# cyu0330/ptbxl-multimodal

Hardware: AMD Instinct MI355X
Metric: ECG windows/s (train step) at 12x1000, batch 256 (higher is better)
Workload: dtype f32; 1 GPU; ECGCNN(5) train step fwd+BCE+bwd+AdamW, 12x1000, fp32, batch 256/GPU, global batch 256; global_batch=256, parallelism=dp1, loop=train_one_epoch, optimizer=FlatAdamW, priming_steps=30

## Files before the change

include/ecg_hip.h:

```cpp
#ifndef ECG_HIP_H
#define ECG_HIP_H

#include <stddef.h>
#include <stdint.h>

#ifdef __cplusplus
extern "C" {
#endif

typedef void *ecg_stream_t;

enum {
    ECG_OK = 0,
    ECG_EINVAL = 1,
    ECG_ELAUNCH = 2,
    ECG_ENODEV = 3
};

int ecg_version(void);
const char *ecg_last_error(void);
int ecg_check_device(void);


int ecg_conv1d_pack_weights(const float *w, float *w_fwd, float *w_bwd,
                            int C_out, int C_in, int K, ecg_stream_t stream);

int ecg_pack_weights_grouped(const float *const *w, float *const *w_fwd, float *const *w_bwd,
                             const int *C_out, const int *C_in, const int *K, int count,
                             ecg_stream_t stream);

int ecg_pack_weights_grouped_mixed(const float *const *w, float *const *w_fwd, float *const *w_bwd,
                                   void *const *wb_fwd, void *const *wb_bwd, const int *C_out,
                                   const int *C_in, const int *K, int count, ecg_stream_t stream);

int ecg_conv1d_fwd_stat_partials(int N, int C_in, int C_out, int L, int K, int pad);

int ecg_conv1d_fwd(const float *x, const float *w_fwd, const float *bias, float *y,
                   float *stat_partials, int N, int C_in, int C_out, int L, int K, int pad,
                   ecg_stream_t stream);

int ecg_conv1d_bwd_data(const float *dy, const float *w_bwd, float *dx,
                        int N, int C_in, int C_out, int L, int K, int pad, ecg_stream_t stream);

int ecg_conv1d_dy_row_stride(int N, int C_in, int C_out, int L, int K, int pad, int need_dx);

int ecg_conv1d_multiplies_per_output_pair(int op, int C_in, int C_out, int K, int pad);
int ecg_conv1d_bwd_data_ld(const float *dy, int ldy, const float *w_bwd, float *dx,
                           int N, int C_in, int C_out, int L, int K, int pad, ecg_stream_t stream);
int ecg_conv1d_bwd_weight_bias_ld(const float *dy, int ldy, const float *x, float *dw, float *db,
                                  float *ws, int N, int C_in, int C_out, int L, int K, int pad,
                                  ecg_stream_t stream);

size_t ecg_conv1d_bwd_weight_ws_floats(int N, int C_in, int C_out, int L, int K, int pad);
int ecg_conv1d_bwd_weight_bias(const float *dy, const float *x, float *dw, float *db, float *ws,
                               int N, int C_in, int C_out, int L, int K, int pad,
                               ecg_stream_t stream);

int ecg_conv1d_bf16_supported(int C_in, int C_out, int K, int pad);
size_t ecg_conv1d_bf16_packed_elems(int C_reduce, int C_result, int K);
int ecg_conv1d_pack_weights_bf16(const float *w, void *wb_fwd, void *wb_bwd, int C_out, int C_in,
                                 int K, ecg_stream_t stream);
int ecg_conv1d_fwd_bf16_yh(const void *x, int x_bf16, int ldx, const void *wb_fwd, const float *bias, void *y_bf16,
                           int ldy, float *stat_partials, int N, int C_in, int C_out, int L, int K, int pad,
                           ecg_stream_t stream);
int ecg_conv1d_fwd_bf16_yh_stat_partials(int N, int C_in, int C_out, int L, int K, int pad, int x_bf16, int ldx, int ldy);
int ecg_conv1d_bf16_ring_tile(int N, int C_red, int C_res, int L_out, int K, int pad, int ld_in, int ld_out);
int ecg_bn_stats_relu_pool_fwd_h(const float *stat_partials, int P, long long count, float *running_mean,
                                 float *running_var, long long *num_batches_tracked, float momentum, float eps,
                                 const void *y_bf16, int ldy, const float *gamma, const float *beta, float *mean,
                                 float *invstd, void *p_bf16, int ldp, int N, int C, int L, ecg_stream_t stream);
int ecg_bn_stats_relu_pool_gap_fwd_yh(const float *stat_partials, int P, long long count, float *running_mean,
                                      float *running_var, long long *num_batches_tracked, float momentum, float eps,
                                      const void *y_bf16, int ldy, const float *gamma, const float *beta, float *mean,
                                      float *invstd, float *out, int N, int C, int L, ecg_stream_t stream);
int ecg_bn_relu_pool_bwd_h(const void *y_bf16, int ldyy, const void *dp, int dp_kind, int ldp, const float *gamma,
                           const float *beta, const float *mean, const float *invstd, void *dy_bf16, int ldy,
                           float *dgamma, float *dbeta, float *ws, int N, int C, int L, int train,
                           ecg_stream_t stream);
int ecg_conv1d_bwd_data_bf16hh(const void *dy_bf16, int ldy, const void *wb_bwd, void *dx_bf16, int ldx, int N,
                               int C_in, int C_out, int L, int K, int pad, ecg_stream_t stream);
int ecg_conv1d_bf16_tk_supported(int C_in, int C_out, int K, int pad);
int ecg_conv1d_bf16_tk_dy_stride(int Lo);
size_t ecg_conv1d_bwd_weight_bf16_ncl_ws_floats(int N, int C_in, int C_out, int L, int K, int pad);
int ecg_conv1d_bwd_weight_bias_bf16_ncl(const void *dy_bf16, int ldy, const void *x, int x_is_bf16, int ldx,
                                        float *dw, float *db, float *ws, int N, int C_in, int C_out, int L,
                                        int K, int pad, ecg_stream_t stream);


int ecg_bn_stat_partials_count(int N, int C, int L);
int ecg_bn_stat_partials(const float *y, float *stat_partials, int N, int C, int L,
                         ecg_stream_t stream);

int ecg_bn_finalize(const float *stat_partials, int P, long long count,
                    float *mean, float *invstd, float *running_mean, float *running_var,
                    long long *num_batches_tracked, int C, float momentum, float eps,
                    ecg_stream_t stream);

int ecg_bn_invstd(const float *var, float *invstd, int C, float eps, ecg_stream_t stream);

int ecg_bn_relu_pool_fwd(const float *y, const float *gamma, const float *beta,
                         const float *mean, const float *invstd, float *p,
                         int N, int C, int L, ecg_stream_t stream);
int ecg_bn_stats_relu_pool_fwd(const float *stat_partials, int P, long long count, float *running_mean,
                               float *running_var, long long *num_batches_tracked, float momentum, float eps,
                               const float *y, const float *gamma, const float *beta, float *mean,
                               float *invstd, float *out, int N, int C, int L, int mode, ecg_stream_t stream);

int ecg_bn_relu_pool_bwd_one_launch_splits(int N, int C, int L, int ldy);
size_t ecg_bn_relu_pool_bwd_one_launch_counter_uints(int N, int C, int L, int ldy);
int ecg_bn_relu_pool_bwd_one_launch(const float *y, const float *dp, const float *gamma, const float *beta,
                                    const float *mean, const float *invstd, float *dy, int ldy,
                                    float *dgamma, float *dbeta, uint32_t *counters, int N, int C, int L,
                                    int train, int gap, int spin_polls, ecg_stream_t stream);

size_t ecg_bn_relu_pool_bwd_ws_floats(int N, int C, int L);
int ecg_bn_relu_pool_bwd(const float *y, const float *dp, const float *gamma, const float *beta,
                         const float *mean, const float *invstd,
                         float *dy, float *dgamma, float *dbeta, float *ws,
                         int N, int C, int L, int train, ecg_stream_t stream);
int ecg_bn_relu_pool_bwd_ld(const float *y, const float *dp, const float *gamma, const float *beta,
                            const float *mean, const float *invstd,
                            float *dy, int ldy, float *dgamma, float *dbeta, float *ws,
                            int N, int C, int L, int train, ecg_stream_t stream);

int ecg_conv1d_bn_relu_pool_eval_supported(int C_in, int C_out, int K, int pad);
int ecg_conv1d_bn_relu_pool_eval_fwd(const float *x, const float *w_fwd, const float *bias,
                                     const float *gamma, const float *beta,
                                     const float *running_mean, const float *running_var,
                                     float eps, float *p, int N, int C_in, int C_out, int L,
                                     int K, int pad, ecg_stream_t stream);
int ecg_conv1d_bn_relu_pool_gap_eval_supported(int C_in, int C_out, int L, int K, int pad);
int ecg_conv1d_bn_relu_pool_gap_eval_fwd(const float *x, const float *w_fwd, const float *bias,
                                         const float *gamma, const float *beta,
                                         const float *running_mean, const float *running_var,
                                         float eps, float *g, int N, int C_in, int C_out, int L,
                                         int K, int pad, ecg_stream_t stream);

int ecg_conv1d_bn_relu_pool_eval_bf16_supported(int C_in, int C_out, int L, int K, int pad, int gap);
int ecg_conv1d_bn_relu_pool_eval_fwd_bf16(const void *x, int x_bf16, int ldx, const void *wb_fwd, const float *bias,
                                          const float *gamma, const float *beta, const float *running_mean,
                                          const float *running_var, float eps, void *p, int p_bf16, int ldp, int N,
                                          int C_in, int C_out, int L, int K, int pad, ecg_stream_t stream);
int ecg_conv1d_bn_relu_pool_gap_eval_fwd_bf16(const void *x, int x_bf16, int ldx, const void *wb_fwd, const float *bias,
                                              const float *gamma, const float *beta, const float *running_mean,
                                              const float *running_var, float eps, float *g, int N, int C_in, int C_out,
                                              int L, int K, int pad, ecg_stream_t stream);

int ecg_bn_relu_pool_gap_fwd(const float *y, const float *gamma, const float *beta,
                             const float *mean, const float *invstd, float *g,
                             int N, int C, int L, ecg_stream_t stream);
int ecg_bn_relu_pool_gap_bwd(const float *y, const float *dg, const float *gamma, const float *beta,
                             const float *mean, const float *invstd,
                             float *dy, float *dgamma, float *dbeta, float *ws,
                             int N, int C, int L, int train, ecg_stream_t stream);
int ecg_bn_relu_pool_gap_bwd_ld(const float *y, const float *dg, const float *gamma,
                                const float *beta, const float *mean, const float *invstd,
                                float *dy, int ldy, float *dgamma, float *dbeta, float *ws,
                                int N, int C, int L, int train, ecg_stream_t stream);

int ecg_gradcam_supported(int C, int Lo, int K, int S);
size_t ecg_gradcam_ws_floats(int N, int C, int Lo, int K, int S);
int ecg_gradcam_fwd(const float *a, int lda, const float *scale, const float *shift, const float *u,
                    long long u_stride_n, float *cam, float *raw, float *alpha, float *g, float *ws,
                    int N, int C, int Lo, int K, int S, int norm, ecg_stream_t stream);

int ecg_bn_apply_fwd(const float *y, const float *gamma, const float *beta, const float *mean,
                     const float *invstd, float *out, int N, int C, int L, ecg_stream_t stream);
size_t ecg_bn_bwd_ws_floats(int N, int C, int L);
int ecg_bn_bwd(const float *y, const float *dout, const float *gamma, const float *mean,
               const float *invstd, float *dy, float *dgamma, float *dbeta, float *ws,
               int N, int C, int L, int train, ecg_stream_t stream);
int ecg_relu_fwd(const float *x, float *out, size_t n, ecg_stream_t stream);
int ecg_relu_bwd(const float *out, const float *dout, float *dx, size_t n, ecg_stream_t stream);
int ecg_maxpool2_fwd(const float *x, float *p, int rows, int L, ecg_stream_t stream);
int ecg_maxpool2_bwd(const float *x, const float *dp, float *dx, int rows, int L, ecg_stream_t stream);


int ecg_gap_fwd(const float *p, float *g, int rows, int L, ecg_stream_t stream);
int ecg_gap_bwd(const float *dg, float *dp, int rows, int L, ecg_stream_t stream);

int ecg_linear_fwd(const float *x, const float *w, const float *b, float *y,
                   int M, int In, int Out, int relu, ecg_stream_t stream);
size_t ecg_linear_bwd_ws_floats(int M, int In, int Out);
int ecg_linear_bwd(const float *x, const float *w, const float *y, const float *dy,
                   float *dx, float *dw, float *db, float *ws,
                   int M, int In, int Out, int relu, ecg_stream_t stream);

int ecg_film_fwd(const float *z, const float *film, float *zc, int M, int F, ecg_stream_t stream);
int ecg_film_bwd(const float *z, const float *film, const float *dzc, float *dz, float *dfilm,
                 int M, int F, ecg_stream_t stream);

int ecg_bce_logits_fwd(const float *x, const float *target, float *loss, float *dx,
                       int numel, double *running_sum, double weight, ecg_stream_t stream);
int ecg_sigmoid_fwd(const float *x, float *prob, size_t n, ecg_stream_t stream);


int ecg_transpose(const float *w, float *wT, int rows, int cols, ecg_stream_t stream);

int ecg_tail_fwd(const float *g, const float *xd, const float *WpT, const float *bp,
                 const float *W0, const float *b0, const float *W2, const float *b2,
                 const float *WfT, const float *bf, const float *Wh, const float *bh,
                 float *z, float *h1, float *h2, float *film, float *zc, float *logits,
                 int M, int F0, int F, int D, int H1, int H, int C, ecg_stream_t stream);

int ecg_tail_bwd_chain(const float *dlogits, const float *dz_extra, const float *z,
                       const float *h1, const float *h2, const float *film,
                       const float *Wp, const float *W0, const float *W2, const float *Wf,
                       const float *Wh, float *dzc, float *dz, float *dfilm, float *dh2m,
                       float *dh1m, float *dg, float *dxd, int M, int F0, int F, int D,
                       int H1, int H, int C, int demo, ecg_stream_t stream);

int ecg_linear_wgrad_grouped(const float *const *G, const float *const *X, float *const *dW,
                             float *const *db, const int *Out, const int *In, int count,
                             int M, ecg_stream_t stream);

int ecg_adamw_step(float *p, const float *g, float *m, float *v, size_t n, int step,
                   float lr, float beta1, float beta2, float eps, float weight_decay,
                   float grad_scale, ecg_stream_t stream);

int ecg_adamw_step_graph(float *p, const float *g, float *m, float *v, size_t n, int *step_dev,
                         float lr, float beta1, float beta2, float eps, float weight_decay,
                         float grad_scale, ecg_stream_t stream);

int ecg_wfdb16_physical(const int16_t *d, const double *gain, const int *baseline, float *out,
                        int B, int T, int leads, ecg_stream_t stream);
int ecg_wfdb16_zscore(const int16_t *d, const double *gain, const int *baseline, float *out,
                      float *stats, int B, int T, int leads, ecg_stream_t stream);
int ecg_zscore_rows(const float *x, float *out, float *stats, int rows, int T, ecg_stream_t stream);
int ecg_host_gather_rows(const void *src, size_t row_bytes, const long long *rows, int n, void *dst);

#ifdef __cplusplus
}
#endif
#endif
```

ptbxl-multimodal_amd/csrc/conv1d_api.hip:

```cpp
#include "common.h"

namespace ecg {
int direct_fwd_stat_partials(int N, int Lo);
int direct_fwd(const float *x, const float *wp, const float *bias, float *y, float *partials,
               int N, int Cin, int Cout, int L, int K, int pad, hipStream_t st);
size_t direct_wgrad_ws_floats(int N, int Cin, int Cout, int K);
int direct_wgrad(const float *dy, const float *x, float *dw, float *db, float *ws, int N, int Cin,
                 int Cout, int L, int K, int pad, hipStream_t st);
int pack_weights(const float *w, float *w_fwd, float *w_bwd, int Co, int Ci, int K,
                 hipStream_t st);
int pack_weights_grouped(const float *const *w, float *const *w_fwd, float *const *w_bwd, void *const *wb_fwd,
                         void *const *wb_bwd, const int *Co, const int *Ci, const int *K, int count, hipStream_t st);
bool mfma_fwd_supported(int Cin, int Cout, int K, int pad);
int mfma_fwd_stat_partials(int N, int Cin, int Cout, int Lo);
int mfma_fwd(const float *x, int ldx, const float *wp, const float *bias, float *y, float *partials,
             int N, int Cin, int Cout, int L, int K, int pad, hipStream_t st);
int mfma_fwd_eval_pool(const float *x, const float *wp, const float *bias, const float *gamma,
                       const float *beta, const float *mean, const float *var, float eps, float *p,
                       int N, int Cin, int Cout, int L, int K, int pad, hipStream_t st, int gap);
bool mfma_fwd_eval_gap_supported(int Cin, int Cout, int L, int K, int pad);
bool mfma_wgrad_supported(int Cin, int Cout, int K, int pad);
size_t mfma_wgrad_ws_floats(int N, int Cin, int Cout, int L, int K, int pad);
bool mfma_wgrad_dma_supported(int Cin, int Cout, int K);
int mfma_multiplies_per_pair(int op, int Cin, int Cout, int K, int pad);
int mfma_wgrad(const float *dy, int ldy, const float *x, float *dw, float *db, float *ws, int N,
               int Cin, int Cout, int L, int K, int pad, hipStream_t st);

static int check_conv_shape(int N, int Cin, int Cout, int L, int K, int pad) {
    ECG_REQUIRE(N > 0 && Cin > 0 && Cout > 0 && L > 0, "conv1d: N=%d C_in=%d C_out=%d L=%d must be > 0",
                N, Cin, Cout, L);
    ECG_REQUIRE(K >= 1 && K <= 31, "conv1d: kernel size %d outside [1,31]", K);
    ECG_REQUIRE(pad >= 0 && pad < K, "conv1d: padding %d outside [0,K)", pad);
    ECG_REQUIRE(L + 2 * pad - K + 1 > 0, "conv1d: empty output (L=%d K=%d pad=%d)", L, K, pad);
    ECG_REQUIRE(N <= 65535, "conv1d: N=%d exceeds grid.z limit 65535", N);
    return ECG_OK;
}
}

using namespace ecg;

ECG_API int ecg_conv1d_pack_weights(const float *w, float *w_fwd, float *w_bwd, int C_out,
                                    int C_in, int K, ecg_stream_t stream) {
    ECG_REQUIRE(w && (w_fwd || w_bwd), "pack_weights: null pointer");
    ECG_REQUIRE(C_out > 0 && C_in > 0 && K >= 1 && K <= 31, "pack_weights: bad shape");
    return pack_weights(w, w_fwd, w_bwd, C_out, C_in, K, as_stream(stream));
}

ECG_API int ecg_pack_weights_grouped(const float *const *w, float *const *w_fwd,
                                     float *const *w_bwd, const int *C_out, const int *C_in,
                                     const int *K, int count, ecg_stream_t stream) {
    ECG_REQUIRE(w && w_fwd && w_bwd && C_out && C_in && K, "pack_weights_grouped: null table");
    ECG_REQUIRE(count >= 1 && count <= 16, "pack_weights_grouped: count=%d outside [1,16]", count);
    for (int q = 0; q < count; ++q) {
        ECG_REQUIRE(w[q] && (w_fwd[q] || w_bwd[q]), "pack_weights_grouped: problem %d has null pointers", q);
        ECG_REQUIRE(C_out[q] > 0 && C_in[q] > 0 && K[q] >= 1 && K[q] <= 31,
                    "pack_weights_grouped: problem %d has a bad shape", q);
    }
    return pack_weights_grouped(w, w_fwd, w_bwd, nullptr, nullptr, C_out, C_in, K, count, as_stream(stream));
}

ECG_API int ecg_pack_weights_grouped_mixed(const float *const *w, float *const *w_fwd, float *const *w_bwd,
                                           void *const *wb_fwd, void *const *wb_bwd, const int *C_out,
                                           const int *C_in, const int *K, int count, ecg_stream_t stream) {
    ECG_REQUIRE(w && w_fwd && w_bwd && wb_fwd && wb_bwd && C_out && C_in && K, "pack_weights_grouped_mixed: null table");
    ECG_REQUIRE(count >= 1 && count <= 16, "pack_weights_grouped_mixed: count=%d outside [1,16]", count);
    for (int q = 0; q < count; ++q) {
        ECG_REQUIRE(w[q] && (w_fwd[q] || w_bwd[q] || wb_fwd[q] || wb_bwd[q]),
                    "pack_weights_grouped_mixed: problem %d has null pointers", q);
        ECG_REQUIRE(C_out[q] > 0 && C_in[q] > 0 && K[q] >= 1 && K[q] <= 31,
                    "pack_weights_grouped_mixed: problem %d has a bad shape", q);
        ECG_REQUIRE(K[q] <= 15 || !(wb_fwd[q] || wb_bwd[q]),
                    "pack_weights_grouped_mixed: problem %d asks for bf16 operands with K=%d > 15", q, K[q]);
    }
    return pack_weights_grouped(w, w_fwd, w_bwd, wb_fwd, wb_bwd, C_out, C_in, K, count, as_stream(stream));
}

ECG_API int ecg_conv1d_fwd_stat_partials(int N, int C_in, int C_out, int L, int K, int pad) {
    int Lo = L + 2 * pad - K + 1;
    if (mfma_fwd_supported(C_in, C_out, K, pad)) return mfma_fwd_stat_partials(N, C_in, C_out, Lo);
    return direct_fwd_stat_partials(N, Lo);
}

ECG_API int ecg_conv1d_fwd(const float *x, const float *w_fwd, const float *bias, float *y,
                           float *stat_partials, int N, int C_in, int C_out, int L, int K, int pad,
                           ecg_stream_t stream) {
    int rc = check_conv_shape(N, C_in, C_out, L, K, pad);
    if (rc) return rc;
    ECG_REQUIRE(x && w_fwd && y, "conv1d_fwd: null pointer");
    if (mfma_fwd_supported(C_in, C_out, K, pad))
        return mfma_fwd(x, L, w_fwd, bias, y, stat_partials, N, C_in, C_out, L, K, pad, as_stream(stream));
    return direct_fwd(x, w_fwd, bias, y, stat_partials, N, C_in, C_out, L, K, pad, as_stream(stream));
}

ECG_API int ecg_conv1d_dy_row_stride(int N, int C_in, int C_out, int L, int K, int pad, int need_dx) {
    (void)N;
    const int Lo = L + 2 * pad - K + 1;
    if (Lo <= 0) return Lo;
    if (mfma_wgrad_dma_supported(C_in, C_out, K) && (!need_dx || mfma_fwd_supported(C_out, C_in, K, K - 1 - pad)))
        return cdiv(Lo, 64) * 64;
    return Lo;
}

ECG_API int ecg_conv1d_multiplies_per_output_pair(int op, int C_in, int C_out, int K, int pad) {
    if (op < 0 || op > 3 || K < 1) return 0;
    return mfma_multiplies_per_pair(op, C_in, C_out, K, pad);
}

ECG_API int ecg_conv1d_bwd_data_ld(const float *dy, int ldy, const float *w_bwd, float *dx, int N,
                                   int C_in, int C_out, int L, int K, int pad, ecg_stream_t stream) {
    int rc = check_conv_shape(N, C_in, C_out, L, K, pad);
    if (rc) return rc;
    ECG_REQUIRE(dy && w_bwd && dx, "conv1d_bwd_data: null pointer");
    const int Lo = L + 2 * pad - K + 1, padb = K - 1 - pad;
    ECG_REQUIRE(ldy >= Lo, "conv1d_bwd_data: dY row stride %d < row length %d", ldy, Lo);
    if (mfma_fwd_supported(C_out, C_in, K, padb))
        return mfma_fwd(dy, ldy, w_bwd, nullptr, dx, nullptr, N, C_out, C_in, Lo, K, padb, as_stream(stream));
    ECG_REQUIRE(ldy == Lo, "conv1d_bwd_data: this shape needs dense dY rows (stride %d != %d); "
                "use the stride ecg_conv1d_dy_row_stride returns", ldy, Lo);
    return direct_fwd(dy, w_bwd, nullptr, dx, nullptr, N, C_out, C_in, Lo, K, padb, as_stream(stream));
}

ECG_API int ecg_conv1d_bwd_data(const float *dy, const float *w_bwd, float *dx, int N, int C_in,
                                int C_out, int L, int K, int pad, ecg_stream_t stream) {
    return ecg_conv1d_bwd_data_ld(dy, L + 2 * pad - K + 1, w_bwd, dx, N, C_in, C_out, L, K, pad, stream);
}

ECG_API size_t ecg_conv1d_bwd_weight_ws_floats(int N, int C_in, int C_out, int L, int K, int pad) {
    if (mfma_wgrad_supported(C_in, C_out, K, pad)) return mfma_wgrad_ws_floats(N, C_in, C_out, L, K, pad);
    return direct_wgrad_ws_floats(N, C_in, C_out, K);
}

ECG_API int ecg_conv1d_bwd_weight_bias_ld(const float *dy, int ldy, const float *x, float *dw,
                                          float *db, float *ws, int N, int C_in, int C_out, int L,
                                          int K, int pad, ecg_stream_t stream) {
    int rc = check_conv_shape(N, C_in, C_out, L, K, pad);
    if (rc) return rc;
    ECG_REQUIRE(dy && x && dw && ws, "conv1d_bwd_weight_bias: null pointer");
    const int Lo = L + 2 * pad - K + 1;
    ECG_REQUIRE(ldy >= Lo, "conv1d_bwd_weight_bias: dY row stride %d < row length %d", ldy, Lo);
    if (mfma_wgrad_supported(C_in, C_out, K, pad))
        return mfma_wgrad(dy, ldy, x, dw, db, ws, N, C_in, C_out, L, K, pad, as_stream(stream));
    ECG_REQUIRE(ldy == Lo, "conv1d_bwd_weight_bias: this shape needs dense dY rows (stride %d != %d); "
                "use the stride ecg_conv1d_dy_row_stride returns", ldy, Lo);
    return direct_wgrad(dy, x, dw, db, ws, N, C_in, C_out, L, K, pad, as_stream(stream));
}

ECG_API int ecg_conv1d_bwd_weight_bias(const float *dy, const float *x, float *dw, float *db,
                                       float *ws, int N, int C_in, int C_out, int L, int K, int pad,
                                       ecg_stream_t stream) {
    return ecg_conv1d_bwd_weight_bias_ld(dy, L + 2 * pad - K + 1, x, dw, db, ws, N, C_in, C_out, L, K,
                                         pad, stream);
}

ECG_API int ecg_conv1d_bn_relu_pool_eval_supported(int C_in, int C_out, int K, int pad) {
    return mfma_fwd_supported(C_in, C_out, K, pad) ? 1 : 0;
}

ECG_API int ecg_conv1d_bn_relu_pool_eval_fwd(const float *x, const float *w_fwd, const float *bias,
                                             const float *gamma, const float *beta,
                                             const float *running_mean, const float *running_var,
                                             float eps, float *p, int N, int C_in, int C_out, int L,
                                             int K, int pad, ecg_stream_t stream) {
    int rc = check_conv_shape(N, C_in, C_out, L, K, pad);
    if (rc) return rc;
    ECG_REQUIRE(x && w_fwd && gamma && beta && running_mean && running_var,
                "conv1d_bn_relu_pool_eval_fwd: null pointer");
    ECG_REQUIRE(mfma_fwd_supported(C_in, C_out, K, pad),
                "conv1d_bn_relu_pool_eval_fwd: shape not covered by the fused kernel "
                "(query ecg_conv1d_bn_relu_pool_eval_supported and use the unfused sequence)");
    const int Lo = L + 2 * pad - K + 1;
    if (Lo / 2 == 0) return ECG_OK;
    ECG_REQUIRE(p, "conv1d_bn_relu_pool_eval_fwd: null output");
    return mfma_fwd_eval_pool(x, w_fwd, bias, gamma, beta, running_mean, running_var, eps, p, N,
                              C_in, C_out, L, K, pad, as_stream(stream), 0);
}

ECG_API int ecg_conv1d_bn_relu_pool_gap_eval_supported(int C_in, int C_out, int L, int K, int pad) {
    return mfma_fwd_eval_gap_supported(C_in, C_out, L, K, pad) ? 1 : 0;
}

ECG_API int ecg_conv1d_bn_relu_pool_gap_eval_fwd(const float *x, const float *w_fwd, const float *bias,
                                                 const float *gamma, const float *beta,
                                                 const float *running_mean, const float *running_var,
                                                 float eps, float *g, int N, int C_in, int C_out, int L,
                                                 int K, int pad, ecg_stream_t stream) {
    int rc = check_conv_shape(N, C_in, C_out, L, K, pad);
    if (rc) return rc;
    ECG_REQUIRE(x && w_fwd && gamma && beta && running_mean && running_var && g,
                "conv1d_bn_relu_pool_gap_eval_fwd: null pointer");
    ECG_REQUIRE(mfma_fwd_eval_gap_supported(C_in, C_out, L, K, pad),
                "conv1d_bn_relu_pool_gap_eval_fwd: shape not covered (the conv output row must fit one time tile; "
                "query ecg_conv1d_bn_relu_pool_gap_eval_supported)");
    return mfma_fwd_eval_pool(x, w_fwd, bias, gamma, beta, running_mean, running_var, eps, g, N,
                              C_in, C_out, L, K, pad, as_stream(stream), 1);
}
```

ptbxl-multimodal_amd/csrc/conv1d_direct.hip:

```cpp
#include "common.h"
#include <cstdlib>

namespace ecg {

constexpr int kTT = 256;
constexpr int kKMax = 31;
constexpr int kCiChunk = 8;

__global__ void pack_weights_kernel(const float *__restrict__ w, float *__restrict__ w_fwd,
                                    float *__restrict__ w_bwd, int Co, int Ci, int K) {
    int idx = blockIdx.x * blockDim.x + threadIdx.x;
    int total = Co * Ci * K;
    if (idx >= total) return;
    int k = idx % K;
    int ci = (idx / K) % Ci;
    int co = idx / (K * Ci);
    float v = w[idx];
    if (w_fwd) w_fwd[((size_t)k * Ci + ci) * Co + co] = v;
    if (w_bwd) w_bwd[((size_t)(K - 1 - k) * Co + co) * Ci + ci] = v;
}

template <int CO_T, bool STATS>
__global__ __launch_bounds__(kTT) void conv1d_direct_kernel(
    const float *__restrict__ x, const float *__restrict__ wp, const float *__restrict__ bias,
    float *__restrict__ y, float *__restrict__ partials, int Cin, int Cout, int L, int Lo, int K,
    int pad, int P) {
    __shared__ float xs[kCiChunk][kTT + kKMax - 1];
    __shared__ float red[4][CO_T * 2];

    const int tl = threadIdx.x;
    const int t0 = blockIdx.x * kTT;
    const int co0 = blockIdx.y * CO_T;
    const int n = blockIdx.z;
    const int span = kTT + K - 1;

    float acc[CO_T];
#pragma unroll
    for (int j = 0; j < CO_T; ++j) acc[j] = 0.f;

    const float *xn = x + (size_t)n * Cin * L;
    for (int ci0 = 0; ci0 < Cin; ci0 += kCiChunk) {
        const int nci = min(kCiChunk, Cin - ci0);
        for (int c = 0; c < nci; ++c) {
            const float *xr = xn + (size_t)(ci0 + c) * L;
            for (int i = tl; i < span; i += kTT) {
                int s = t0 - pad + i;
                xs[c][i] = (s >= 0 && s < L) ? xr[s] : 0.f;
            }
        }
        __syncthreads();
        for (int c = 0; c < nci; ++c) {
            for (int k = 0; k < K; ++k) {
                const float xv = xs[c][tl + k];
                const float *wr = wp + ((size_t)k * Cin + (ci0 + c)) * Cout + co0;
#pragma unroll
                for (int j = 0; j < CO_T; ++j) acc[j] = __fmaf_rn(wr[j], xv, acc[j]);
            }
        }
        __syncthreads();
    }

    const int t = t0 + tl;
    const bool valid = t < Lo;
#pragma unroll
    for (int j = 0; j < CO_T; ++j) {
        if (bias) acc[j] += bias[co0 + j];
        if (valid) y[((size_t)n * Cout + co0 + j) * Lo + t] = acc[j];
    }

    if (STATS) {
        const int wave = tl >> 6, lane = tl & 63;
#pragma unroll
        for (int j = 0; j < CO_T; ++j) {
            float v = valid ? acc[j] : 0.f;
            float s = wave_sum(v), q = wave_sum(v * v);
            if (lane == 0) { red[wave][2 * j] = s; red[wave][2 * j + 1] = q; }
        }
        __syncthreads();
        if (tl < CO_T * 2) {
            float s = red[0][tl] + red[1][tl] + red[2][tl] + red[3][tl];
            int j = tl >> 1;
            int pidx = n * gridDim.x + blockIdx.x;
            partials[((size_t)(co0 + j) * P + pidx) * 2 + (tl & 1)] = s;
        }
    }
}

static int pick_co_tile(int Cout) {
    for (int c : {16, 8, 4, 2}) if (Cout % c == 0) return c;
    return 1;
}

template <bool STATS>
static void launch_direct(const float *x, const float *wp, const float *bias, float *y,
                          float *partials, int N, int Cin, int Cout, int L, int Lo, int K, int pad,
                          int P, hipStream_t st) {
    int cot = pick_co_tile(Cout);
    dim3 grid(cdiv(Lo, kTT), Cout / cot, N), block(kTT);
#define ECG_LAUNCH(CT) \
    hipLaunchKernelGGL((conv1d_direct_kernel<CT, STATS>), grid, block, 0, st, x, wp, bias, y, \
                       partials, Cin, Cout, L, Lo, K, pad, P)
    switch (cot) {
        case 16: ECG_LAUNCH(16); break;
        case 8: ECG_LAUNCH(8); break;
        case 4: ECG_LAUNCH(4); break;
        case 2: ECG_LAUNCH(2); break;
        default: ECG_LAUNCH(1); break;
    }
#undef ECG_LAUNCH
}

int direct_fwd_stat_partials(int N, int Lo) { return N * cdiv(Lo, kTT); }

int direct_fwd(const float *x, const float *wp, const float *bias, float *y, float *partials,
               int N, int Cin, int Cout, int L, int K, int pad, hipStream_t st) {
    const int Lo = L + 2 * pad - K + 1;
    const int P = direct_fwd_stat_partials(N, Lo);
    if (partials)
        launch_direct<true>(x, wp, bias, y, partials, N, Cin, Cout, L, Lo, K, pad, P, st);
    else
        launch_direct<false>(x, wp, bias, y, nullptr, N, Cin, Cout, L, Lo, K, pad, P, st);
    return check_launch("conv1d_direct_kernel");
}

template <int KK, int CO_R>
__global__ __launch_bounds__(kTT) void conv1d_wgrad_direct_kernel(
    const float *__restrict__ dy, const float *__restrict__ x, float *__restrict__ slab,
    int N, int Cin, int Cout, int L, int Lo, int pad, int S) {
    __shared__ float xs[kTT + KK - 1];
    __shared__ float red[4][CO_R * KK + CO_R];

    const int tl = threadIdx.x;
    const int ci = blockIdx.x;
    const int co0 = blockIdx.y * CO_R;
    const int s = blockIdx.z;
    const int n_begin = (int)((long long)N * s / S), n_end = (int)((long long)N * (s + 1) / S);

    float acc[CO_R][KK];
    float bacc[CO_R];
#pragma unroll
    for (int j = 0; j < CO_R; ++j) {
        bacc[j] = 0.f;
#pragma unroll
        for (int k = 0; k < KK; ++k) acc[j][k] = 0.f;
    }

    for (int n = n_begin; n < n_end; ++n) {
        const float *xr = x + ((size_t)n * Cin + ci) * L;
        const float *dyn = dy + ((size_t)n * Cout + co0) * Lo;
        for (int t0 = 0; t0 < Lo; t0 += kTT) {
            __syncthreads();
            for (int i = tl; i < kTT + KK - 1; i += kTT) {
                int sidx = t0 - pad + i;
                xs[i] = (sidx >= 0 && sidx < L) ? xr[sidx] : 0.f;
            }
            __syncthreads();
            const int t = t0 + tl;
            float xv[KK];
#pragma unroll
            for (int k = 0; k < KK; ++k) xv[k] = xs[tl + k];
#pragma unroll
            for (int j = 0; j < CO_R; ++j) {
                float d = (t < Lo) ? dyn[(size_t)j * Lo + t] : 0.f;
                bacc[j] += d;
#pragma unroll
                for (int k = 0; k < KK; ++k) acc[j][k] = __fmaf_rn(d, xv[k], acc[j][k]);
            }
        }
    }

    const int wave = tl >> 6, lane = tl & 63;
#pragma unroll
    for (int j = 0; j < CO_R; ++j) {
#pragma unroll
        for (int k = 0; k < KK; ++k) {
            float v = wave_sum(acc[j][k]);
            if (lane == 0) red[wave][j * KK + k] = v;
        }
        float b = wave_sum(bacc[j]);
        if (lane == 0) red[wave][CO_R * KK + j] = b;
    }
    __syncthreads();
    const size_t wslab = (size_t)Cout * Cin * KK;
    if (tl < CO_R * KK) {
        int j = tl / KK, k = tl % KK;
        float v = red[0][tl] + red[1][tl] + red[2][tl] + red[3][tl];
        slab[(size_t)s * wslab + ((size_t)(co0 + j) * Cin + ci) * KK + k] = v;
    } else if (tl < CO_R * KK + CO_R && ci == 0) {
        int j = tl - CO_R * KK;
        float v = red[0][tl] + red[1][tl] + red[2][tl] + red[3][tl];
        slab[(size_t)S * wslab + (size_t)s * Cout + co0 + j] = v;
    }
}

__global__ __launch_bounds__(kTT) void conv1d_wgrad_generic_kernel(
    const float *__restrict__ dy, const float *__restrict__ x, float *__restrict__ slab,
    int N, int Cin, int Cout, int L, int Lo, int K, int pad) {
    __shared__ double red[4];
    const int ci = blockIdx.x, co = blockIdx.y, tl = threadIdx.x;
    const int wave = tl >> 6, lane = tl & 63;
    const size_t wslab = (size_t)Cout * Cin * K;
    for (int k = 0; k <= K; ++k) {
        if (k == K && ci != 0) break;
        double a = 0.0;
        for (int n = 0; n < N; ++n) {
            const float *dyr = dy + ((size_t)n * Cout + co) * Lo;
            const float *xr = x + ((size_t)n * Cin + ci) * L;
            for (int t = tl; t < Lo; t += kTT) {
                if (k == K) { a += dyr[t]; continue; }
                int sidx = t + k - pad;
                if (sidx >= 0 && sidx < L) a += (double)dyr[t] * (double)xr[sidx];
            }
        }
        a = wave_sum(a);
        __syncthreads();
        if (lane == 0) red[wave] = a;
        __syncthreads();
        if (tl == 0) {
            float v = (float)(red[0] + red[1] + red[2] + red[3]);
            if (k == K) slab[wslab + co] = v;
            else slab[((size_t)co * Cin + ci) * K + k] = v;
        }
    }
}

template <int G>
__global__ __launch_bounds__(64 * G) void wgrad_reduce_kernel(const float *__restrict__ slab,
                                                              float *__restrict__ dw,
                                                              float *__restrict__ db, size_t wslab,
                                                              int Cout, int S) {
    __shared__ double part[G][64];
    const int lane = threadIdx.x & 63, w = threadIdx.x >> 6;
    const size_t i = (size_t)blockIdx.x * 64 + lane;
    const size_t total = wslab + Cout;
    const bool live = i < total && (i < wslab || db);
    double a = 0.0;
    if (live) {
        const float *src = i < wslab ? slab + i : slab + (size_t)S * wslab + (i - wslab);
        const size_t stride = i < wslab ? wslab : (size_t)Cout;
        int s = w;
        for (; s + 3 * G < S; s += 4 * G) {
            const float v0 = src[(size_t)s * stride], v1 = src[(size_t)(s + G) * stride];
            const float v2 = src[(size_t)(s + 2 * G) * stride], v3 = src[(size_t)(s + 3 * G) * stride];
            a += (double)v0; a += (double)v1; a += (double)v2; a += (double)v3;
        }
        for (; s < S; s += G) a += (double)src[(size_t)s * stride];
    }
    if (G > 1) {
        part[w][lane] = a;
        __syncthreads();
        if (w != 0) return;
#pragma unroll
        for (int g = 1; g < G; ++g) a += part[g][lane];
    }
    if (live) {
        if (i < wslab) dw[i] = (float)a; else db[i - wslab] = (float)a;
    }
}

template <int G>
__global__ __launch_bounds__(64 * G) void wgrad_reduce4_kernel(const float *__restrict__ slab, float *__restrict__ dw,
                                                               float *__restrict__ db, size_t wslab, int Cout, int S) {
    __shared__ double part[G][64][4];
    const int lane = threadIdx.x & 63, w = threadIdx.x >> 6;
    const size_t i = ((size_t)blockIdx.x * 64 + lane) * 4;
    const size_t total = wslab + Cout;
    const bool live = i < total && (i < wslab || db);
    double a[4] = {0.0, 0.0, 0.0, 0.0};
    if (live) {
        const float *src = i < wslab ? slab + i : slab + (size_t)S * wslab + (i - wslab);
        const size_t stride = i < wslab ? wslab : (size_t)Cout;
        int s = w;
        for (; s + 7 * G < S; s += 8 * G) {
            float4 v[8];
#pragma unroll
            for (int u = 0; u < 8; ++u) v[u] = *reinterpret_cast<const float4 *>(src + (size_t)(s + u * G) * stride);
#pragma unroll
            for (int u = 0; u < 8; ++u) {
                a[0] += (double)v[u].x; a[1] += (double)v[u].y; a[2] += (double)v[u].z; a[3] += (double)v[u].w;
            }
        }
        for (; s + 3 * G < S; s += 4 * G) {
            const float4 v0 = *reinterpret_cast<const float4 *>(src + (size_t)s * stride);
            const float4 v1 = *reinterpret_cast<const float4 *>(src + (size_t)(s + G) * stride);
            const float4 v2 = *reinterpret_cast<const float4 *>(src + (size_t)(s + 2 * G) * stride);
            const float4 v3 = *reinterpret_cast<const float4 *>(src + (size_t)(s + 3 * G) * stride);
            a[0] += (double)v0.x; a[0] += (double)v1.x; a[0] += (double)v2.x; a[0] += (double)v3.x;
            a[1] += (double)v0.y; a[1] += (double)v1.y; a[1] += (double)v2.y; a[1] += (double)v3.y;
            a[2] += (double)v0.z; a[2] += (double)v1.z; a[2] += (double)v2.z; a[2] += (double)v3.z;
            a[3] += (double)v0.w; a[3] += (double)v1.w; a[3] += (double)v2.w; a[3] += (double)v3.w;
        }
        for (; s < S; s += G) {
            const float4 v = *reinterpret_cast<const float4 *>(src + (size_t)s * stride);
            a[0] += (double)v.x; a[1] += (double)v.y; a[2] += (double)v.z; a[3] += (double)v.w;
        }
    }
    if (G > 1) {
#pragma unroll
        for (int e = 0; e < 4; ++e) part[w][lane][e] = a[e];
        __syncthreads();
        if (w != 0) return;
#pragma unroll
        for (int g = 1; g < G; ++g)
#pragma unroll
            for (int e = 0; e < 4; ++e) a[e] += part[g][lane][e];
    }
    if (live) {
        const float4 o = make_float4((float)a[0], (float)a[1], (float)a[2], (float)a[3]);
        if (i < wslab) *reinterpret_cast<float4 *>(dw + i) = o; else *reinterpret_cast<float4 *>(db + (i - wslab)) = o;
    }
}

int wgrad_reduce(const float *ws, float *dw, float *db, size_t wslab, int Cout, int S,
                 hipStream_t st) {
    const size_t total = wslab + Cout;
    if (wslab % 4 == 0 && Cout % 4 == 0 && (size_t)cdiv(total, 64) >= 1024 &&
        ((reinterpret_cast<uintptr_t>(ws) | reinterpret_cast<uintptr_t>(dw) | reinterpret_cast<uintptr_t>(db)) & 15) == 0) {
        hipLaunchKernelGGL((wgrad_reduce4_kernel<1>), dim3(cdiv(total / 4, 64)), dim3(64), 0, st, ws, dw, db, wslab, Cout, S);
        return check_launch("wgrad_reduce4_kernel");
    }
    const dim3 grid(cdiv(total, 64));
    int G = 1;
    while (G < 16 && (size_t)grid.x * G < 1024 && S / (2 * G) >= 8) G *= 2;
#define ECG_RED(GG) hipLaunchKernelGGL((wgrad_reduce_kernel<GG>), grid, dim3(64 * GG), 0, st, ws, dw, db, wslab, Cout, S)
    switch (G) {
        case 1: ECG_RED(1); break;
        case 2: ECG_RED(2); break;
        case 4: ECG_RED(4); break;
        case 8: ECG_RED(8); break;
        default: ECG_RED(16); break;
    }
#undef ECG_RED
    return check_launch("wgrad_reduce_kernel");
}

static bool wgrad_fast_ok(int Cout, int K) { return K == 15 && Cout % 8 == 0; }

int direct_wgrad_splits(int N, int Cin, int Cout, int K) {
    if (!wgrad_fast_ok(Cout, K)) return 1;
    long long base = (long long)Cin * (Cout / 8);
    long long s = (2048 + base - 1) / base;
    if (s < 1) s = 1;
    if (s > N) s = N;
    return (int)s;
}

size_t direct_wgrad_ws_floats(int N, int Cin, int Cout, int K) {
    int S = direct_wgrad_splits(N, Cin, Cout, K);
    return (size_t)S * ((size_t)Cout * Cin * K + Cout);
}

int direct_wgrad(const float *dy, const float *x, float *dw, float *db, float *ws, int N, int Cin,
                 int Cout, int L, int K, int pad, hipStream_t st) {
    const int Lo = L + 2 * pad - K + 1;
    const int S = direct_wgrad_splits(N, Cin, Cout, K);
    const size_t wslab = (size_t)Cout * Cin * K;
    if (wgrad_fast_ok(Cout, K)) {
        dim3 grid(Cin, Cout / 8, S), block(kTT);
        hipLaunchKernelGGL((conv1d_wgrad_direct_kernel<15, 8>), grid, block, 0, st, dy, x, ws, N,
                           Cin, Cout, L, Lo, pad, S);
    } else {
        dim3 grid(Cin, Cout), block(kTT);
        hipLaunchKernelGGL(conv1d_wgrad_generic_kernel, grid, block, 0, st, dy, x, ws, N, Cin,
                           Cout, L, Lo, K, pad);
    }
    int rc = check_launch("conv1d_wgrad kernel");
    if (rc) return rc;
    return wgrad_reduce(ws, dw, db, wslab, Cout, S, st);
}

int pack_weights(const float *w, float *w_fwd, float *w_bwd, int Co, int Ci, int K, hipStream_t st);

constexpr int kMaxPack = 16;
constexpr int kPackCo = 16, kPackCi = 16, kPackKMax = 15;
struct PackProb { const float *w; float *w_fwd, *w_bwd; unsigned short *wb_fwd, *wb_bwd; int Co, Ci, K, block0, ci_tiles; };
struct PackArgs { PackProb p[kMaxPack]; int count; };

__device__ __forceinline__ unsigned pack_bf16_pair(float lo, float hi) {
    return (unsigned)__builtin_bit_cast(unsigned short, (__bf16)lo) | ((unsigned)__builtin_bit_cast(unsigned short, (__bf16)hi) << 16);
}

__device__ __forceinline__ void pack_tile_bf16(const PackProb &pr, const float *tile, int ld, int co0, int ci0, int nco,
                                               int nci, int tid) {
    const int K = pr.K;
    if (pr.wb_fwd) {
        unsigned *dst = reinterpret_cast<unsigned *>(pr.wb_fwd + ((size_t)(ci0 / kPackCi) * K * pr.Co + co0) * kPackCi);
        for (int e = tid; e < K * nco * 8; e += 256) {
            const int jp = e & 7, r = e >> 3, co = r % nco, k = r / nco;
            const float lo = 2 * jp < nci ? tile[co * ld + (2 * jp) * K + k] : 0.f;
            const float hi = 2 * jp + 1 < nci ? tile[co * ld + (2 * jp + 1) * K + k] : 0.f;
            dst[((size_t)k * pr.Co + co) * 8 + jp] = pack_bf16_pair(lo, hi);
        }
    }
    if (pr.wb_bwd) {
        unsigned *dst = reinterpret_cast<unsigned *>(pr.wb_bwd + ((size_t)(co0 / kPackCo) * K * pr.Ci + ci0) * kPackCo);
        for (int e = tid; e < K * nci * 8; e += 256) {
            const int jp = e & 7, r = e >> 3, ci = r % nci, k = r / nci;
            const float lo = 2 * jp < nco ? tile[(2 * jp) * ld + ci * K + (K - 1 - k)] : 0.f;
            const float hi = 2 * jp + 1 < nco ? tile[(2 * jp + 1) * ld + ci * K + (K - 1 - k)] : 0.f;
            dst[((size_t)k * pr.Ci + ci) * 8 + jp] = pack_bf16_pair(lo, hi);
        }
    }
}

__global__ __launch_bounds__(256) void pack_weights_grouped_kernel(PackArgs a) {
    __shared__ float tile[kPackCo * (kPackCi * kPackKMax + 1)];
    int pi = 0;
#pragma unroll
    for (int q = 1; q < kMaxPack; ++q)
        if (q < a.count && (int)blockIdx.x >= a.p[q].block0) pi = q;
    const PackProb pr = a.p[pi];
    const int t = (int)blockIdx.x - pr.block0;
    const int co0 = (t / pr.ci_tiles) * kPackCo, ci0 = (t % pr.ci_tiles) * kPackCi;
    const int nco = min(kPackCo, pr.Co - co0), nci = min(kPackCi, pr.Ci - ci0);
    const int K = pr.K, run = nci * K, ld = kPackCi * kPackKMax + 1;
    const int tid = threadIdx.x;
    if (K == 15 && nco == kPackCo && nci == kPackCi) {
        constexpr int KC = 15, RUN = kPackCi * KC;
        const float *src = pr.w + ((size_t)co0 * pr.Ci + ci0) * KC;
        static_assert((kPackCo * RUN) % 256 == 0, "whole passes");
#pragma unroll
        for (int it = 0; it < kPackCo * RUN / 256; ++it) {
            const int e = tid + 256 * it;
            const int co = e / RUN, r = e - co * RUN;
            tile[co * ld + r] = src[(size_t)co * pr.Ci * KC + r];
        }
        __syncthreads();
        if (pr.w_fwd) {
#pragma unroll
            for (int it = 0; it < kPackCo * RUN / 256; ++it) {
                const int e = tid + 256 * it;
                const int co = e % kPackCo, r = e / kPackCo, k = r / kPackCi, ci = r - k * kPackCi;
                pr.w_fwd[((size_t)k * pr.Ci + ci0 + ci) * pr.Co + co0 + co] = tile[co * ld + ci * KC + k];
            }
        }
        if (pr.w_bwd) {
#pragma unroll
            for (int it = 0; it < kPackCo * RUN / 256; ++it) {
                const int e = tid + 256 * it;
                const int ci = e % kPackCi, r = e / kPackCi, co = r % kPackCo, k = r / kPackCo;
                pr.w_bwd[((size_t)(KC - 1 - k) * pr.Co + co0 + co) * pr.Ci + ci0 + ci] = tile[co * ld + ci * KC + k];
            }
        }
        pack_tile_bf16(pr, tile, ld, co0, ci0, nco, nci, tid);
        return;
    }
    for (int e = tid; e < nco * run; e += 256) {
        const int co = e / run, r = e - co * run;
        tile[co * ld + r] = pr.w[((size_t)(co0 + co) * pr.Ci + ci0) * K + r];
    }
    __syncthreads();
    if (pr.w_fwd)
        for (int e = tid; e < run * kPackCo; e += 256) {
            const int co = e % kPackCo, r = e / kPackCo;
            const int k = r / nci, ci = r - k * nci;
            if (co < nco) pr.w_fwd[((size_t)k * pr.Ci + ci0 + ci) * pr.Co + co0 + co] = tile[co * ld + ci * K + k];
        }
    if (pr.w_bwd)
        for (int e = tid; e < K * nco * nci; e += 256) {
            const int ci = e % nci, r = e / nci;
            const int co = r % nco, k = r / nco;
            pr.w_bwd[((size_t)(K - 1 - k) * pr.Co + co0 + co) * pr.Ci + ci0 + ci] = tile[co * ld + ci * K + k];
        }
    pack_tile_bf16(pr, tile, ld, co0, ci0, nco, nci, tid);
}

int pack_weights_grouped(const float *const *w, float *const *w_fwd, float *const *w_bwd, void *const *wb_fwd,
                         void *const *wb_bwd, const int *Co, const int *Ci, const int *K, int count, hipStream_t st) {
    PackArgs a;
    a.count = count;
    int blocks = 0;
    for (int q = 0; q < count; ++q) {
        if (K[q] > kPackKMax) {
            int rc = pack_weights(w[q], w_fwd[q], w_bwd[q], Co[q], Ci[q], K[q], st);
            if (rc) return rc;
            a.p[q] = PackProb{nullptr, nullptr, nullptr, nullptr, nullptr, 0, 0, 1, blocks, 1};
            continue;
        }
        const int ci_tiles = cdiv(Ci[q], kPackCi);
        a.p[q] = PackProb{w[q], w_fwd[q], w_bwd[q], static_cast<unsigned short *>(wb_fwd ? wb_fwd[q] : nullptr),
                          static_cast<unsigned short *>(wb_bwd ? wb_bwd[q] : nullptr), Co[q], Ci[q], K[q], blocks, ci_tiles};
        blocks += cdiv(Co[q], kPackCo) * ci_tiles;
    }
    for (int q = count; q < kMaxPack; ++q) a.p[q] = PackProb{nullptr, nullptr, nullptr, nullptr, nullptr, 0, 0, 1, 1 << 30, 1};
    if (blocks == 0) return ECG_OK;
    hipLaunchKernelGGL(pack_weights_grouped_kernel, dim3(blocks), dim3(256), 0, st, a);
    return check_launch("pack_weights_grouped_kernel");
}

int pack_weights(const float *w, float *w_fwd, float *w_bwd, int Co, int Ci, int K,
                 hipStream_t st) {
    int total = Co * Ci * K;
    hipLaunchKernelGGL(pack_weights_kernel, dim3(cdiv(total, 256)), dim3(256), 0, st, w, w_fwd,
                       w_bwd, Co, Ci, K);
    return check_launch("pack_weights_kernel");
}

}
```

ptbxl-multimodal_amd/csrc/conv1d_mfma.hip:

```cpp
#include "mfma_util.h"
#include <cstdlib>
#include <type_traits>

namespace ecg {

constexpr int kKM = 15;

#ifdef ECG_STAMP
__device__ unsigned long long *g_stamps = nullptr;
#endif

__device__ __forceinline__ f32x16 mfma32(float a, float b, f32x16 c) {
    return __builtin_amdgcn_mfma_f32_32x32x2f32(a, b, c, 0, 0, 0);
}

__device__ __forceinline__ void wait_lgkm_f(int n) {
    switch (n) {
        case 1: __builtin_amdgcn_s_waitcnt(0xC17F); break;
        case 2: __builtin_amdgcn_s_waitcnt(0xC27F); break;
        case 3: __builtin_amdgcn_s_waitcnt(0xC37F); break;
        case 4: __builtin_amdgcn_s_waitcnt(0xC47F); break;
        default: break;
    }
}

enum { EPI_PLAIN = 0, EPI_STATS = 1, EPI_EVAL = 2, EPI_EVAL_GAP = 3 };
struct EvalEpi { const float *gamma, *beta, *mean, *var; float eps; int gap; };

#ifndef ECG_FFA_MINB
#define ECG_FFA_MINB 2
#endif
#ifndef ECG_FFA_FLP2
#define ECG_FFA_FLP2 64
#endif
template <int CO_T, int M_T, int WCO, int WT, int EPI, int CI_C = 4, int FLP = 1>
__global__ __launch_bounds__(256, ECG_FFA_MINB) void conv1d_mfma_ffa_kernel(
    const float *__restrict__ x, const float *__restrict__ wp, const float *__restrict__ bias,
    float *__restrict__ y, float *__restrict__ partials, int Cin, int Cout, int L, int ldx, int Lo,
    int pad, int P, int tiles_t, EvalEpi ev) {
    constexpr bool STATS = (EPI == EPI_STATS), GAP = (EPI == EPI_EVAL_GAP);
    constexpr bool EVALM = (EPI == EPI_EVAL || EPI == EPI_EVAL_GAP);
    static_assert(WCO * WT == 4, "4 waves per workgroup");
    static_assert(kKM == 15, "tap split 8 + 7");
    static_assert(CO_T / WCO == 32 && M_T / WT == 32, "one 32 x 32 accumulator per product and wave");
    constexpr int KK = kKM, NJ = (KK + 1) / 2, NST = NJ * (CI_C / 2);
    constexpr int T_T = 2 * M_T, TS = T_T - 2;
    constexpr int XS = T_T + 16;
    constexpr int WSZ = KK * CI_C * CO_T;
    constexpr int NDMA = (WSZ + 255) / 256;
    constexpr int WPAD = NDMA * 256;
    constexpr int DPW = (NDMA + 3) / 4;
    constexpr int XEL = CI_C * XS;
    constexpr int XLOADS = (XEL + 255) / 256;
    constexpr int IMG = WPAD + XEL;
    constexpr int BXS = M_T + 1;
    constexpr int REDF = (STATS || GAP) ? 4 * 32 * 2 : 0;
    static_assert(CO_T * BXS + REDF <= 2 * IMG, "B exchange + stat scratch alias the dead images");
    static_assert(NST >= 2 * XLOADS + DPW, "not enough steps to spread the staging over");

    __shared__ __attribute__((aligned(1024))) float lds[2 * IMG];

    const int tid = threadIdx.x, lane = tid & 63, wave = tid >> 6;
    const int half = lane >> 5, l31 = lane & 31;
    ECG_STAMP_AT(g_stamps, 0);
    const int CT = Cout / CO_T;
    const int tile = xcd_chunked(blockIdx.x, gridDim.x);
    const int tile_co = tile % CT, tile_nt = tile / CT;
    const int tile_t = tile_nt % tiles_t, n = tile_nt / tiles_t;
    const int t0 = tile_t * TS, co0 = tile_co * CO_T;
    const int wco = (wave / WT) * 32, wm = (wave % WT) * 32;
    const float *xn = x + (size_t)n * Cin * ldx;

    f32x16 acc[3], acc2[3];
    f32x16 zero16;
#pragma unroll
    for (int r = 0; r < 16; ++r) zero16[r] = 0.f;
#pragma unroll
    for (int a = 0; a < 3; ++a) { acc[a] = zero16; acc2[a] = zero16; }

    const int pch = co0 + wco + acc_row(l31 & 15, half);
    const float p_b = bias ? bias[pch] : 0.f;
    float p_mu = 0.f, p_sc = 0.f, p_be = 0.f;
    if (EVALM) {
        const float is = (float)(1.0 / sqrt((double)ev.var[pch] + (double)ev.eps));
        p_sc = is * ev.gamma[pch]; p_mu = ev.mean[pch]; p_be = ev.beta[pch];
    }

    int woff[DPW];
#pragma unroll
    for (int j = 0; j < DPW; ++j) {
        const int e = min(((j * 4 + wave) * 64 + lane) * 4, WSZ - 4);
        const int row = e / CO_T, col = e - row * CO_T;
        const int k = row / CI_C, ci = row - k * CI_C;
        woff[j] = (k * Cin + ci) * Cout + col;
    }
    int xoff[XLOADS];
    unsigned xmask = 0;
#pragma unroll
    for (int j = 0; j < XLOADS; ++j) {
        const int e = min(tid + 256 * j, XEL - 1);
        const int ci = e / XS, pos = e - ci * XS;
        const int s = t0 - pad + pos;
        xoff[j] = ci * ldx + min(max(s, 0), L - 1);
        xmask |= ((s >= 0) && (s < L)) ? (1u << j) : 0u;
    }
    float xreg[XLOADS];

    const unsigned lds_base = (unsigned)(size_t)(__attribute__((address_space(3))) float *)lds;
    const int wave_u = __builtin_amdgcn_readfirstlane(wave);
    auto dma_w = [&](int j, int ci0, float *img) {
        if ((j * 4 + wave_u) < NDMA)
            glds16(wp + (size_t)ci0 * Cout + co0, (unsigned)woff[j] * 4u,
                   (unsigned)__builtin_amdgcn_readfirstlane((int)(lds_base + (unsigned)((img - lds) + (j * 4 + wave_u) * 256) * 4u)));
    };
    auto load_x = [&](int j, int ci0) { xreg[j] = xn[(size_t)ci0 * ldx + xoff[j]]; };
    auto commit_x = [&](int j, float *img) {
        const int e = tid + 256 * j;
        const unsigned keep = 0u - ((xmask >> j) & 1u);
        if (256 * (j + 1) <= XEL || e < XEL)
            img[WPAD + e] = __uint_as_float(__float_as_uint(xreg[j]) & keep);
    };

    const int nchunks = Cin / CI_C;
#pragma unroll
    for (int j = 0; j < DPW; ++j) dma_w(j, 0, lds);
#pragma unroll
    for (int j = 0; j < XLOADS; ++j) load_x(j, 0);
#pragma unroll
    for (int j = 0; j < XLOADS; ++j) commit_x(j, lds);
    if (nchunks > 1) {
#pragma unroll
        for (int j = 0; j < XLOADS; ++j) load_x(j, CI_C);
    }
    asm volatile("s_waitcnt vmcnt(0)" ::: "memory");
    __syncthreads();
    ECG_STAMP_AT(g_stamps, 1);

    typedef float f32x2t __attribute__((ext_vector_type(2)));
    auto chunk = [&](int c, auto open_c, auto close_c) {
        constexpr bool OPEN = decltype(open_c)::value, CLOSE = decltype(close_c)::value;
        const float *ws = lds + (c & 1) * IMG, *xs = ws + WPAD;
        float *nxt = lds + ((c + 1) & 1) * IMG;
        const bool do_next = c + 1 < nchunks, do_next2 = c + 2 < nchunks;
        const int ci_next = (c + 1) * CI_C, ci_next2 = (c + 2) * CI_C;

        auto ld = [&](int st, float &wa, float &wb, f32x2t &xq) {
            const int j = st / (CI_C / 2), cp = st % (CI_C / 2);
            const float *wrow = ws + ((2 * j * CI_C + 2 * cp + half) * CO_T + wco + l31);
            wa = wrow[0];
            wb = (2 * j + 1 < KK) ? wrow[CI_C * CO_T] : 0.f;
            xq = *reinterpret_cast<const f32x2t *>(xs + (2 * cp + half) * XS + 2 * (wm + l31) + 2 * j);
        };
        float wa_c, wb_c, wa_n, wb_n, wprev[CI_C / 2];
        f32x2t xq_c, xq_n;
#pragma unroll
        for (int i = 0; i < CI_C / 2; ++i) wprev[i] = 0.f;
        ld(0, wa_c, wb_c, xq_c);
#pragma unroll
        for (int st = 0; st < NST; ++st) {
            const int j = st / (CI_C / 2), cp = st % (CI_C / 2);
            ld(st + 1 < NST ? st + 1 : 0, wa_n, wb_n, xq_n);
            wait_lgkm_f(3);
            if (st < XLOADS) {
                if (do_next) commit_x(st, nxt);
            } else if (st < XLOADS + DPW) {
                if (do_next) dma_w(st - XLOADS, ci_next, nxt);
            } else if (st < 2 * XLOADS + DPW) {
                if (do_next2) load_x(st - XLOADS - DPW, ci_next2);
            }
            const float wc = wa_c - wprev[cp];
            const float xc = xq_c[0] - xq_c[1];
            __builtin_amdgcn_sched_barrier(0);
            acc[0] = mfma32(wa_c, xq_c[0], (OPEN && j == 0 && cp == 0) ? zero16 : acc[0]);
            if (2 * j + 1 < KK) acc[1] = mfma32(wb_c, xq_c[1], (OPEN && j == 0 && cp == 0) ? zero16 : acc[1]);
            acc[2] = mfma32(wc, xc, (OPEN && j == 0 && cp == 0) ? zero16 : acc[2]);
            __builtin_amdgcn_sched_barrier(0);
            wprev[cp] = wb_c;
            wa_c = wa_n; wb_c = wb_n; xq_c = xq_n;
        }
        if (CLOSE) {
#pragma unroll
            for (int a = 0; a < 3; ++a) acc2[a] += acc[a];
        }
        asm volatile("s_waitcnt vmcnt(0)" ::: "memory");
        __syncthreads();
        if (c == 0) ECG_STAMP_AT(g_stamps, 2);
    };
    {
        const std::true_type yes{};
        const std::false_type no{};
        int c = 0;
        if (FLP == 2) {
            for (; c + 1 < nchunks; c += 2) { chunk(c, yes, no); chunk(c + 1, no, yes); }
        }
        for (; c < nchunks; ++c) chunk(c, yes, yes);
    }
#pragma unroll
    for (int a = 0; a < 3; ++a) acc[a] = acc2[a];
    ECG_STAMP_AT(g_stamps, 3);

    __builtin_amdgcn_s_waitcnt(0x0F70);
    float *bx = lds, *red = lds + CO_T * BXS;
#pragma unroll
    for (int r = 0; r < 16; ++r) bx[(wco + acc_row(r, half)) * BXS + wm + l31] = acc[1][r];
    __syncthreads();
    f32x16 bn;
#pragma unroll
    for (int r = 0; r < 16; ++r) bn[r] = bx[(wco + acc_row(r, half)) * BXS + min(wm + l31 + 1, M_T - 1)];
    auto pick = [&](float v, int r) {
        const int vi = __float_as_int(v);
        const float lo = __int_as_float(__builtin_amdgcn_readlane(vi, r));
        const float hi = __int_as_float(__builtin_amdgcn_readlane(vi, r + 32));
        return half ? hi : lo;
    };
    float st_s = 0.f, st_q = 0.f;
    const int m = wm + l31, t = t0 + 2 * m;
    const bool ok0 = m < M_T - 1 && t < Lo, ok1 = m < M_T - 1 && t + 1 < Lo;
    const int Lp = Lo >> 1, pm = (t0 >> 1) + m;
    const bool okp = m < M_T - 1 && pm < Lp;
    float *yw = EVALM ? y + ((size_t)n * Cout + co0 + wco + 4 * half) * Lp + pm
                      : y + ((size_t)n * Cout + co0 + wco + 4 * half) * Lo + t;
#pragma unroll
    for (int r = 0; r < 16; ++r) {
        const int rowk = (r & 3) + 8 * (r >> 2);
        const float bv = pick(p_b, r);
        const float v0 = (acc[0][r] + acc[1][r]) + bv;
        const float v1 = ((acc[0][r] + bn[r]) - acc[2][r]) + bv;
        float s = 0.f, q = 0.f;
        if (EVALM) {
            const float mu = pick(p_mu, r), sc = pick(p_sc, r), be = pick(p_be, r);
            const float mx = fmaxf(fmaxf(bn_apply1(v0, mu, sc, be), bn_apply1(v1, mu, sc, be)), 0.f);
            if (GAP) {
                s = row16_sum(okp ? mx : 0.f);
                st_s += ((l31 & 15) == r) ? s : 0.f;
            } else if (okp) yw[rowk * Lp] = mx;
            continue;
        }
        typedef float f32x2u __attribute__((ext_vector_type(2), aligned(4)));
        if (ok1) { f32x2u v; v[0] = v0; v[1] = v1; *reinterpret_cast<f32x2u *>(yw + rowk * Lo) = v; }
        else if (ok0) yw[rowk * Lo] = v0;
        if (STATS) {
            if (ok0) { s += v0; q = __fmaf_rn(v0, v0, q); }
            if (ok1) { s += v1; q = __fmaf_rn(v1, v1, q); }
        }
        if (STATS) {
            const bool mine = (l31 & 15) == r;
            s = row16_sum(s);
            st_s += mine ? s : 0.f;
            q = row16_sum(q);
            st_q += mine ? q : 0.f;
        }
    }
    if (STATS || GAP) {
        const float s = st_s + __shfl_xor(st_s, 16, 64);
        const float q = st_q + __shfl_xor(st_q, 16, 64);
        if (l31 < 16) {
            const int lc = acc_row(l31, half);
            red[(wave * 32 + lc) * 2] = s;
            red[(wave * 32 + lc) * 2 + 1] = q;
        }
        __syncthreads();
    }
    if (GAP) {
        for (int col = tid; col < CO_T; col += 256) {
            const int wrow = col / 32, lc = col - wrow * 32;
            float g = 0.f;
#pragma unroll
            for (int j = 0; j < WT; ++j) g += red[((wrow * WT + j) * 32 + lc) * 2];
            y[(size_t)n * Cout + co0 + col] = g / (float)Lp;
        }
    }
    if (STATS) {
        for (int e = tid; e < CO_T * 2; e += 256) {
            const int col = e >> 1, w = e & 1;
            const int wrow = col / 32, lc = col - wrow * 32;
            float s2 = 0.f;
#pragma unroll
            for (int j = 0; j < WT; ++j) s2 += red[((wrow * WT + j) * 32 + lc) * 2 + w];
            const int pidx = n * tiles_t + tile_t;
            partials[((size_t)(co0 + col) * P + pidx) * 2 + w] = s2;
        }
    }
#ifdef ECG_STAMP
    asm volatile("s_waitcnt vmcnt(0)" ::: "memory");
#endif
    ECG_STAMP_AT(g_stamps, 4);
}

struct FwdCfg { int co_t, t_t, stride; };

static FwdCfg fwd_cfg(int Cout) {
    if (Cout % 64 == 0) return {64, 128, 126};
    return {32, 256, 254};
}

bool mfma_fwd_supported(int Cin, int Cout, int K, int pad) {
    (void)pad;
    return K == kKM && Cin % 4 == 0 && Cout % 32 == 0;
}

int mfma_fwd_stat_partials(int N, int Cin, int Cout, int Lo) {
    (void)Cin;
    return N * cdiv(Lo, fwd_cfg(Cout).stride);
}

template <int CO_T, int T_T, int WCO, int WT>
static void launch_fwd(const float *x, const float *wp, const float *bias, float *y,
                       float *partials, const EvalEpi *ev, int N, int Cin, int Cout, int L, int ldx,
                       int Lo, int pad, hipStream_t st) {
    const int tiles_t = cdiv(Lo, T_T - 2);
    dim3 grid((unsigned)((size_t)tiles_t * (Cout / CO_T) * N)), block(256);
    const int P = N * tiles_t;
    const EvalEpi none{nullptr, nullptr, nullptr, nullptr, 0.f, 0};
#define ECG_FFA(MODE, EV) do { \
    if (ECG_FFA_FLP2 && Cin % 8 == 0 && Cin >= ECG_FFA_FLP2) \
        hipLaunchKernelGGL((conv1d_mfma_ffa_kernel<CO_T, T_T / 2, WCO, WT, MODE, 4, 2>), grid, block, 0, st, x, wp, \
                           bias, y, partials, Cin, Cout, L, ldx, Lo, pad, P, tiles_t, EV); \
    else \
        hipLaunchKernelGGL((conv1d_mfma_ffa_kernel<CO_T, T_T / 2, WCO, WT, MODE>), grid, block, 0, st, x, wp, bias, y, \
                           partials, Cin, Cout, L, ldx, Lo, pad, P, tiles_t, EV); } while (0)
    if (ev && ev->gap) ECG_FFA(EPI_EVAL_GAP, *ev);
    else if (ev) ECG_FFA(EPI_EVAL, *ev);
    else if (partials) ECG_FFA(EPI_STATS, none);
    else ECG_FFA(EPI_PLAIN, none);
#undef ECG_FFA
}

static int mfma_fwd_any(const float *x, const float *wp, const float *bias, float *y,
                        float *partials, const EvalEpi *ev, int N, int Cin, int Cout, int L, int ldx,
                        int K, int pad, hipStream_t st) {
    const int Lo = L + 2 * pad - K + 1;
    if (fwd_cfg(Cout).co_t == 64)
        launch_fwd<64, 128, 2, 2>(x, wp, bias, y, partials, ev, N, Cin, Cout, L, ldx, Lo, pad, st);
    else
        launch_fwd<32, 256, 1, 4>(x, wp, bias, y, partials, ev, N, Cin, Cout, L, ldx, Lo, pad, st);
    return check_launch("conv1d_mfma_ffa_kernel");
}

int mfma_fwd(const float *x, int ldx, const float *wp, const float *bias, float *y, float *partials,
             int N, int Cin, int Cout, int L, int K, int pad, hipStream_t st) {
    return mfma_fwd_any(x, wp, bias, y, partials, nullptr, N, Cin, Cout, L, ldx, K, pad, st);
}

int mfma_fwd_eval_pool(const float *x, const float *wp, const float *bias, const float *gamma,
                       const float *beta, const float *mean, const float *var, float eps, float *p,
                       int N, int Cin, int Cout, int L, int K, int pad, hipStream_t st, int gap) {
    const EvalEpi ev{gamma, beta, mean, var, eps, gap};
    return mfma_fwd_any(x, wp, bias, p, nullptr, &ev, N, Cin, Cout, L, L, K, pad, st);
}

bool mfma_fwd_eval_gap_supported(int Cin, int Cout, int L, int K, int pad) {
    const int Lo = L + 2 * pad - K + 1;
    return mfma_fwd_supported(Cin, Cout, K, pad) && Lo >= 2 && Lo <= fwd_cfg(Cout).stride;
}

template <int M_T, int R_T, int WM, int WR, int WK, int T_T, int KK>
__global__ __launch_bounds__(256, 2) void conv1d_mfma_wgrad_kernel(
    const float *__restrict__ dy, const float *__restrict__ x, float *__restrict__ slab, int N,
    int Cin, int Cout, int L, int Lo, int ldy, int pad, int S) {
    static_assert(WM * WR * WK == 4, "4 waves per workgroup");
    constexpr int MC = M_T / WM / 32, MR = R_T / WR / 32;
    constexpr int TW = T_T / WK;
    constexpr int NST = TW / 2;
    constexpr int DS = T_T + 1;
    constexpr int XSPAN = T_T + KK - 1;
    constexpr int XS = ((XSPAN - KK + 31) / 32) * 32 + KK;
    constexpr int NCI = (R_T + KK - 2) / KK + 1;
    constexpr int DEL = M_T * T_T, DLOADS = DEL / 256;
    constexpr int XEL = NCI * XS, XLOADS = (XEL + 255) / 256;
    constexpr int NOPS = DLOADS + XLOADS;
    constexpr int IMG = M_T * DS + XEL;
    constexpr int ACCF = MC * MR * 16 * 64;
    constexpr int LDSF = (WK > 1 && WM * WR * ACCF > 2 * IMG) ? WM * WR * ACCF : 2 * IMG;
    static_assert(XS >= XSPAN, "x row stride too small");
    static_assert(DEL % 256 == 0, "dY tile must be a whole number of 256-thread passes");
    static_assert(256 % T_T == 0 || T_T % 256 == 0, "dY tile rows per pass");
    static_assert(XLOADS <= 32 && DLOADS <= 64, "mask bits");

    __shared__ float lds[LDSF + (WK > 1 ? 4 * 32 : 0)];

    const int tid = threadIdx.x, lane = tid & 63, wave = tid >> 6;
    const int half = lane >> 5, l31 = lane & 31;
    const int R = Cin * KK;
    const int RT = (R + R_T - 1) / R_T, CT = Cout / M_T;
    const int tile = xcd_chunked(blockIdx.x, gridDim.x);
    const int tile_r = tile % RT, tile_cs = tile / RT;
    const int r0 = tile_r * R_T, co0 = (tile_cs % CT) * M_T, s = tile_cs / CT;
    const int wk = wave % WK, wr = (wave / WK) % WR, wm = wave / (WK * WR);
    const int wm0 = wm * (M_T / WM), wr0 = wr * (R_T / WR), wt0 = wk * TW;
    const int ci_base = r0 / KK;
    const int n_begin = (int)((long long)N * s / S), n_end = (int)((long long)N * (s + 1) / S);

    int xcol[MR];
#pragma unroll
    for (int j = 0; j < MR; ++j) {
        int r = r0 + wr0 + 32 * j + l31;
        if (r >= R) r = R - 1;
        const int ci = r / KK;
        xcol[j] = (ci - ci_base) * XS + (r - ci * KK);
    }

    f32x16 acc[MC][MR], acc2[MC][MR];
    f32x16 zero16;
#pragma unroll
    for (int r = 0; r < 16; ++r) zero16[r] = 0.f;
#pragma unroll
    for (int a = 0; a < MC; ++a)
#pragma unroll
        for (int b = 0; b < MR; ++b) { acc[a][b] = zero16; acc2[a][b] = zero16; }
    float bsum[MC], bsum2[MC];
#pragma unroll
    for (int a = 0; a < MC; ++a) bsum[a] = bsum2[a] = 0.f;
    const bool want_bias = (tile_r == 0) && (wr == 0);

    constexpr int RPP = (T_T >= 256) ? 1 : 256 / T_T;
    constexpr int PPR = (T_T >= 256) ? T_T / 256 : 1;
    const int drow0 = (T_T >= 256) ? 0 : tid / T_T, dtt = (T_T >= 256) ? tid : tid % T_T;
    int xci[XLOADS], xpos[XLOADS];
#pragma unroll
    for (int j = 0; j < XLOADS; ++j) {
        const int e = min(tid + 256 * j, XEL - 1);
        xci[j] = min(ci_base + e / XS, Cin - 1) * L;
        xpos[j] = e % XS - pad;
    }
    float dreg[DLOADS], xreg[XLOADS];
    unsigned xmask = 0, dmask = 0;
    const int ntt = (Lo + T_T - 1) / T_T;
    const int total = (n_end - n_begin) * ntt;

    const float *dyn = dy, *xn = x;
    int dvoff = 0, t0 = 0;
    auto stage_setup = [&](int it) {
        const int n = n_begin + it / ntt;
        t0 = (it % ntt) * T_T;
        dyn = dy + ((size_t)n * Cout + co0) * ldy + t0;
        xn = x + (size_t)n * Cin * L;
        dvoff = drow0 * ldy + min(dtt, Lo - 1 - t0);
        dmask = 0;
#pragma unroll
        for (int q = 0; q < PPR; ++q) dmask |= (t0 + dtt + 256 * q < Lo) ? (1u << q) : 0u;
    };
    auto load_op = [&](int o) {
        if (o < DLOADS) {
            const int extra = (o % PPR) * 256;
            const float *pj = dyn + (size_t)(o / PPR) * RPP * ldy;
            dreg[o] = pj[PPR == 1 ? dvoff : drow0 * ldy + min(dtt + extra, Lo - 1 - t0)];
        } else {
            const int j = o - DLOADS;
            const int sidx = t0 + xpos[j];
            xreg[j] = xn[xci[j] + min(max(sidx, 0), L - 1)];
            const unsigned bit = ((sidx >= 0) && (sidx < L)) ? (1u << j) : 0u;
            xmask = (j == 0) ? bit : (xmask | bit);
        }
    };
    unsigned cxmask = 0, cdmask = 0;
    auto commit_op = [&](int o, float *img) {
        if (o < DLOADS) {
            const int row = drow0 + (o / PPR) * RPP, tt = dtt + (o % PPR) * 256;
            const unsigned keep = 0u - ((cdmask >> (o % PPR)) & 1u);
            img[row * DS + tt] = __uint_as_float(__float_as_uint(dreg[o]) & keep);
        } else {
            const int j = o - DLOADS;
            const int e = tid + 256 * j;
            const unsigned keep = 0u - ((cxmask >> j) & 1u);
            if (256 * (j + 1) <= XEL || e < XEL)
                img[M_T * DS + e] = __uint_as_float(__float_as_uint(xreg[j]) & keep);
        }
    };

    if (total > 0) {
        stage_setup(0);
#pragma unroll
        for (int o = 0; o < NOPS; ++o) load_op(o);
        cxmask = xmask; cdmask = dmask;
#pragma unroll
        for (int o = 0; o < NOPS; ++o) commit_op(o, lds);
        if (total > 1) {
            stage_setup(1);
#pragma unroll
            for (int o = 0; o < NOPS; ++o) load_op(o);
        }
    }
    __syncthreads();

    for (int it = 0; it < total; ++it) {
        const float *dys = lds + (it & 1) * IMG, *xs = dys + M_T * DS;
        float *nxt = lds + ((it + 1) & 1) * IMG;
        const bool do_commit = it + 1 < total, do_load = it + 2 < total;
        cxmask = xmask; cdmask = dmask;
        if (do_load) stage_setup(it + 2);

        const float *arow = dys + (wm0 + l31) * DS + wt0 + half;
        const float *brow = xs + wt0 + half;
        auto ld = [&](int tp, float *a, float *b) {
#pragma unroll
            for (int i = 0; i < MC; ++i) a[i] = arow[32 * i * DS + tp];
#pragma unroll
            for (int j = 0; j < MR; ++j) b[j] = brow[xcol[j] + tp];
        };
        float a_c[MC], b_c[MR], a_n[MC], b_n[MR];
        ld(0, a_c, b_c);
        constexpr int H1 = NST / 2;
#pragma unroll
        for (int st = 0; st < NST; ++st) {
            ld(st + 1 < NST ? 2 * (st + 1) : 0, a_n, b_n);
            if (st < H1) {
                if (do_commit) {
#pragma unroll
                    for (int o = st * NOPS / H1; o < (st + 1) * NOPS / H1; ++o) commit_op(o, nxt);
                }
            } else {
                if (do_load) {
#pragma unroll
                    for (int o = (st - H1) * NOPS / (NST - H1); o < (st - H1 + 1) * NOPS / (NST - H1); ++o)
                        load_op(o);
                }
            }
            __builtin_amdgcn_sched_barrier(0);
#pragma unroll
            for (int i = 0; i < MC; ++i) bsum[i] = (st == 0) ? a_c[i] : bsum[i] + a_c[i];
#pragma unroll
            for (int i = 0; i < MC; ++i)
#pragma unroll
                for (int j = 0; j < MR; ++j)
                    acc[i][j] = mfma32(a_c[i], b_c[j], (st == 0) ? zero16 : acc[i][j]);
            __builtin_amdgcn_sched_barrier(0);
#pragma unroll
            for (int i = 0; i < MC; ++i) a_c[i] = a_n[i];
#pragma unroll
            for (int j = 0; j < MR; ++j) b_c[j] = b_n[j];
        }
#pragma unroll
        for (int i = 0; i < MC; ++i)
#pragma unroll
            for (int j = 0; j < MR; ++j) acc2[i][j] += acc[i][j];
#pragma unroll
        for (int i = 0; i < MC; ++i) bsum2[i] += bsum[i];
        __syncthreads();
    }

#pragma unroll
    for (int i = 0; i < MC; ++i) {
        bsum[i] = bsum2[i];
#pragma unroll
        for (int j = 0; j < MR; ++j) acc[i][j] = acc2[i][j];
    }
    if (WK > 1) {
        float *bred = lds + LDSF;
        float *ex = lds + (wr + WR * wm) * ACCF;
        for (int w = 1; w < WK; ++w) {
            __syncthreads();
            if (wk == w) {
#pragma unroll
                for (int i = 0; i < MC; ++i)
#pragma unroll
                    for (int j = 0; j < MR; ++j)
#pragma unroll
                        for (int r = 0; r < 16; ++r)
                            ex[((i * MR + j) * 16 + r) * 64 + lane] = acc[i][j][r];
            }
            __syncthreads();
            if (wk == 0) {
#pragma unroll
                for (int i = 0; i < MC; ++i)
#pragma unroll
                    for (int j = 0; j < MR; ++j)
#pragma unroll
                        for (int r = 0; r < 16; ++r)
                            acc[i][j][r] += ex[((i * MR + j) * 16 + r) * 64 + lane];
            }
        }
        static_assert(WK == 1 || (WM == 1 && MC == 1), "the bias exchange below assumes one 32-channel row, wk fastest in the wave index");
        {
            const float b = bsum[0] + __shfl_xor(bsum[0], 32, 64);
            __syncthreads();
            if (want_bias && half == 0) bred[wave * 32 + l31] = b;
            __syncthreads();
            if (want_bias && wave == 0 && half == 0) {
                float t = bred[l31];
                for (int w = 1; w < WK; ++w) t += bred[w * 32 + l31];
                bsum[0] = t;
            }
        }
    } else if (want_bias) {
#pragma unroll
        for (int i = 0; i < MC; ++i) bsum[i] += __shfl_xor(bsum[i], 32, 64);
    }

    const size_t wslab = (size_t)Cout * R;
    if (wk == 0) {
        float *out = slab + (size_t)s * wslab;
#pragma unroll
        for (int i = 0; i < MC; ++i)
#pragma unroll
            for (int j = 0; j < MR; ++j) {
                const int r = r0 + wr0 + 32 * j + l31;
                if (r < R) {
#pragma unroll
                    for (int q = 0; q < 16; ++q) {
                        const int co = co0 + wm0 + 32 * i + acc_row(q, half);
                        out[(size_t)co * R + r] = acc[i][j][q];
                    }
                }
            }
        if (want_bias && half == 0) {
#pragma unroll
            for (int i = 0; i < MC; ++i)
                slab[(size_t)S * wslab + (size_t)s * Cout + co0 + wm0 + 32 * i + l31] = bsum[i];
        }
    }
}

template <int M_T, int R_T, int WM, int WR, int WK, int KK, int T_T = 64>
__global__ __launch_bounds__(256, 2) void conv1d_mfma_wgrad_dma_kernel(
    const float *__restrict__ dy, const float *__restrict__ x, float *__restrict__ slab, int N,
    int Cin, int Cout, int L, int Lo, int ldy, int pad, int S) {
    static_assert(WM * WR * WK == 4, "4 waves per workgroup");
    static_assert(T_T == 64 || T_T == 128, "64 or 128 time steps per stage");
    constexpr int LPR = T_T / 4, RPP = 64 / LPR;
    constexpr int MC = M_T / WM / 32, MR = R_T / WR / 32;
    constexpr int TW = T_T / WK;
    constexpr int NST = TW / 2, NGRP = NST / 4;
    static_assert(NST % 4 == 0, "whole groups of four steps");
    constexpr int XSPAN = T_T + KK - 1;
    constexpr int XS = ((XSPAN - KK + 31) / 32) * 32 + KK;
    constexpr int NCI = (R_T + KK - 2) / KK + 1;
    constexpr int XEL = NCI * XS, XLOADS = (XEL + 255) / 256;
    constexpr int AEL = M_T * T_T;
    constexpr int NDMA = AEL / 256;
    constexpr int DPW = NDMA / 4;
    constexpr int IMG = ((AEL + XEL + 63) / 64) * 64;
    constexpr int ACCF = MC * MR * 16 * 64;
    static_assert(WK == 1 || WM * WR * ACCF + 4 * 32 <= 2 * IMG, "accumulator exchange must fit the dead images");
    static_assert(XS >= XSPAN, "x row stride too small");
    static_assert(NDMA % 4 == 0, "dY image must split evenly over the four waves");
    static_assert(XLOADS <= 32, "mask bits");
    static_assert(NST >= 2 * XLOADS + DPW, "not enough steps to spread the staging over");

    __shared__ __attribute__((aligned(1024))) float lds[2 * IMG];
    ECG_STAMP_AT(g_stamps, 0);

    const int tid = threadIdx.x, lane = tid & 63, wave = tid >> 6;
    const int half = lane >> 5, l31 = lane & 31;
    const int R = Cin * KK;
    const int RT = (R + R_T - 1) / R_T, CT = Cout / M_T;
    const int tile = xcd_chunked(blockIdx.x, gridDim.x);
    const int tile_r = tile % RT, tile_cs = tile / RT;
    const int r0 = tile_r * R_T, co0 = (tile_cs % CT) * M_T, s = tile_cs / CT;
    const int wk = wave % WK, wr = (wave / WK) % WR, wm = wave / (WK * WR);
    const int wm0 = wm * (M_T / WM), wr0 = wr * (R_T / WR), wt0 = wk * TW;
    const int ci_base = r0 / KK;
    const int ntt = (Lo + T_T - 1) / T_T;
    const int it_begin = (int)((long long)N * ntt * s / S), it_end = (int)((long long)N * ntt * (s + 1) / S);

    int xcol[MR];
#pragma unroll
    for (int j = 0; j < MR; ++j) {
        int r = r0 + wr0 + 32 * j + l31;
        if (r >= R) r = R - 1;
        const int ci = r / KK;
        xcol[j] = (ci - ci_base) * XS + (r - ci * KK);
    }

    f32x16 acc[MC][MR], acc2[MC][MR];
    f32x16 zero16;
#pragma unroll
    for (int r = 0; r < 16; ++r) zero16[r] = 0.f;
#pragma unroll
    for (int a = 0; a < MC; ++a)
#pragma unroll
        for (int b = 0; b < MR; ++b) { acc[a][b] = zero16; acc2[a][b] = zero16; }
    float bsum[MC], bsum2[MC];
#pragma unroll
    for (int a = 0; a < MC; ++a) bsum[a] = bsum2[a] = 0.f;
    const bool want_bias = (tile_r == 0) && (wr == 0);

    int doff[DPW];
#pragma unroll
    for (int j = 0; j < DPW; ++j) {
        const int row = (j * 4 + wave) * RPP + lane / LPR;
        doff[j] = row * ldy + (((lane % LPR) ^ (row & 15)) << 2);
    }
    int xci[XLOADS], xpos[XLOADS];
#pragma unroll
    for (int j = 0; j < XLOADS; ++j) {
        const int e = min(tid + 256 * j, XEL - 1);
        xci[j] = min(ci_base + e / XS, Cin - 1) * L;
        xpos[j] = e % XS - pad;
    }
    float xreg[XLOADS];
    unsigned xmask = 0, cxmask = 0;
    const int total = it_end - it_begin;

    int sn = it_begin / ntt, stt = it_begin - sn * ntt;
    int dn = sn, dtt = stt;
    auto advance = [&]() { if (++stt == ntt) { stt = 0; ++sn; } };
    const unsigned lds_base = (unsigned)(size_t)(__attribute__((address_space(3))) float *)lds;
    const int wave_u = __builtin_amdgcn_readfirstlane(wave);
    auto dma_a = [&](int j, float *img) {
        const float *base = dy + ((size_t)min(dn, N - 1) * Cout + co0) * ldy + dtt * T_T;
        glds16(base, (unsigned)doff[j] * 4u,
               (unsigned)__builtin_amdgcn_readfirstlane((int)(lds_base + (unsigned)((img - lds) + (j * 4 + wave_u) * 256) * 4u)));
    };
    auto load_x = [&](int j) {
        const float *xn = x + (size_t)min(sn, N - 1) * Cin * L;
        const int sidx = stt * T_T + xpos[j];
        xreg[j] = xn[xci[j] + min(max(sidx, 0), L - 1)];
        const unsigned bit = ((sidx >= 0) && (sidx < L)) ? (1u << j) : 0u;
        xmask = (j == 0) ? bit : (xmask | bit);
    };
    auto commit_x = [&](int j, float *img) {
        const int e = tid + 256 * j;
        const unsigned keep = 0u - ((cxmask >> j) & 1u);
        if (256 * (j + 1) <= XEL || e < XEL)
            img[AEL + e] = __uint_as_float(__float_as_uint(xreg[j]) & keep);
    };

    if (total > 0) {
#pragma unroll
        for (int j = 0; j < DPW; ++j) dma_a(j, lds);
#pragma unroll
        for (int j = 0; j < XLOADS; ++j) load_x(j);
        cxmask = xmask;
#pragma unroll
        for (int j = 0; j < XLOADS; ++j) commit_x(j, lds);
        advance();
        dn = sn; dtt = stt;
#pragma unroll
        for (int j = 0; j < XLOADS; ++j) load_x(j);
        advance();
    }
    asm volatile("s_waitcnt vmcnt(0)" ::: "memory");
    __syncthreads();
    ECG_STAMP_AT(g_stamps, 1);

    const int aoff = (wm0 + l31) * T_T, swz = (l31 & 15) << 2;
    for (int it = 0; it < total; ++it) {
        const float *dys = lds + (it & 1) * IMG, *xs = dys + AEL;
        float *nxt = lds + ((it + 1) & 1) * IMG;
        cxmask = xmask;

        const float *arow = dys + aoff;
        const float *brow = xs + 4 * half + wt0;
        auto lda = [&](int g, f32x4 *a) {
#pragma unroll
            for (int i = 0; i < MC; ++i)
                a[i] = *reinterpret_cast<const f32x4 *>(arow + 32 * i * T_T + ((((2 * g) << 2) + (half << 2) + wt0) ^ swz));
        };
        auto ldb = [&](int st, float *b) {
            const int tp = 8 * (st >> 2) + (st & 3);
#pragma unroll
            for (int j = 0; j < MR; ++j) b[j] = brow[xcol[j] + tp];
        };
        f32x4 aq_c[MC], aq_n[MC];
        float b_c[MR], b_n[MR];
        lda(0, aq_c);
        ldb(0, b_c);
#pragma unroll
        for (int st = 0; st < NST; ++st) {
            const int j4 = st & 3;
            ldb(st + 1 < NST ? st + 1 : 0, b_n);
            if (j4 == 2 && (st >> 2) + 1 < NGRP) lda((st >> 2) + 1, aq_n);
            if (st < XLOADS) commit_x(st, nxt);
            else if (st < 2 * XLOADS) load_x(st - XLOADS);
            else if (st < 2 * XLOADS + DPW) dma_a(st - 2 * XLOADS, nxt);
            __builtin_amdgcn_sched_barrier(0);
#pragma unroll
            for (int i = 0; i < MC; ++i) bsum[i] = (st == 0) ? aq_c[i][j4] : bsum[i] + aq_c[i][j4];
#pragma unroll
            for (int i = 0; i < MC; ++i)
#pragma unroll
                for (int j = 0; j < MR; ++j)
                    acc[i][j] = mfma32(aq_c[i][j4], b_c[j], (st == 0) ? zero16 : acc[i][j]);
            __builtin_amdgcn_sched_barrier(0);
#pragma unroll
            for (int j = 0; j < MR; ++j) b_c[j] = b_n[j];
            if (j4 == 3) {
#pragma unroll
                for (int i = 0; i < MC; ++i) aq_c[i] = aq_n[i];
            }
        }
#pragma unroll
        for (int i = 0; i < MC; ++i)
#pragma unroll
            for (int j = 0; j < MR; ++j) acc2[i][j] += acc[i][j];
#pragma unroll
        for (int i = 0; i < MC; ++i) bsum2[i] += bsum[i];
        dn = sn; dtt = stt;
        advance();
        asm volatile("s_waitcnt vmcnt(0)" ::: "memory");
        __syncthreads();
        if (it == 0) ECG_STAMP_AT(g_stamps, 2);
    }
    ECG_STAMP_AT(g_stamps, 3);
#ifdef ECG_STAMP
    if (g_stamps && threadIdx.x == 0)
        g_stamps[(size_t)blockIdx.x * 8 + 5] = (unsigned long long)(total & 0xFFFF) |
            ((unsigned long long)__builtin_amdgcn_s_getreg((31 << 11) | 4) << 16) |
            ((unsigned long long)(__builtin_amdgcn_s_getreg((31 << 11) | 20) & 0xF) << 48);
#endif

#pragma unroll
    for (int i = 0; i < MC; ++i) {
        bsum[i] = bsum2[i];
#pragma unroll
        for (int j = 0; j < MR; ++j) acc[i][j] = acc2[i][j];
    }
    if (want_bias) {
#pragma unroll
        for (int i = 0; i < MC; ++i) bsum[i] += __shfl_xor(bsum[i], 32, 64);
    }
    if (WK > 1) {
        float *ex = lds + (wr + WR * wm) * ACCF, *bex = lds + WM * WR * ACCF;
        for (int w = 1; w < WK; ++w) {
            __syncthreads();
            if (wk == w) {
#pragma unroll
                for (int i = 0; i < MC; ++i)
#pragma unroll
                    for (int j = 0; j < MR; ++j)
#pragma unroll
                        for (int r = 0; r < 16; ++r) ex[((i * MR + j) * 16 + r) * 64 + lane] = acc[i][j][r];
                if (want_bias && half == 0 && MC == 1) bex[(wr + WR * wm) * 32 + l31] = bsum[0];
            }
            __syncthreads();
            if (wk == 0) {
#pragma unroll
                for (int i = 0; i < MC; ++i)
#pragma unroll
                    for (int j = 0; j < MR; ++j)
#pragma unroll
                        for (int r = 0; r < 16; ++r) acc[i][j][r] += ex[((i * MR + j) * 16 + r) * 64 + lane];
                if (want_bias && half == 0 && MC == 1) bsum[0] += bex[(wr + WR * wm) * 32 + l31];
            }
        }
        static_assert(WK == 1 || MC == 1, "the bias exchange above assumes one 32-channel row per wave");
        if (wk != 0) return;
    }
    const size_t wslab = (size_t)Cout * R;
    float *out = slab + (size_t)s * wslab;
#pragma unroll
    for (int i = 0; i < MC; ++i)
#pragma unroll
        for (int j = 0; j < MR; ++j) {
            const int r = r0 + wr0 + 32 * j + l31;
            if (r < R) {
#pragma unroll
                for (int q = 0; q < 16; ++q) {
                    const int co = co0 + wm0 + 32 * i + acc_row(q, half);
                    out[(size_t)co * R + r] = acc[i][j][q];
                }
            }
        }
    if (want_bias && half == 0) {
#pragma unroll
        for (int i = 0; i < MC; ++i)
            slab[(size_t)S * wslab + (size_t)s * Cout + co0 + wm0 + 32 * i + l31] = bsum[i];
    }
#ifdef ECG_STAMP
    asm volatile("s_waitcnt vmcnt(0)" ::: "memory");
#endif
    ECG_STAMP_AT(g_stamps, 4);
}

template <int M_T, int R_T, int WM, int WR, int T_T>
__global__ __launch_bounds__(256, 2) void conv1d_mfma_wgrad_ffa_kernel(
    const float *__restrict__ dy, const float *__restrict__ x, float *__restrict__ slab, int N,
    int Cin, int Cout, int L, int Lo, int ldy, int pad, int S) {
    static_assert(WM * WR == 4, "4 waves per workgroup");
    static_assert(kKM == 15, "tap split 8 + 7");
    static_assert(T_T == 64 || T_T == 128, "64 or 128 time steps per stage");
    constexpr int LPR = T_T / 4, RPP = 64 / LPR;
    constexpr int MC = M_T / WM / 32, MR = R_T / WR / 32;
    constexpr int NST = T_T / 4, NGRP = NST / 4;
    constexpr int XS = T_T + 16;
    static_assert(XS % 64 == 16, "x rows 16 banks apart");
    constexpr int NCI = (R_T + 6) / 7 + 1;
    constexpr int XEL = NCI * XS, XLOADS = (XEL + 255) / 256;
    constexpr int AEL = M_T * T_T;
    constexpr int NDMA = AEL / 256;
    constexpr int DPW = NDMA / 4;
    constexpr int IMG = ((AEL + XEL + 63) / 64) * 64;
    constexpr int OPS = 2 * XLOADS + DPW;
    static_assert(NDMA % 4 == 0, "dY image must split evenly over the four waves");
    static_assert(XLOADS <= 32, "mask bits");
    static_assert(2 * IMG * 4 <= 80 * 1024, "two workgroups per CU");

    __shared__ __attribute__((aligned(1024))) float lds[2 * IMG];
    ECG_STAMP_AT(g_stamps, 0);

    const int tid = threadIdx.x, lane = tid & 63, wave = tid >> 6;
    const int half = lane >> 5, l31 = lane & 31;
    const int RU = Cin * 8, RV = Cin * 7;
    const int TU = (RU + R_T - 1) / R_T, TV = (RV + R_T - 1) / R_T;
    const int RT = 2 * TU + TV, CT = Cout / M_T;
    const int tile = xcd_chunked(blockIdx.x, gridDim.x);
    const int tile_r = tile % RT, tile_cs = tile / RT;
    const int fam = tile_r < TU ? 0 : (tile_r < TU + TV ? 1 : 2);
    const int tile_rf = tile_r - (fam == 0 ? 0 : (fam == 1 ? TU : TU + TV));
    const int NJ = fam == 1 ? 7 : 8, RF = Cin * NJ, offf = fam == 0 ? 0 : (fam == 1 ? RU : RU + RV);
    const int r0 = tile_rf * R_T, co0 = (tile_cs % CT) * M_T, s = tile_cs / CT;
    const int wr = wave % WR, wm = wave / WR;
    const int wm0 = wm * (M_T / WM), wr0 = wr * (R_T / WR);
    const int ci_base = r0 / NJ;
    const int ntt = (Lo + T_T - 1) / T_T;
    const int it_begin = (int)((long long)N * ntt * s / S), it_end = (int)((long long)N * ntt * (s + 1) / S);

    int xcol[MR];
#pragma unroll
    for (int j = 0; j < MR; ++j) {
        int r = r0 + wr0 + 32 * j + l31;
        if (r >= RF) r = RF - 1;
        const int ci = r / NJ;
        xcol[j] = (ci - ci_base) * XS + 2 * (r - ci * NJ) + 8 * half;
    }

    f32x16 acc[MC][MR], acc2[MC][MR];
    f32x16 zero16;
#pragma unroll
    for (int r = 0; r < 16; ++r) zero16[r] = 0.f;
#pragma unroll
    for (int a = 0; a < MC; ++a)
#pragma unroll
        for (int b = 0; b < MR; ++b) { acc[a][b] = zero16; acc2[a][b] = zero16; }
    float bsum[MC], bsum2[MC];
#pragma unroll
    for (int a = 0; a < MC; ++a) bsum[a] = bsum2[a] = 0.f;
    const bool want_bias = (tile_r == 0) && (wr == 0);

    int doff[DPW];
#pragma unroll
    for (int j = 0; j < DPW; ++j) {
        const int row = (j * 4 + wave) * RPP + lane / LPR;
        doff[j] = row * ldy + (((lane % LPR) ^ (row & 15)) << 2);
    }
    float xreg[XLOADS];
    unsigned xmask = 0, cxmask = 0;
    const int total = it_end - it_begin;

    int sn = it_begin / ntt, stt = it_begin - sn * ntt;
    int dn = sn, dtt = stt;
    auto advance = [&]() { if (++stt == ntt) { stt = 0; ++sn; } };
    const unsigned lds_base = (unsigned)(size_t)(__attribute__((address_space(3))) float *)lds;
    const int wave_u = __builtin_amdgcn_readfirstlane(wave);
    auto dma_a = [&](int j, float *img) {
        const float *base = dy + ((size_t)min(dn, N - 1) * Cout + co0) * ldy + dtt * T_T;
        glds16(base, (unsigned)doff[j] * 4u,
               (unsigned)__builtin_amdgcn_readfirstlane((int)(lds_base + (unsigned)((img - lds) + (j * 4 + wave_u) * 256) * 4u)));
    };
    auto load_x = [&](int j) {
        const float *xn = x + (size_t)min(sn, N - 1) * Cin * L;
        const int e = min(tid + 256 * j, XEL - 1), row = e / XS;
        const int sidx = stt * T_T + (e - row * XS) - pad;
        xreg[j] = xn[min(ci_base + row, Cin - 1) * L + min(max(sidx, 0), L - 1)];
        const unsigned bit = ((sidx >= 0) && (sidx < L)) ? (1u << j) : 0u;
        xmask = (j == 0) ? bit : (xmask | bit);
    };
    auto commit_x = [&](int j, float *img) {
        const int e = tid + 256 * j;
        const unsigned keep = 0u - ((cxmask >> j) & 1u);
        if (256 * (j + 1) <= XEL || e < XEL)
            img[AEL + e] = __uint_as_float(__float_as_uint(xreg[j]) & keep);
    };

    if (total > 0) {
#pragma unroll
        for (int j = 0; j < DPW; ++j) dma_a(j, lds);
#pragma unroll
        for (int j = 0; j < XLOADS; ++j) load_x(j);
        cxmask = xmask;
#pragma unroll
        for (int j = 0; j < XLOADS; ++j) commit_x(j, lds);
        advance();
        dn = sn; dtt = stt;
#pragma unroll
        for (int j = 0; j < XLOADS; ++j) load_x(j);
        advance();
    }
    asm volatile("s_waitcnt vmcnt(0)" ::: "memory");
    __syncthreads();
    ECG_STAMP_AT(g_stamps, 1);

    typedef float f32x2t __attribute__((ext_vector_type(2)));
    const int aoff = (wm0 + l31) * T_T, swz = (l31 & 15) << 2;
    auto stage = [&](auto fam_c, int it) {
        constexpr int FAM = decltype(fam_c)::value;
        const float *dys = lds + (it & 1) * IMG, *xs = dys + AEL;
        float *nxt = lds + ((it + 1) & 1) * IMG;
        cxmask = xmask;
        const float *arow = dys + aoff;
        auto lda_lo = [&](int g, f32x4 *lo, float *prev) {
#pragma unroll
            for (int i = 0; i < MC; ++i) {
                const float *rb = arow + 32 * i * T_T;
                const int c0 = 4 * g + 2 * half;
                lo[i] = *reinterpret_cast<const f32x4 *>(rb + ((c0 << 2) ^ swz));
                if (FAM == 1) {
                    const float pv = rb[((max(c0 - 1, 0) << 2) ^ swz) + 3];
                    prev[i] = (g == 0 && half == 0) ? 0.f : pv;
                }
            }
        };
        auto lda_hi = [&](int g, f32x4 *hi) {
#pragma unroll
            for (int i = 0; i < MC; ++i)
                hi[i] = *reinterpret_cast<const f32x4 *>(arow + 32 * i * T_T + (((4 * g + 2 * half + 1) << 2) ^ swz));
        };
        auto ldb = [&](int st, f32x2t *b) {
            const int tp = 16 * (st >> 2) + 2 * (st & 3);
#pragma unroll
            for (int j = 0; j < MR; ++j) b[j] = *reinterpret_cast<const f32x2t *>(xs + xcol[j] + tp);
        };
        f32x4 lo_c[MC], hi_c[MC], lo_n[MC];
        float pv_c[MC], pv_n[MC];
        f32x2t b_c[MR], b_n[MR];
        lda_lo(0, lo_c, pv_c);
        lda_hi(0, hi_c);
        ldb(0, b_c);
#pragma unroll
        for (int st = 0; st < NST; ++st) {
            const int j4 = st & 3;
            ldb(st + 1 < NST ? st + 1 : 0, b_n);
            if (j4 == 2 && (st >> 2) + 1 < NGRP) lda_lo((st >> 2) + 1, lo_n, pv_n);
            if (j4 == 0 && st > 0) lda_hi(st >> 2, hi_c);
#pragma unroll
            for (int o = st * OPS / NST; o < (st + 1) * OPS / NST; ++o) {
                if (o < DPW) dma_a(o, nxt);
                else if (o < DPW + XLOADS) commit_x(o - DPW, nxt);
                else load_x(o - DPW - XLOADS);
            }
            float av[MC], bv[MR];
#pragma unroll
            for (int i = 0; i < MC; ++i) {
                const f32x4 d = j4 < 2 ? lo_c[i] : hi_c[i];
                const float d0 = d[2 * (j4 & 1)], d1 = d[2 * (j4 & 1) + 1];
                const float dp = j4 == 0 ? pv_c[i] : (j4 == 1 ? lo_c[i][1] : (j4 == 2 ? lo_c[i][3] : hi_c[i][1]));
                av[i] = FAM == 0 ? d0 + d1 : (FAM == 1 ? d0 + dp : d1);
            }
#pragma unroll
            for (int j = 0; j < MR; ++j) bv[j] = FAM == 0 ? b_c[j][0] : (FAM == 1 ? b_c[j][1] : b_c[j][0] - b_c[j][1]);
            __builtin_amdgcn_sched_barrier(0);
            if (FAM == 0) {
#pragma unroll
                for (int i = 0; i < MC; ++i) bsum[i] = (st == 0) ? av[i] : bsum[i] + av[i];
            }
#pragma unroll
            for (int i = 0; i < MC; ++i)
#pragma unroll
                for (int j = 0; j < MR; ++j)
                    acc[i][j] = mfma32(av[i], bv[j], (st == 0) ? zero16 : acc[i][j]);
            __builtin_amdgcn_sched_barrier(0);
#pragma unroll
            for (int j = 0; j < MR; ++j) b_c[j] = b_n[j];
            if (j4 == 3) {
#pragma unroll
                for (int i = 0; i < MC; ++i) { lo_c[i] = lo_n[i]; pv_c[i] = pv_n[i]; }
            }
        }
        if (FAM == 1) {
#pragma unroll
            for (int i = 0; i < MC; ++i) {
                const float dl = arow[32 * i * T_T + (((LPR - 1) << 2) ^ swz) + 3];
                const float a = half ? 0.f : dl;
#pragma unroll
                for (int j = 0; j < MR; ++j)
                    acc[i][j] = mfma32(a, xs[xcol[j] - 8 * half + T_T + 1], acc[i][j]);
            }
        }
#pragma unroll
        for (int i = 0; i < MC; ++i)
#pragma unroll
            for (int j = 0; j < MR; ++j) acc2[i][j] += acc[i][j];
        if (FAM == 0) {
#pragma unroll
            for (int i = 0; i < MC; ++i) bsum2[i] += bsum[i];
        }
        dn = sn; dtt = stt;
        advance();
        asm volatile("s_waitcnt vmcnt(%0)" :: "n"(XLOADS) : "memory");
        __syncthreads();
    };
    if (fam == 0) { for (int it = 0; it < total; ++it) { stage(std::integral_constant<int, 0>{}, it); if (it == 0) ECG_STAMP_AT(g_stamps, 2); } }
    else if (fam == 1) { for (int it = 0; it < total; ++it) { stage(std::integral_constant<int, 1>{}, it); if (it == 0) ECG_STAMP_AT(g_stamps, 2); } }
    else { for (int it = 0; it < total; ++it) { stage(std::integral_constant<int, 2>{}, it); if (it == 0) ECG_STAMP_AT(g_stamps, 2); } }
    ECG_STAMP_AT(g_stamps, 3);
#ifdef ECG_STAMP
    if (g_stamps && threadIdx.x == 0)
        g_stamps[(size_t)blockIdx.x * 8 + 5] = (unsigned long long)(total & 0xFFFF) |
            ((unsigned long long)__builtin_amdgcn_s_getreg((31 << 11) | 4) << 16) |
            ((unsigned long long)(__builtin_amdgcn_s_getreg((31 << 11) | 20) & 0xF) << 48);
#endif

#pragma unroll
    for (int i = 0; i < MC; ++i) {
        bsum[i] = bsum2[i];
#pragma unroll
        for (int j = 0; j < MR; ++j) acc[i][j] = acc2[i][j];
    }
    if (want_bias) {
#pragma unroll
        for (int i = 0; i < MC; ++i) bsum[i] += __shfl_xor(bsum[i], 32, 64);
    }
    const size_t RVT = (size_t)Cin * 23, wslab = (size_t)Cout * RVT;
    float *out = slab + (size_t)s * wslab + offf;
#pragma unroll
    for (int i = 0; i < MC; ++i)
#pragma unroll
        for (int j = 0; j < MR; ++j) {
            const int r = r0 + wr0 + 32 * j + l31;
            if (r < RF) {
#pragma unroll
                for (int q = 0; q < 16; ++q) {
                    const int co = co0 + wm0 + 32 * i + acc_row(q, half);
                    out[(size_t)co * RVT + r] = acc[i][j][q];
                }
            }
        }
    if (want_bias && half == 0) {
#pragma unroll
        for (int i = 0; i < MC; ++i)
            slab[(size_t)S * wslab + (size_t)s * Cout + co0 + wm0 + 32 * i + l31] = bsum[i];
    }
#ifdef ECG_STAMP
    asm volatile("s_waitcnt vmcnt(0)" ::: "memory");
#endif
    ECG_STAMP_AT(g_stamps, 4);
}

__global__ __launch_bounds__(64) void wgrad_ffa_reduce_kernel(const float *__restrict__ slab, float *__restrict__ dw,
                                                              float *__restrict__ db, int Cin, int Cout, int S) {
    const int lane = threadIdx.x;
    const size_t i = (size_t)blockIdx.x * 64 + lane;
    const size_t npair = (size_t)Cout * Cin * 8, RVT = (size_t)Cin * 23, wslab = (size_t)Cout * RVT;
    const bool live = i < npair + Cout && (i < npair || db);
    double a[4] = {0.0, 0.0, 0.0, 0.0};
    int j = 0;
    size_t o = 0;
    if (live) {
        if (i < npair) {
            const int co = (int)(i / ((size_t)Cin * 8)), rem = (int)(i - (size_t)co * Cin * 8);
            const int ci = rem >> 3;
            j = rem & 7;
            o = ((size_t)co * Cin + ci) * 15 + 2 * j;
            const int jv = j < 7 ? j : 6;
            const float *pu = slab + (size_t)co * RVT + ci * 8 + j;
            const float *pg = slab + (size_t)co * RVT + Cin * 15 + ci * 8 + j;
            const float *pv = slab + (size_t)co * RVT + Cin * 8 + ci * 7 + jv;
            const int g1 = j < 7 ? 1 : 0;
            int s = 0;
            for (; s + 3 < S; s += 4) {
                float v[4][4];
#pragma unroll
                for (int u = 0; u < 4; ++u) {
                    const size_t off = (size_t)(s + u) * wslab;
                    v[u][0] = pu[off]; v[u][1] = pg[off]; v[u][2] = pv[off]; v[u][3] = pg[off + g1];
                }
#pragma unroll
                for (int u = 0; u < 4; ++u)
#pragma unroll
                    for (int e = 0; e < 4; ++e) a[e] += (double)v[u][e];
            }
            for (; s < S; ++s) {
                const size_t off = (size_t)s * wslab;
                a[0] += (double)pu[off]; a[1] += (double)pg[off]; a[2] += (double)pv[off]; a[3] += (double)pg[off + g1];
            }
        } else {
            const float *src = slab + (size_t)S * wslab + (i - npair);
            for (int s = 0; s < S; ++s) a[0] += (double)src[(size_t)s * Cout];
        }
    }
    if (live) {
        if (i < npair) {
            dw[o] = (float)(a[0] - a[1]);
            if (j < 7) dw[o + 1] = (float)(a[2] + a[3]);
        } else db[i - npair] = (float)a[0];
    }
}

int wgrad_reduce(const float *ws, float *dw, float *db, size_t wslab, int Cout, int S,
                 hipStream_t st);

struct WgCfg { int m_t, r_t, splits; };

#ifndef ECG_WG_SLOTS
#define ECG_WG_SLOTS 512
#endif
#ifndef ECG_WG_TT128
#define ECG_WG_TT128 1
#endif

static WgCfg wgrad_cfg(int N, int Cin, int Cout, int Lo, bool dma, int tt = 64) {
    const int R = Cin * kKM;
    constexpr int slots = ECG_WG_SLOTS;
    WgCfg c;
    if (Cout % 128 == 0) c = {128, 128, 0};
    else if (Cout % 64 == 0) c = {64, 128, 0};
    else c = {32, 192, 0};
    const int tiles = cdiv(R, c.r_t) * (Cout / c.m_t);
    int s = slots / tiles;
    const long long cap = dma ? (long long)N * cdiv(Lo, tt) : N;
    if (s > cap) s = (int)cap;
    if (s < 1) s = 1;
    c.splits = s;
    return c;
}

static bool wgrad_ffa_ok(int Cin, int Cout, bool dma) { return dma && Cout % 128 == 0 && Cin >= 128; }
static int wgrad_ffa_tiles(int Cin, int Cout) { return (2 * cdiv(Cin * 8, 128) + cdiv(Cin * 7, 128)) * (Cout / 128); }
static int wgrad_ffa_splits(int N, int Cin, int Cout, int Lo) {
    long long s = ECG_WG_SLOTS / wgrad_ffa_tiles(Cin, Cout);
    const long long cap = (long long)N * cdiv(Lo, 64);
    if (s > cap) s = cap;
    if (s < 1) s = 1;
    return (int)s;
}

bool mfma_wgrad_dma_supported(int Cin, int Cout, int K);
int mfma_multiplies_per_pair(int op, int Cin, int Cout, int K, int pad) {
    if (op == 2) return (K == kKM && wgrad_ffa_ok(Cin, Cout, mfma_wgrad_dma_supported(Cin, Cout, K))) ? 23 : 2 * K;
    const bool mfma = op == 1 ? mfma_fwd_supported(Cout, Cin, K, K - 1 - pad) : mfma_fwd_supported(Cin, Cout, K, pad);
    return mfma ? 23 : 2 * K;
}

bool mfma_wgrad_supported(int Cin, int Cout, int K, int pad) {
    (void)pad; (void)Cin;
    return K == kKM && Cout % 32 == 0;
}

size_t mfma_wgrad_ws_floats(int N, int Cin, int Cout, int L, int K, int pad) {
    const int Lo = L + 2 * pad - K + 1;
    const WgCfg a = wgrad_cfg(N, Cin, Cout, Lo, false), b = wgrad_cfg(N, Cin, Cout, Lo, true);
    size_t need = (size_t)(a.splits > b.splits ? a.splits : b.splits) * ((size_t)Cout * Cin * K + Cout);
    if (wgrad_ffa_ok(Cin, Cout, true)) {
        const size_t ffa = (size_t)wgrad_ffa_splits(N, Cin, Cout, Lo) * ((size_t)Cout * Cin * 23 + Cout);
        if (ffa > need) need = ffa;
    }
    return need;
}

bool mfma_wgrad_dma_supported(int Cin, int Cout, int K) {
    (void)Cin;
    return K == kKM && Cout % 32 == 0;
}

int mfma_wgrad(const float *dy, int ldy, const float *x, float *dw, float *db, float *ws, int N,
               int Cin, int Cout, int L, int K, int pad, hipStream_t st) {
    const int Lo = L + 2 * pad - K + 1;
    const int R = Cin * K;
    const bool dma = mfma_wgrad_dma_supported(Cin, Cout, K) && ldy % 64 == 0 && ldy >= cdiv(Lo, 64) * 64 &&
                     (reinterpret_cast<uintptr_t>(dy) & 15) == 0;
    const bool tt128 = ECG_WG_TT128 && dma && Cout % 128 != 0 && ldy % 128 == 0 && ldy >= cdiv(Lo, 128) * 128;
    if (wgrad_ffa_ok(Cin, Cout, dma)) {
        const int S = wgrad_ffa_splits(N, Cin, Cout, Lo);
        dim3 fgrid((unsigned)(wgrad_ffa_tiles(Cin, Cout) * S)), fblock(256);
        hipLaunchKernelGGL((conv1d_mfma_wgrad_ffa_kernel<128, 128, 2, 2, 64>), fgrid, fblock, 0, st, dy, x, ws, N, Cin, Cout, L, Lo,
                           ldy, pad, S);
        int frc = check_launch("conv1d_mfma_wgrad_ffa_kernel");
        if (frc) return frc;
        const size_t nout = (size_t)Cout * Cin * 8 + Cout;
        const dim3 rgrid((unsigned)cdiv(nout, (size_t)64));
        hipLaunchKernelGGL(wgrad_ffa_reduce_kernel, rgrid, dim3(64), 0, st, ws, dw, db, Cin, Cout, S);
        return check_launch("wgrad_ffa_reduce_kernel");
    }
    const WgCfg c = wgrad_cfg(N, Cin, Cout, Lo, dma, tt128 ? 128 : 64);
    dim3 grid((unsigned)(cdiv(R, c.r_t) * (Cout / c.m_t) * c.splits)), block(256);
#define ECG_WG(KERNEL) \
    hipLaunchKernelGGL(KERNEL, grid, block, 0, st, dy, x, ws, N, Cin, Cout, L, Lo, ldy, pad, c.splits)
    if (dma && c.m_t == 128) ECG_WG((conv1d_mfma_wgrad_dma_kernel<128, 128, 2, 2, 1, kKM>));
    else if (tt128 && c.m_t == 64) ECG_WG((conv1d_mfma_wgrad_dma_kernel<64, 128, 2, 2, 1, kKM, 128>));
    else if (tt128) ECG_WG((conv1d_mfma_wgrad_dma_kernel<32, 192, 1, 2, 2, kKM, 128>));
    else if (dma && c.m_t == 64) ECG_WG((conv1d_mfma_wgrad_dma_kernel<64, 128, 2, 2, 1, kKM>));
    else if (dma) ECG_WG((conv1d_mfma_wgrad_dma_kernel<32, 192, 1, 2, 2, kKM>));
    else if (c.m_t == 128) ECG_WG((conv1d_mfma_wgrad_kernel<128, 128, 2, 2, 1, 64, kKM>));
    else if (c.m_t == 64) ECG_WG((conv1d_mfma_wgrad_kernel<64, 128, 2, 2, 1, 64, kKM>));
    else ECG_WG((conv1d_mfma_wgrad_kernel<32, 192, 1, 2, 2, 128, kKM>));
#undef ECG_WG
    int rc = check_launch("conv1d_mfma_wgrad_kernel");
    if (rc) return rc;
    return wgrad_reduce(ws, dw, db, (size_t)Cout * R, Cout, c.splits, st);
}

}

#ifdef ECG_STAMP
extern "C" __attribute__((visibility("default"))) int ecg_debug_set_stamp_buffer(unsigned long long *buf) {
    return (int)hipMemcpyToSymbol(HIP_SYMBOL(ecg::g_stamps), &buf, sizeof(buf));
}
#endif
```

ptbxl-multimodal_amd/ecg_hip/_lib.py:

```python
import ctypes
import functools
import os
import threading

import torch

_HERE = os.path.dirname(os.path.abspath(__file__))
LIB_PATH = os.environ.get("ECG_HIP_LIB") or os.path.join(os.path.dirname(_HERE), "lib", "libecg_hip.so")

_vp, _i, _f, _sz, _ll = ctypes.c_void_p, ctypes.c_int, ctypes.c_float, ctypes.c_size_t, ctypes.c_longlong

SIGNATURES = {
    "ecg_version": (_i, []),
    "ecg_last_error": (ctypes.c_char_p, []),
    "ecg_check_device": (_i, []),
    "ecg_conv1d_pack_weights": (_i, [_vp, _vp, _vp, _i, _i, _i, _vp]),
    "ecg_pack_weights_grouped": (_i, [_vp, _vp, _vp, _vp, _vp, _vp, _i, _vp]),
    "ecg_bn_relu_pool_bwd_one_launch_splits": (_i, [_i, _i, _i, _i]),
    "ecg_bn_relu_pool_bwd_one_launch_counter_uints": (_sz, [_i, _i, _i, _i]),
    "ecg_bn_relu_pool_bwd_one_launch": (_i, [_vp] * 7 + [_i] + [_vp] * 3 + [_i] * 6 + [_vp]),
    "ecg_pack_weights_grouped_mixed": (_i, [_vp, _vp, _vp, _vp, _vp, _vp, _vp, _vp, _i, _vp]),
    "ecg_conv1d_fwd_stat_partials": (_i, [_i, _i, _i, _i, _i, _i]),
    "ecg_conv1d_fwd": (_i, [_vp, _vp, _vp, _vp, _vp, _i, _i, _i, _i, _i, _i, _vp]),
    "ecg_conv1d_bwd_data": (_i, [_vp, _vp, _vp, _i, _i, _i, _i, _i, _i, _vp]),
    "ecg_conv1d_bwd_weight_ws_floats": (_sz, [_i, _i, _i, _i, _i, _i]),
    "ecg_conv1d_bwd_weight_bias": (_i, [_vp, _vp, _vp, _vp, _vp, _i, _i, _i, _i, _i, _i, _vp]),
    "ecg_conv1d_dy_row_stride": (_i, [_i] * 7),
    "ecg_conv1d_multiplies_per_output_pair": (_i, [_i] * 5),
    "ecg_conv1d_bwd_data_ld": (_i, [_vp, _i, _vp, _vp, _i, _i, _i, _i, _i, _i, _vp]),
    "ecg_conv1d_bwd_weight_bias_ld": (_i, [_vp, _i, _vp, _vp, _vp, _vp, _i, _i, _i, _i, _i, _i, _vp]),
    "ecg_conv1d_bf16_supported": (_i, [_i, _i, _i, _i]),
    "ecg_conv1d_bf16_packed_elems": (_sz, [_i, _i, _i]),
    "ecg_conv1d_pack_weights_bf16": (_i, [_vp, _vp, _vp, _i, _i, _i, _vp]),
    "ecg_conv1d_fwd_bf16_yh": (_i, [_vp, _i, _i, _vp, _vp, _vp, _i, _vp] + [_i] * 6 + [_vp]),
    "ecg_conv1d_fwd_bf16_yh_stat_partials": (_i, [_i] * 9),
    "ecg_conv1d_bf16_ring_tile": (_i, [_i] * 8),
    "ecg_bn_stats_relu_pool_fwd_h": (_i, [_vp, _i, _ll, _vp, _vp, _vp, _f, _f, _vp, _i, _vp, _vp, _vp, _vp, _vp, _i, _i, _i, _i, _vp]),
    "ecg_bn_relu_pool_bwd_h": (_i, [_vp, _i, _vp, _i, _i] + [_vp] * 5 + [_i] + [_vp] * 3 + [_i] * 4 + [_vp]),
    "ecg_conv1d_bwd_data_bf16hh": (_i, [_vp, _i, _vp, _vp, _i] + [_i] * 6 + [_vp]),
    "ecg_conv1d_bf16_tk_supported": (_i, [_i] * 4),
    "ecg_conv1d_bf16_tk_dy_stride": (_i, [_i]),
    "ecg_conv1d_bwd_weight_bf16_ncl_ws_floats": (_sz, [_i] * 6),
    "ecg_conv1d_bwd_weight_bias_bf16_ncl": (_i, [_vp, _i, _vp, _i, _i, _vp, _vp, _vp] + [_i] * 6 + [_vp]),
    "ecg_bn_stat_partials_count": (_i, [_i, _i, _i]),
    "ecg_bn_stat_partials": (_i, [_vp, _vp, _i, _i, _i, _vp]),
    "ecg_bn_finalize": (_i, [_vp, _i, _ll, _vp, _vp, _vp, _vp, _vp, _i, _f, _f, _vp]),
    "ecg_bn_invstd": (_i, [_vp, _vp, _i, _f, _vp]),
    "ecg_bn_relu_pool_fwd": (_i, [_vp, _vp, _vp, _vp, _vp, _vp, _i, _i, _i, _vp]),
    "ecg_bn_stats_relu_pool_fwd": (_i, [_vp, _i, _ll, _vp, _vp, _vp, _f, _f] + [_vp] * 6 + [_i] * 4 + [_vp]),
    "ecg_bn_stats_relu_pool_gap_fwd_yh": (_i, [_vp, _i, _ll, _vp, _vp, _vp, _f, _f, _vp, _i] + [_vp] * 5 + [_i] * 3 + [_vp]),
    "ecg_bn_relu_pool_bwd_ws_floats": (_sz, [_i, _i, _i]),
    "ecg_bn_relu_pool_bwd": (_i, [_vp] * 10 + [_i, _i, _i, _i, _vp]),
    "ecg_bn_relu_pool_bwd_ld": (_i, [_vp] * 7 + [_i] + [_vp] * 3 + [_i, _i, _i, _i, _vp]),
    "ecg_conv1d_bn_relu_pool_eval_supported": (_i, [_i, _i, _i, _i]),
    "ecg_conv1d_bn_relu_pool_eval_fwd": (_i, [_vp] * 7 + [_f, _vp, _i, _i, _i, _i, _i, _i, _vp]),
    "ecg_conv1d_bn_relu_pool_gap_eval_supported": (_i, [_i] * 5),
    "ecg_conv1d_bn_relu_pool_gap_eval_fwd": (_i, [_vp] * 7 + [_f, _vp, _i, _i, _i, _i, _i, _i, _vp]),
    "ecg_conv1d_bn_relu_pool_eval_bf16_supported": (_i, [_i] * 6),
    "ecg_conv1d_bn_relu_pool_eval_fwd_bf16": (_i, [_vp, _i, _i] + [_vp] * 6 + [_f, _vp, _i, _i] + [_i] * 6 + [_vp]),
    "ecg_conv1d_bn_relu_pool_gap_eval_fwd_bf16": (_i, [_vp, _i, _i] + [_vp] * 6 + [_f, _vp] + [_i] * 6 + [_vp]),
    "ecg_bn_relu_pool_gap_fwd": (_i, [_vp, _vp, _vp, _vp, _vp, _vp, _i, _i, _i, _vp]),
    "ecg_bn_relu_pool_gap_bwd": (_i, [_vp] * 10 + [_i, _i, _i, _i, _vp]),
    "ecg_bn_relu_pool_gap_bwd_ld": (_i, [_vp] * 7 + [_i] + [_vp] * 3 + [_i, _i, _i, _i, _vp]),
    "ecg_gradcam_supported": (_i, [_i] * 4),
    "ecg_gradcam_ws_floats": (_sz, [_i] * 5),
    "ecg_gradcam_fwd": (_i, [_vp, _i, _vp, _vp, _vp, _ll] + [_vp] * 5 + [_i] * 6 + [_vp]),
    "ecg_bn_apply_fwd": (_i, [_vp] * 6 + [_i, _i, _i, _vp]),
    "ecg_bn_bwd_ws_floats": (_sz, [_i, _i, _i]),
    "ecg_bn_bwd": (_i, [_vp] * 9 + [_i, _i, _i, _i, _vp]),
    "ecg_relu_fwd": (_i, [_vp, _vp, _sz, _vp]),
    "ecg_relu_bwd": (_i, [_vp, _vp, _vp, _sz, _vp]),
    "ecg_maxpool2_fwd": (_i, [_vp, _vp, _i, _i, _vp]),
    "ecg_maxpool2_bwd": (_i, [_vp, _vp, _vp, _i, _i, _vp]),
    "ecg_gap_fwd": (_i, [_vp, _vp, _i, _i, _vp]),
    "ecg_gap_bwd": (_i, [_vp, _vp, _i, _i, _vp]),
    "ecg_linear_fwd": (_i, [_vp, _vp, _vp, _vp, _i, _i, _i, _i, _vp]),
    "ecg_linear_bwd_ws_floats": (_sz, [_i, _i, _i]),
    "ecg_linear_bwd": (_i, [_vp] * 8 + [_i, _i, _i, _i, _vp]),
    "ecg_film_fwd": (_i, [_vp, _vp, _vp, _i, _i, _vp]),
    "ecg_film_bwd": (_i, [_vp] * 5 + [_i, _i, _vp]),
    "ecg_bce_logits_fwd": (_i, [_vp, _vp, _vp, _vp, _i, _vp, ctypes.c_double, _vp]),
    "ecg_sigmoid_fwd": (_i, [_vp, _vp, _sz, _vp]),
    "ecg_transpose": (_i, [_vp, _vp, _i, _i, _vp]),
    "ecg_tail_fwd": (_i, [_vp] * 18 + [_i] * 7 + [_vp]),
    "ecg_tail_bwd_chain": (_i, [_vp] * 18 + [_i] * 8 + [_vp]),
    "ecg_linear_wgrad_grouped": (_i, [_vp, _vp, _vp, _vp, _vp, _vp, _i, _i, _vp]),
    "ecg_adamw_step": (_i, [_vp, _vp, _vp, _vp, _sz, _i, _f, _f, _f, _f, _f, _f, _vp]),
    "ecg_adamw_step_graph": (_i, [_vp, _vp, _vp, _vp, _sz, _vp, _f, _f, _f, _f, _f, _f, _vp]),
    "ecg_wfdb16_physical": (_i, [_vp, _vp, _vp, _vp, _i, _i, _i, _vp]),
    "ecg_wfdb16_zscore": (_i, [_vp, _vp, _vp, _vp, _vp, _i, _i, _i, _vp]),
    "ecg_zscore_rows": (_i, [_vp, _vp, _vp, _i, _i, _vp]),
    "ecg_host_gather_rows": (_i, [_vp, _sz, _vp, _i, _vp]),
}

_lock = threading.Lock()
_lib = None


class EcgHipError(RuntimeError):
    pass


def load():
    global _lib
    if _lib is not None:
        return _lib
    with _lock:
        if _lib is None:
            if not os.path.exists(LIB_PATH):
                raise EcgHipError(
                    f"{LIB_PATH} is missing: build it with `python -c 'import __graft_entry__ as g; g.build()'` "
                    "(or `make -C ptbxl-multimodal_amd/csrc`). CUDA tensors have no fallback path.")
            lib = ctypes.CDLL(LIB_PATH)
            for name, (res, args) in SIGNATURES.items():
                fn = getattr(lib, name)
                fn.restype, fn.argtypes = res, args
            _lib = lib
    return _lib


def last_error():
    return load().ecg_last_error().decode("utf-8", "replace")


_raw_stream = getattr(torch._C, "_cuda_getCurrentRawStream", None)
_raw_device = getattr(torch._C, "_cuda_getDevice", None)


def stream():
    if _raw_stream is not None and _raw_device is not None:
        return _raw_stream(_raw_device())
    return torch.cuda.current_stream().cuda_stream


def ptr(t):
    if t is None:
        return None
    if t.is_cuda and t.is_contiguous():
        return t.data_ptr()
    if not t.is_cuda:
        raise EcgHipError("a CPU tensor reached a HIP kernel wrapper: ecg_hip.functional's Functions take CUDA(HIP) "
                          "tensors only (the nn modules route CPU inputs to stock torch before getting here)")
    raise EcgHipError("ecg_hip kernels need contiguous tensors")


_F32 = torch.float32


def f32(t):
    if t is None:
        return None
    if t.dtype is _F32 and t.is_cuda and t.is_contiguous():
        return t.data_ptr()
    if t.dtype != torch.float32:
        raise EcgHipError(f"ecg_hip kernels compute in float32; got {t.dtype}")
    return ptr(t)


_events = None


def call(name, *args):
    lib = load()
    if _events is None:
        rc = getattr(lib, name)(*args)
    else:
        e0, e1 = torch.cuda.Event(enable_timing=True), torch.cuda.Event(enable_timing=True)
        e0.record()
        rc = getattr(lib, name)(*args)
        e1.record()
        _events.append((name, tuple(a for a in args[:-1] if isinstance(a, int) and abs(a) < (1 << 31)), e0, e1))
    if rc != 0:
        raise EcgHipError(f"{name} failed (code {rc}): {last_error()}")


class kernel_timing:

    def __enter__(self):
        global _events
        _events = []
        self.result = {}
        return self

    def __exit__(self, *exc):
        global _events
        ev, _events = _events, None
        torch.cuda.synchronize()
        for name, sig, e0, e1 in ev:
            self.result.setdefault((name, sig), []).append(e0.elapsed_time(e1))
        return False


def ptr_table(tensors, any_dtype=False):
    arr = (ctypes.c_void_p * len(tensors))(*[(ptr if any_dtype else f32)(t) for t in tensors])
    return arr


def int_table(values):
    return (ctypes.c_int * len(values))(*[int(v) for v in values])


@functools.lru_cache(maxsize=4096)
def query(name, *args):
    return getattr(load(), name)(*args)
```

ptbxl-multimodal_amd/ecg_hip/functional.py:

```python
import torch

from . import _lib as L
from . import eval_bf16 as _EB

_call, _query, _f32, _st = L.call, L.query, L.f32, L.stream


def _empty(ref, *shape):
    return torch.empty(shape, dtype=torch.float32, device=ref.device)


import weakref as _weakref

_grad_sinks = {}


def register_grad_sinks(params, views):
    for p, v in zip(params, views):
        _grad_sinks[p.data_ptr()] = (_weakref.ref(p), v)


def unregister_grad_sinks(keys):
    for k in keys:
        _grad_sinks.pop(k, None)


_sinks_handed = set()


def _forget_handed_sinks():
    _sinks_handed.clear()


def _grad_out(key, ref, *shape):
    ent = _grad_sinks.get(key) if key is not None else None
    if ent is not None and key not in _sinks_handed:
        p, v = ent[0](), ent[1]
        if p is not None and p.grad is None and v.device == ref.device and v.numel() == _numel(shape):
            try:
                if not _sinks_handed:
                    torch.autograd.Variable._execution_engine.queue_callback(_forget_handed_sinks)
                _sinks_handed.add(key)
            except RuntimeError:
                return torch.empty(shape, dtype=torch.float32, device=ref.device)
            return v.view(shape)
    return torch.empty(shape, dtype=torch.float32, device=ref.device)


import os as _os

_bn_one_launch = (_os.environ.get("ECG_BN_BWD_RESIDENT", "1") != "0"
                  and _os.environ.get("ECG_HIP_REHEARSE_ON_ONE_GPU") != "1")
_bn_spin_polls = int(_os.environ.get("ECG_BN_BWD_RESIDENT_SPIN", "-1"))
_backward_collectives = {}
_collectives_by_ptr = None
_bn_counters = {}


def set_bn_backward_one_launch(on, spin_polls=None):
    global _bn_one_launch, _bn_spin_polls
    prev, _bn_one_launch = _bn_one_launch, bool(on)
    if spin_polls is not None:
        _bn_spin_polls = int(spin_polls)
    return prev


def declare_backward_collectives(params, busy, owner=None):
    global _collectives_by_ptr
    for p in params:
        k = p if isinstance(p, int) else id(p)
        if busy is None:
            ent = _backward_collectives.get(k)
            if ent is not None and (owner is None or ent[2] == owner):
                del _backward_collectives[k]
        elif not isinstance(p, int):
            _backward_collectives[k] = (_weakref.ref(p), bool(busy), owner)
    _collectives_by_ptr = None


def parameters_rehomed():
    global _collectives_by_ptr
    _collectives_by_ptr = None


def _multi_rank():
    d = torch.distributed
    return d.is_available() and d.is_initialized() and d.get_world_size() > 1


def bn_backward_one_launch_allowed(key):
    global _collectives_by_ptr
    if not _bn_one_launch:
        return False
    if _collectives_by_ptr is None:
        tab = {}
        for k, (ref, busy, _owner) in list(_backward_collectives.items()):
            p = ref()
            if p is None:
                del _backward_collectives[k]
            else:
                tab[p.data_ptr()] = busy
        _collectives_by_ptr = tab
    busy = _collectives_by_ptr.get(key)
    return (not _multi_rank()) if busy is None else (not busy)


def _bn_bwd_counters(ref, n_uints):
    if torch.cuda.is_current_stream_capturing():
        return torch.zeros(n_uints, dtype=torch.int32, device=ref.device)
    key = (ref.device.index, _st())
    t = _bn_counters.get(key)
    if t is None or t.numel() < n_uints:
        t = torch.zeros(max(n_uints, 4352), dtype=torch.int32, device=ref.device)
        _bn_counters[key] = t
    return t


def _numel(shape):
    n = 1
    for d in shape:
        n *= int(d)
    return n


def _key(t):
    return None if t is None else t.data_ptr()


def _contig(t):
    return t if t.is_contiguous() else t.contiguous()


def conv1d_pack(w, need_bwd=True):
    Co, Ci, K = w.shape
    w_fwd = torch.empty_like(w).view(K, Ci, Co)
    w_bwd = torch.empty_like(w).view(K, Co, Ci) if need_bwd else None
    _call("ecg_conv1d_pack_weights", _f32(w), _f32(w_fwd), _f32(w_bwd), Co, Ci, K, _st())
    return w_fwd, w_bwd


_conv_precision = _os.environ.get("ECG_HIP_CONV_PRECISION", "fp32")


def set_conv_precision(mode):
    global _conv_precision
    if mode not in ("fp32", "bf16"):
        raise ValueError("conv precision must be 'fp32' or 'bf16'")
    _conv_precision = mode


def get_conv_precision():
    return _conv_precision


class conv_precision:

    def __init__(self, mode):
        self.mode = mode

    def __enter__(self):
        self.prev = get_conv_precision()
        set_conv_precision(self.mode)

    def __exit__(self, *exc):
        set_conv_precision(self.prev)
        return False


_inference_precision = _os.environ.get("ECG_HIP_INFERENCE_PRECISION", "fp32")


def set_inference_precision(mode):
    global _inference_precision
    if mode not in ("fp32", "bf16"):
        raise ValueError("inference precision must be 'fp32' or 'bf16'")
    _inference_precision = mode


def get_inference_precision():
    return _inference_precision


class inference_precision(conv_precision):

    def __enter__(self):
        self.prev = get_inference_precision()
        set_inference_precision(self.mode)

    def __exit__(self, *exc):
        set_inference_precision(self.prev)
        return False


def conv1d_pack_bf16(w, need_bwd=True):
    Co, Ci, K = w.shape
    nf = _query("ecg_conv1d_bf16_packed_elems", Ci, Co, K)
    wb_fwd = torch.empty(nf, dtype=torch.bfloat16, device=w.device)
    wb_bwd = None
    if need_bwd:
        wb_bwd = torch.empty(_query("ecg_conv1d_bf16_packed_elems", Co, Ci, K), dtype=torch.bfloat16, device=w.device)
    _call("ecg_conv1d_pack_weights_bf16", _f32(w), L.ptr(wb_fwd), L.ptr(wb_bwd), Co, Ci, K, _st())
    return wb_fwd, wb_bwd


class WeightPacker:

    def __init__(self):
        self._key = None

    def __deepcopy__(self, memo):
        return WeightPacker()

    def __getstate__(self):
        return {}

    def __setstate__(self, state):
        self._key = None

    def pack(self, convs, linears, need_bwd):
        srcs = [c.weight for c in convs] + [l.weight for l in linears]
        mixed = _conv_precision == "bf16" and bool(need_bwd)
        infer = _inference_precision == "bf16" and not need_bwd
        key = (need_bwd, mixed, infer) + tuple((w.data_ptr(), tuple(w.shape)) for w in srcs)
        if key != self._key:
            self._key = key
            self.conv_packs, self.linear_T, fw, bw, hf, hb, co, ci, kk = [], [], [], [], [], [], [], [], []
            for i, c in enumerate(convs):
                w = _contig(c.weight)
                Co, Ci, K = w.shape
                want_bwd = need_bwd and i > 0
                if (mixed and _bf16_block_ok(Ci, Co, K, c.padding[0], 16, want_bwd)) or (infer and _EB.packable(Ci, Co, K,
                                                                                                    c.padding[0])):
                    wf = wb = None
                    hwf = torch.empty(_query("ecg_conv1d_bf16_packed_elems", Ci, Co, K), dtype=torch.bfloat16, device=w.device)
                    hwb = (torch.empty(_query("ecg_conv1d_bf16_packed_elems", Co, Ci, K), dtype=torch.bfloat16,
                                       device=w.device) if want_bwd else None)
                    self.conv_packs.append((None, None, hwf, hwb))
                else:
                    hwf = hwb = None
                    wf = torch.empty_like(w).view(K, Ci, Co)
                    wb = torch.empty_like(w).view(K, Co, Ci) if want_bwd else None
                    self.conv_packs.append((wf, wb))
                fw.append(wf); bw.append(wb); hf.append(hwf); hb.append(hwb); co.append(Co); ci.append(Ci); kk.append(K)
            for l in linears:
                w = _contig(l.weight)
                wt = torch.empty(w.shape[1], w.shape[0], dtype=w.dtype, device=w.device)
                self.linear_T.append(wt)
                fw.append(wt); bw.append(None); hf.append(None); hb.append(None)
                co.append(w.shape[0]); ci.append(w.shape[1]); kk.append(1)
            self._mixed = any(t is not None for t in hf)
            tabs = [L.ptr_table([_contig(w) for w in srcs]), L.ptr_table(fw), L.ptr_table(bw)]
            if self._mixed:
                tabs += [L.ptr_table(hf, any_dtype=True), L.ptr_table(hb, any_dtype=True)]
            self._tables = tuple(tabs) + (L.int_table(co), L.int_table(ci), L.int_table(kk), len(srcs))
        _call("ecg_pack_weights_grouped_mixed" if self._mixed else "ecg_pack_weights_grouped", *self._tables, _st())
        return self.conv_packs, self.linear_T


def conv1d_forward_raw(x, w_fwd, bias, Co, K, pad, want_stats):
    N, Ci, Lin = x.shape
    Lo = Lin + 2 * pad - K + 1
    if Lo <= 0:
        raise L.EcgHipError(f"conv1d: empty output for L={Lin}, K={K}, pad={pad}")
    y = _empty(x, N, Co, Lo)
    partials, P = None, 0
    if want_stats:
        P = _query("ecg_conv1d_fwd_stat_partials", N, Ci, Co, Lin, K, pad)
        partials = _empty(x, Co * P * 2)
    _call("ecg_conv1d_fwd", _f32(x), _f32(w_fwd), _f32(bias), _f32(y), _f32(partials),
          N, Ci, Co, Lin, K, pad, _st())
    return y, partials, P


def conv1d_backward_raw(x, dy, w_shape, w_bwd, pad, need_dx, need_db=True, ldy=None, sink_keys=(None, None)):
    N, Ci, Lin = x.shape
    Co, _, K = w_shape
    if ldy is None:
        ldy = Lin + 2 * pad - K + 1
    dw = _grad_out(sink_keys[0], x, Co, Ci, K)
    db = _grad_out(sink_keys[1], x, Co) if need_db else None
    ws = _empty(x, max(1, _query("ecg_conv1d_bwd_weight_ws_floats", N, Ci, Co, Lin, K, pad)))
    _call("ecg_conv1d_bwd_weight_bias_ld", _f32(dy), ldy, _f32(x), _f32(dw), _f32(db), _f32(ws), N, Ci, Co, Lin, K, pad,
          _st())
    dx = None
    if need_dx:
        dx = torch.empty_like(x)
        _call("ecg_conv1d_bwd_data_ld", _f32(dy), ldy, _f32(w_bwd), _f32(dx), N, Ci, Co, Lin, K, pad, _st())
    return dx, dw, db


def bn_batch_stats(y, partials, P, running_mean, running_var, nbt, momentum, eps):
    N, C, Lo = y.shape
    if partials is None:
        P = _query("ecg_bn_stat_partials_count", N, C, Lo)
        partials = _empty(y, C * P * 2)
        _call("ecg_bn_stat_partials", _f32(y), _f32(partials), N, C, Lo, _st())
    mean, invstd = _empty(y, C), _empty(y, C)
    if nbt is not None and nbt.dtype != torch.int64:
        raise L.EcgHipError("num_batches_tracked must be int64")
    _call("ecg_bn_finalize", _f32(partials), P, N * Lo, _f32(mean), _f32(invstd),
          _f32(running_mean), _f32(running_var), L.ptr(nbt), C, float(momentum), float(eps), _st())
    return mean, invstd


def bn_eval_stats(running_mean, running_var, eps):
    invstd = torch.empty_like(running_var)
    _call("ecg_bn_invstd", _f32(running_var), _f32(invstd), running_var.numel(), float(eps), _st())
    return running_mean, invstd


def _bn_momentum(momentum, nbt):
    if momentum is None:
        return 1.0 / (int(nbt.item()) + 1) if nbt is not None else 0.0
    return float(momentum)


def _bf16_block_ok(Ci, Co, K, pad, Lin, need_dx):
    if K > 15:
        return False
    sup = _query("ecg_conv1d_bf16_supported", Ci, Co, K, pad)
    return bool((sup & 1) and (sup & 4) and (not need_dx or (sup & 2)) and Lin + 2 * pad - K + 1 >= 2)


_EVAL, _FP32, _BF16, _EVAL_BF16 = "eval", "fp32", "bf16", "eval_bf16"


class ConvBlockFn(torch.autograd.Function):

    @staticmethod
    def forward(ctx, x, w, b, gamma, beta, running_mean, running_var, nbt, training, momentum,
                eps, pad, gap=False, packed=None, grad_enabled=True, x_len=None, next_bf16=False):
        x, w = _contig(x), _contig(w)
        Co, Ci, K = w.shape
        x_h = x.dtype == torch.bfloat16
        use_batch = training or running_mean is None
        need_grad = grad_enabled and any(ctx.needs_input_grad)
        need_dx = bool(need_grad and ctx.needs_input_grad[0])
        Lin = x_len if x_h else x.shape[2]
        Lo = Lin + 2 * pad - K + 1
        if Lo <= 0:
            raise L.EcgHipError(f"conv1d: empty output for L={Lin}, K={K}, pad={pad}")
        mode = _FP32
        if _conv_precision == "bf16" and use_batch and need_grad and _bf16_block_ok(Ci, Co, K, pad, Lin, need_dx):
            mode = _BF16
        elif not use_batch and not need_grad:
            mode = _EVAL
            if _inference_precision == "bf16" and _EB.takes(x, Ci, Co, K, pad, Lin, gap):
                mode = _EVAL_BF16
        if x_h and mode not in (_BF16, _EVAL_BF16):
            raise L.EcgHipError("ConvBlock: input arrived as a bf16 activation but this block does not take the mixed-"
                                "precision form (conv precision / BatchNorm mode changed between blocks?)")
        ctx.mode, ctx.pad, ctx.gap, ctx.batch_stats, ctx.Lin, ctx.Lo = mode, pad, gap, use_batch, Lin, Lo
        ctx.sink_keys = (_key(w), _key(b), _key(gamma), _key(beta))
        if mode == _EVAL_BF16:
            wb, _ = ConvBlockFn._weights(w, packed, True, False)
            return _EB.forward(x, wb, w.shape, b, gamma, beta, running_mean, running_var, eps, pad, gap, Lin, next_bf16)
        if mode == _EVAL:
            p = ConvBlockFn._fwd_eval(x, w, b, gamma, beta, running_mean, running_var, eps, pad, gap, packed)
            if p is not None:
                return p
            ctx.mode = mode = _FP32
        if mode == _BF16:
            return ConvBlockFn._fwd_bf16(ctx, x, w, b, gamma, beta, running_mean, running_var, nbt, training, momentum, eps,
                                         packed, need_dx, next_bf16)
        return ConvBlockFn._fwd_fp32(ctx, x, w, b, gamma, beta, running_mean, running_var, nbt, training, momentum, eps,
                                     packed, need_grad, need_dx)

    @staticmethod
    def _weights(w, packed, bf16, need_bwd):
        if bf16:
            if packed is not None and len(packed) == 4 and packed[2] is not None and (packed[3] is not None or not need_bwd):
                return packed[2], packed[3]
            return conv1d_pack_bf16(w, need_bwd=need_bwd)
        if packed is not None and packed[0] is not None and (packed[1] is not None or not need_bwd):
            return packed[0], packed[1]
        return conv1d_pack(w, need_bwd=need_bwd)

    @staticmethod
    def _fwd_eval(x, w, b, gamma, beta, running_mean, running_var, eps, pad, gap, packed):
        N, Ci, Lin = x.shape
        Co, _, K = w.shape
        Lo = Lin + 2 * pad - K + 1
        if not gap and _query("ecg_conv1d_bn_relu_pool_eval_supported", Ci, Co, K, pad):
            w_fwd, _ = ConvBlockFn._weights(w, packed, False, False)
            p = _empty(x, N, Co, Lo // 2)
            _call("ecg_conv1d_bn_relu_pool_eval_fwd", _f32(x), _f32(w_fwd), _f32(b), _f32(gamma), _f32(beta),
                  _f32(running_mean), _f32(running_var), float(eps), _f32(p), N, Ci, Co, Lin, K, pad, _st())
            return p
        if gap and _query("ecg_conv1d_bn_relu_pool_gap_eval_supported", Ci, Co, Lin, K, pad):
            w_fwd, _ = ConvBlockFn._weights(w, packed, False, False)
            g = _empty(x, N, Co)
            _call("ecg_conv1d_bn_relu_pool_gap_eval_fwd", _f32(x), _f32(w_fwd), _f32(b), _f32(gamma), _f32(beta),
                  _f32(running_mean), _f32(running_var), float(eps), _f32(g), N, Ci, Co, Lin, K, pad, _st())
            return g
        return None

    @staticmethod
    def _fwd_fp32(ctx, x, w, b, gamma, beta, running_mean, running_var, nbt, training, momentum, eps, packed, need_grad,
                  need_dx):
        N, Ci, Lin = x.shape
        Co, _, K = w.shape
        pad, gap, use_batch, Lo = ctx.pad, ctx.gap, ctx.batch_stats, ctx.Lo
        w_fwd, w_bwd = ConvBlockFn._weights(w, packed, False, need_dx)
        y, partials, P = conv1d_forward_raw(x, w_fwd, b, Co, K, pad, want_stats=use_batch)
        p = _empty(x, N, Co) if gap else _empty(x, N, Co, Lo // 2)
        if use_batch:
            rm, rv, cnt = (running_mean, running_var, nbt) if training else (None, None, None)
            if cnt is not None and cnt.dtype != torch.int64:
                raise L.EcgHipError("num_batches_tracked must be int64")
            mean, invstd = _empty(x, Co), _empty(x, Co)
            _call("ecg_bn_stats_relu_pool_fwd", _f32(partials), P, N * Lo, _f32(rm), _f32(rv), L.ptr(cnt),
                  _bn_momentum(momentum, nbt), float(eps), _f32(y), _f32(gamma), _f32(beta), _f32(mean), _f32(invstd),
                  _f32(p), N, Co, Lo, 1 if gap else 0, _st())
        else:
            mean, invstd = bn_eval_stats(running_mean, running_var, eps)
            _call("ecg_bn_relu_pool_gap_fwd" if gap else "ecg_bn_relu_pool_fwd", _f32(y), _f32(gamma), _f32(beta),
                  _f32(mean), _f32(invstd), _f32(p), N, Co, Lo, _st())
        ctx.save_for_backward(x, w, y, gamma, beta, mean, invstd)
        ctx.w_bwd = w_bwd
        return p

    @staticmethod
    def _bwd_fp32(ctx, dp):
        x, w, y, gamma, beta, mean, invstd = ctx.saved_tensors
        N, Co, Lo = y.shape
        if dp is None:
            dp = torch.zeros(N, Co, *(() if ctx.gap else (Lo // 2,)), device=y.device)
        dp = _contig(dp)
        Ci, Lin, K = x.shape[1], x.shape[2], w.shape[2]
        need_dx = ctx.needs_input_grad[0]
        kw, kb, kg, kbe = ctx.sink_keys
        dgamma, dbeta = _grad_out(kg, y, Co), _grad_out(kbe, y, Co)
        ldy = _query("ecg_conv1d_dy_row_stride", N, Ci, Co, Lin, K, ctx.pad, int(bool(need_dx)))
        dy = _empty(y, N, Co, ldy)
        if bn_backward_one_launch_allowed(kw) and _query("ecg_bn_relu_pool_bwd_one_launch_splits", N, Co, Lo, ldy):
            n_u = _query("ecg_bn_relu_pool_bwd_one_launch_counter_uints", N, Co, Lo, ldy)
            cnt = _bn_bwd_counters(y, n_u) if n_u else None
            _call("ecg_bn_relu_pool_bwd_one_launch", _f32(y), _f32(dp), _f32(gamma), _f32(beta), _f32(mean),
                  _f32(invstd), _f32(dy), ldy, _f32(dgamma), _f32(dbeta), L.ptr(cnt), N, Co, Lo,
                  1 if ctx.batch_stats else 0, 1 if ctx.gap else 0, _bn_spin_polls, _st())
        else:
            ws = _empty(y, _query("ecg_bn_relu_pool_bwd_ws_floats", N, Co, Lo))
            _call("ecg_bn_relu_pool_gap_bwd_ld" if ctx.gap else "ecg_bn_relu_pool_bwd_ld", _f32(y), _f32(dp),
                  _f32(gamma), _f32(beta), _f32(mean), _f32(invstd), _f32(dy), ldy, _f32(dgamma),
                  _f32(dbeta), _f32(ws), N, Co, Lo, 1 if ctx.batch_stats else 0, _st())
        dx, dw, db = conv1d_backward_raw(x, dy, w.shape, ctx.w_bwd, ctx.pad, need_dx, ldy=ldy, sink_keys=(kw, kb))
        return dx, dw, db, dgamma, dbeta

    @staticmethod
    def _fwd_bf16(ctx, x, w, b, gamma, beta, running_mean, running_var, nbt, training, momentum, eps, packed, need_dx,
                  next_bf16):
        N, Ci = x.shape[0], x.shape[1]
        Co, _, K = w.shape
        pad, gap, Lin, Lo = ctx.pad, ctx.gap, ctx.Lin, ctx.Lo
        x_h = x.dtype == torch.bfloat16
        ctx.x_cast = False
        if not x_h and (need_dx or Lin % 8 != 0 or x.data_ptr() % 16 != 0):
            xh = torch.zeros(N, Ci, (Lin + 7) & ~7, dtype=torch.bfloat16, device=x.device)
            xh[:, :, :Lin].copy_(x)
            x, x_h, ctx.x_cast = xh, True, True
        ldx = x.shape[2] if x_h else 0
        w_fwd, w_bwd = ConvBlockFn._weights(w, packed, True, need_dx)
        ldyh = (Lo + 7) & ~7
        y = torch.empty(N, Co, ldyh, dtype=torch.bfloat16, device=x.device)
        P = _query("ecg_conv1d_fwd_bf16_yh_stat_partials", N, Ci, Co, Lin, K, pad, 1 if x_h else 0, ldx, ldyh)
        partials = _empty(x, Co * P * 2)
        _call("ecg_conv1d_fwd_bf16_yh", L.ptr(x), 1 if x_h else 0, ldx, L.ptr(w_fwd), _f32(b), L.ptr(y), ldyh,
              _f32(partials), N, Ci, Co, Lin, K, pad, _st())
        rm, rv, cnt = (running_mean, running_var, nbt) if training else (None, None, None)
        if cnt is not None and cnt.dtype != torch.int64:
            raise L.EcgHipError("num_batches_tracked must be int64")
        mean, invstd = _empty(x, Co), _empty(x, Co)
        ldp = 0
        if gap:
            p = _empty(x, N, Co)
            _call("ecg_bn_stats_relu_pool_gap_fwd_yh", _f32(partials), P, N * Lo, _f32(rm), _f32(rv), L.ptr(cnt),
                  _bn_momentum(momentum, nbt), float(eps), L.ptr(y), ldyh, _f32(gamma), _f32(beta), _f32(mean), _f32(invstd),
                  _f32(p), N, Co, Lo, _st())
        else:
            ldp = (Lo // 2 + 7) & ~7
            p = torch.empty(N, Co, ldp, dtype=torch.bfloat16, device=x.device)
            _call("ecg_bn_stats_relu_pool_fwd_h", _f32(partials), P, N * Lo, _f32(rm), _f32(rv), L.ptr(cnt),
                  _bn_momentum(momentum, nbt), float(eps), L.ptr(y), ldyh, _f32(gamma), _f32(beta), _f32(mean),
                  _f32(invstd), L.ptr(p), ldp, N, Co, Lo, _st())
            if not next_bf16:
                p, ldp = p[:, :, :Lo // 2].float(), 0
        ctx.save_for_backward(x, w, y, gamma, beta, mean, invstd)
        ctx.w_bwd, ctx.ldyh, ctx.ldp = w_bwd, ldyh, ldp
        ctx.set_materialize_grads(False)
        return p

    @staticmethod
    def _bwd_bf16(ctx, dp):
        x, w, y, gamma, beta, mean, invstd = ctx.saved_tensors
        N, Co, Lo, Lin = y.shape[0], y.shape[1], ctx.Lo, ctx.Lin
        if dp is None:
            dp = (torch.zeros(N, Co, ctx.ldp, dtype=torch.bfloat16, device=y.device) if ctx.ldp else
                  torch.zeros(N, Co, *(() if ctx.gap else (Lo // 2,)), device=y.device))
        dp = _contig(dp)
        if ctx.ldp and (dp.dtype != torch.bfloat16 or dp.shape[2] != ctx.ldp):
            raise L.EcgHipError("ConvBlock backward: the gradient of a bf16 activation must be bf16 of the same shape")
        Ci, K = x.shape[1], w.shape[2]
        x_h = x.dtype == torch.bfloat16
        need_dx = ctx.needs_input_grad[0]
        kw, kb, kg, kbe = ctx.sink_keys
        dgamma, dbeta = _grad_out(kg, y, Co), _grad_out(kbe, y, Co)
        ws = _empty(y, _query("ecg_bn_relu_pool_bwd_ws_floats", N, Co, Lo))
        ldt = _query("ecg_conv1d_bf16_tk_dy_stride", Lo)
        dyh = torch.empty(N, Co, ldt, dtype=torch.bfloat16, device=y.device)
        dp_kind, dp_ld = (1, 0) if ctx.gap else ((0, ctx.ldp) if ctx.ldp else (2, Lo // 2))
        _call("ecg_bn_relu_pool_bwd_h", L.ptr(y), ctx.ldyh, L.ptr(dp), dp_kind, dp_ld, _f32(gamma), _f32(beta), _f32(mean),
              _f32(invstd), L.ptr(dyh), ldt, _f32(dgamma), _f32(dbeta), _f32(ws), N, Co, Lo, 1, _st())
        dw, db = _grad_out(kw, x, Co, Ci, K), _grad_out(kb, x, Co)
        ws2 = _empty(y, max(1, _query("ecg_conv1d_bwd_weight_bf16_ncl_ws_floats", N, Ci, Co, Lin, K, ctx.pad)))
        _call("ecg_conv1d_bwd_weight_bias_bf16_ncl", L.ptr(dyh), ldt, L.ptr(x), 1 if x_h else 0, x.shape[2], _f32(dw),
              _f32(db), _f32(ws2), N, Ci, Co, Lin, K, ctx.pad, _st())
        dx = None
        if need_dx:
            dx = torch.empty_like(x)
            _call("ecg_conv1d_bwd_data_bf16hh", L.ptr(dyh), ldt, L.ptr(ctx.w_bwd), L.ptr(dx), x.shape[2], N, Ci, Co,
                  Lin, K, ctx.pad, _st())
            if ctx.x_cast:
                dx = dx[:, :, :Lin].float()
        return dx, dw, db, dgamma, dbeta

    @staticmethod
    def backward(ctx, dp):
        grads = ConvBlockFn._bwd_bf16(ctx, dp) if ctx.mode == _BF16 else ConvBlockFn._bwd_fp32(ctx, dp)
        return grads + (None,) * 12


class BceWithLogitsFn(torch.autograd.Function):

    @staticmethod
    def forward(ctx, logits, target, running, weight):
        logits, target = _contig(logits), _contig(target)
        if logits.shape != target.shape:
            raise ValueError(f"Target size ({tuple(target.shape)}) must be the same as input size ({tuple(logits.shape)})")
        if running is not None and (running.dtype != torch.float64 or running.numel() != 1):
            raise L.EcgHipError("running loss accumulator must be a float64 scalar tensor")
        loss = _empty(logits, 1)
        dx = torch.empty_like(logits) if ctx.needs_input_grad[0] else None
        _call("ecg_bce_logits_fwd", _f32(logits), _f32(target), _f32(loss), _f32(dx), logits.numel(),
              L.ptr(running), float(weight), _st())
        ctx.save_for_backward(dx)
        return loss.view(())

    @staticmethod
    def backward(ctx, dloss):
        (dx,) = ctx.saved_tensors
        one = _unit_grads.get(dloss.device)
        if one is not None and dloss.data_ptr() == one.data_ptr():
            return dx, None, None, None
        return dx * dloss, None, None, None


_unit_grads = {}


def backward_from_loss(loss):
    one = _unit_grads.get(loss.device)
    if one is None:
        one = _unit_grads[loss.device] = torch.ones((), dtype=loss.dtype, device=loss.device)
    _sinks_handed.clear()
    loss.backward(one)


def conv_block(x, conv, bn, gap=False, packed=None):
    return conv_block_chain(x, conv, bn, gap, packed)[0]


def conv_block_chain(x, conv, bn, gap=False, packed=None, carry=None, next_conv=None, next_bn=None, next_gap=False):
    nxt = False
    if next_conv is not None and not gap:
        x_len = carry if x.dtype == torch.bfloat16 else x.shape[2]
        Lo = x_len + 2 * conv.padding[0] - conv.kernel_size[0] + 1
        nK, npad = next_conv.kernel_size[0], next_conv.padding[0]
        if _conv_precision == "bf16":
            nxt = bool(next_bn is not None and (next_bn.training or next_bn.running_mean is None)
                       and torch.is_grad_enabled()
                       and _bf16_block_ok(conv.out_channels, next_conv.out_channels, nK, npad, Lo // 2, True))
        if not nxt and _inference_precision == "bf16" and not torch.is_grad_enabled():
            nxt = bool(not (bn.training or bn.running_mean is None) and next_bn is not None
                       and not (next_bn.training or next_bn.running_mean is None)
                       and _EB.takes(x, conv.in_channels, conv.out_channels, conv.kernel_size[0], conv.padding[0], x_len,
                                     False)
                       and _EB.covered(conv.out_channels, next_conv.out_channels, nK, npad, Lo // 2, next_gap, True))
    p = ConvBlockFn.apply(x, conv.weight, conv.bias, bn.weight, bn.bias, bn.running_mean, bn.running_var,
                          bn.num_batches_tracked, bn.training, bn.momentum, bn.eps, conv.padding[0], gap, packed,
                          torch.is_grad_enabled(), carry, nxt)
    if p.dtype == torch.bfloat16:
        x_len = carry if x.dtype == torch.bfloat16 else x.shape[2]
        return p, (x_len + 2 * conv.padding[0] - conv.kernel_size[0] + 1) // 2
    return p, None


class TailFn(torch.autograd.Function):

    @staticmethod
    def forward(ctx, g, xd, Wp, bp, W0, b0, W2, b2, Wf, bf, Wh, bh, WpT=None, WfT=None):
        g = _contig(g)
        M, F0 = g.shape
        F, C = Wp.shape[0], Wh.shape[0]
        demo = xd is not None
        if WpT is None:
            WpT = _empty(g, F0, F)
            _call("ecg_transpose", _f32(_contig(Wp)), _f32(WpT), F, F0, _st())
        z, logits = _empty(g, M, F), _empty(g, M, C)
        D = H1 = H = 0
        xdc = h1 = h2 = film = zc = None
        if demo:
            xdc = _contig(xd)
            D, H1, H = xdc.shape[1], W0.shape[0], W2.shape[0]
            if WfT is None:
                WfT = _empty(g, H, 2 * F)
                _call("ecg_transpose", _f32(_contig(Wf)), _f32(WfT), 2 * F, H, _st())
            h1, h2, film, zc = _empty(g, M, H1), _empty(g, M, H), _empty(g, M, 2 * F), _empty(g, M, F)
        _call("ecg_tail_fwd", _f32(g), _f32(xdc), _f32(WpT), _f32(bp), _f32(W0), _f32(b0), _f32(W2),
              _f32(b2), _f32(WfT), _f32(bf), _f32(_contig(Wh)), _f32(bh), _f32(z), _f32(h1), _f32(h2),
              _f32(film), _f32(zc), _f32(logits), M, F0, F, D, H1, H, C, _st())
        ctx.save_for_backward(g, xdc, Wp, W0, W2, Wf, Wh, z, h1, h2, film, zc)
        ctx.dims = (M, F0, F, D, H1, H, C, demo)
        ctx.sink_keys = tuple(_key(t) for t in (Wp, bp, W0, b0, W2, b2, Wf, bf, Wh, bh))
        ctx.set_materialize_grads(False)
        return logits, z

    @staticmethod
    def backward(ctx, dlogits, dz_extra):
        g, xd, Wp, W0, W2, Wf, Wh, z, h1, h2, film, zc = ctx.saved_tensors
        M, F0, F, D, H1, H, C, demo = ctx.dims
        if dlogits is None:
            dlogits = torch.zeros(M, C, dtype=torch.float32, device=g.device)
        dlogits = _contig(dlogits)
        dz, dg = _empty(g, M, F), _empty(g, M, F0)
        dzc = dfilm = dh2m = dh1m = dxd = None
        if demo:
            dzc, dfilm = _empty(g, M, F), _empty(g, M, 2 * F)
            dh2m, dh1m = _empty(g, M, H), _empty(g, M, H1)
            if ctx.needs_input_grad[1]:
                dxd = _empty(g, M, D)
        dze = None if dz_extra is None else _contig(dz_extra)
        _call("ecg_tail_bwd_chain", _f32(dlogits), _f32(dze), _f32(z), _f32(h1), _f32(h2), _f32(film),
              _f32(Wp), _f32(W0), _f32(W2), _f32(Wf), _f32(Wh), _f32(dzc), _f32(dz), _f32(dfilm),
              _f32(dh2m), _f32(dh1m), _f32(dg), _f32(dxd), M, F0, F, D, H1, H, C, int(demo), _st())
        k = ctx.sink_keys
        dWp, dbp = _grad_out(k[0], g, *Wp.shape), _grad_out(k[1], g, F)
        dWh, dbh = _grad_out(k[8], g, *Wh.shape), _grad_out(k[9], g, C)
        if demo:
            dW0, db0 = _grad_out(k[2], g, *W0.shape), _grad_out(k[3], g, H1)
            dW2, db2 = _grad_out(k[4], g, *W2.shape), _grad_out(k[5], g, H)
            dWf, dbf = _grad_out(k[6], g, *Wf.shape), _grad_out(k[7], g, 2 * F)
            Gs, Xs = [dz, dfilm, dh2m, dh1m, dlogits], [g, h2, h1, xd, zc]
            dWs, dbs = [dWp, dWf, dW2, dW0, dWh], [dbp, dbf, db2, db0, dbh]
        else:
            dW0 = db0 = dW2 = db2 = dWf = dbf = None
            Gs, Xs, dWs, dbs = [dz, dlogits], [g, z], [dWp, dWh], [dbp, dbh]
        _call("ecg_linear_wgrad_grouped", L.ptr_table(Gs), L.ptr_table(Xs), L.ptr_table(dWs),
              L.ptr_table(dbs), L.int_table([w.shape[0] for w in dWs]),
              L.int_table([w.shape[1] for w in dWs]), len(Gs), M, _st())
        return dg, dxd, dWp, dbp, dW0, db0, dW2, db2, dWf, dbf, dWh, dbh, None, None


def tail(g, x_demo, proj, head, mlp0=None, mlp2=None, film_gen=None, transposed=None):
    WpT = transposed[0] if transposed else None
    if x_demo is None:
        return TailFn.apply(g, None, proj.weight, proj.bias, None, None, None, None, None, None,
                            head.weight, head.bias, WpT, None)
    WfT = transposed[1] if transposed else None
    return TailFn.apply(g, x_demo, proj.weight, proj.bias, mlp0.weight, mlp0.bias, mlp2.weight,
                        mlp2.bias, film_gen.weight, film_gen.bias, head.weight, head.bias, WpT, WfT)


def film(z, film_raw):
    if not z.is_cuda:
        gamma, beta = film_raw.chunk(2, dim=-1)
        return (1.0 + torch.tanh(gamma)) * z + beta
    return FilmFn.apply(z, film_raw)


def binary_cross_entropy_with_logits(logits, target, running=None, weight=1.0):
    if not logits.is_cuda:
        loss = torch.nn.functional.binary_cross_entropy_with_logits(logits, target)
        if running is not None:
            running += loss.detach().double() * weight
        return loss
    return BceWithLogitsFn.apply(logits, target, running, weight)


def sigmoid(x):
    if not x.is_cuda:
        return torch.sigmoid(x.detach())
    x = _contig(x.detach())
    out = torch.empty_like(x)
    _call("ecg_sigmoid_fwd", _f32(x), _f32(out), x.numel(), _st())
    return out


def zscore_per_lead(x, out=None, return_stats=False):
    x = _contig(x)
    T = x.shape[-1]
    rows = x.numel() // T
    if out is None:
        out = torch.empty_like(x)
    stats = _empty(x, rows, 2)
    _call("ecg_zscore_rows", _f32(x), _f32(out), _f32(stats), rows, T, _st())
    return (out, stats) if return_stats else out


def wfdb16_to_windows(d, gain, baseline, normalize=True, return_stats=False):
    if d.dtype != torch.int16 or gain.dtype != torch.float64 or baseline.dtype != torch.int32:
        raise L.EcgHipError("wfdb16_to_windows: d must be int16, gain float64, baseline int32")
    d, gain, baseline = _contig(d), _contig(gain), _contig(baseline)
    B, T, leads = d.shape
    if tuple(gain.shape) != (B, leads) or tuple(baseline.shape) != (B, leads):
        raise L.EcgHipError("wfdb16_to_windows: gain/baseline must be [B, leads]")
    x = torch.empty(B, leads, T, dtype=torch.float32, device=d.device)
    if not normalize:
        _call("ecg_wfdb16_physical", L.ptr(d), L.ptr(gain), L.ptr(baseline), _f32(x), B, T, leads, _st())
        return x
    stats = _empty(x, B * leads, 2)
    _call("ecg_wfdb16_zscore", L.ptr(d), L.ptr(gain), L.ptr(baseline), _f32(x), _f32(stats), B, T, leads, _st())
    return (x, stats) if return_stats else x


from .leaves import BatchNormFn, Conv1dFn, FilmFn, GapFn, LinearFn, MaxPool2Fn, ReLUFn
```

Before: 181,600 windows/s.

## Fold weight-gradient slab reduction into the data-gradient conv launch as rider blocks

Splits the weight-gradient path so the partial-slab kernel runs first and the final cross-split reduction runs as extra rider workgroups appended to the data-gradient MFMA conv grid. This removes one separate reduce kernel launch per conv layer and lets the reduction overlap with the input-gradient convolution. A new C API entry and Python dispatch use this fused path for fp32 when event timing is off. The cost is more template variants and LDS reuse for the combine step, and the reduce now competes with conv tiles for CUs.

```diff
diff --git a/include/ecg_hip.h b/include/ecg_hip.h
--- a/include/ecg_hip.h
+++ b/include/ecg_hip.h
@@ -50,6 +50,9 @@
 int ecg_conv1d_bwd_weight_bias_ld(const float *dy, int ldy, const float *x, float *dw, float *db,
                                   float *ws, int N, int C_in, int C_out, int L, int K, int pad,
                                   ecg_stream_t stream);
+int ecg_conv1d_bwd_weight_data_ld(const float *dy, int ldy, const float *x, const float *w_bwd,
+                                  float *dw, float *db, float *dx, float *ws, int N, int C_in,
+                                  int C_out, int L, int K, int pad, ecg_stream_t stream);
 
 size_t ecg_conv1d_bwd_weight_ws_floats(int N, int C_in, int C_out, int L, int K, int pad);
 int ecg_conv1d_bwd_weight_bias(const float *dy, const float *x, float *dw, float *db, float *ws,
diff --git a/ptbxl-multimodal_amd/csrc/conv1d_api.hip b/ptbxl-multimodal_amd/csrc/conv1d_api.hip
--- a/ptbxl-multimodal_amd/csrc/conv1d_api.hip
+++ b/ptbxl-multimodal_amd/csrc/conv1d_api.hip
@@ -1,4 +1,5 @@
 #include "common.h"
+#include "wgrad_reduce.h"
 
 namespace ecg {
 int direct_fwd_stat_partials(int N, int Lo);
@@ -7,6 +8,8 @@
 size_t direct_wgrad_ws_floats(int N, int Cin, int Cout, int K);
 int direct_wgrad(const float *dy, const float *x, float *dw, float *db, float *ws, int N, int Cin,
                  int Cout, int L, int K, int pad, hipStream_t st);
+int direct_wgrad_slabs(const float *dy, const float *x, float *dw, float *db, float *ws, int N, int Cin,
+                       int Cout, int L, int K, int pad, hipStream_t st, WgradReduce *red);
 int pack_weights(const float *w, float *w_fwd, float *w_bwd, int Co, int Ci, int K,
                  hipStream_t st);
 int pack_weights_grouped(const float *const *w, float *const *w_fwd, float *const *w_bwd, void *const *wb_fwd,
@@ -25,6 +28,11 @@
 int mfma_multiplies_per_pair(int op, int Cin, int Cout, int K, int pad);
 int mfma_wgrad(const float *dy, int ldy, const float *x, float *dw, float *db, float *ws, int N,
                int Cin, int Cout, int L, int K, int pad, hipStream_t st);
+int mfma_wgrad_slabs(const float *dy, int ldy, const float *x, float *dw, float *db, float *ws, int N,
+                     int Cin, int Cout, int L, int K, int pad, hipStream_t st, WgradReduce *red);
+int mfma_wgrad_reduce(const WgradReduce &red, hipStream_t st);
+int mfma_fwd_rider(const float *x, int ldx, const float *wp, float *y, int N, int Cin, int Cout, int L, int K, int pad,
+                   WgradReduce red, hipStream_t st);
 
 static int check_conv_shape(int N, int Cin, int Cout, int L, int K, int pad) {
     ECG_REQUIRE(N > 0 && Cin > 0 && Cout > 0 && L > 0, "conv1d: N=%d C_in=%d C_out=%d L=%d must be > 0",
@@ -152,6 +160,28 @@
                                          pad, stream);
 }
 
+ECG_API int ecg_conv1d_bwd_weight_data_ld(const float *dy, int ldy, const float *x, const float *w_bwd,
+                                          float *dw, float *db, float *dx, float *ws, int N, int C_in,
+                                          int C_out, int L, int K, int pad, ecg_stream_t stream) {
+    int rc = check_conv_shape(N, C_in, C_out, L, K, pad);
+    if (rc) return rc;
+    ECG_REQUIRE(dy && x && w_bwd && dw && dx && ws, "conv1d_bwd_weight_data: null pointer");
+    const int Lo = L + 2 * pad - K + 1, padb = K - 1 - pad;
+    ECG_REQUIRE(ldy >= Lo, "conv1d_bwd_weight_data: dY row stride %d < row length %d", ldy, Lo);
+    const bool wg_mfma = mfma_wgrad_supported(C_in, C_out, K, pad), dg_mfma = mfma_fwd_supported(C_out, C_in, K, padb);
+    ECG_REQUIRE((wg_mfma && dg_mfma) || ldy == Lo, "conv1d_bwd_weight_data: this shape needs dense dY rows (stride %d != %d); "
+                "use the stride ecg_conv1d_dy_row_stride returns", ldy, Lo);
+    hipStream_t st = as_stream(stream);
+    WgradReduce red;
+    rc = wg_mfma ? mfma_wgrad_slabs(dy, ldy, x, dw, db, ws, N, C_in, C_out, L, K, pad, st, &red)
+                 : direct_wgrad_slabs(dy, x, dw, db, ws, N, C_in, C_out, L, K, pad, st, &red);
+    if (rc) return rc;
+    if (dg_mfma) return mfma_fwd_rider(dy, ldy, w_bwd, dx, N, C_out, C_in, Lo, K, padb, red, st);
+    rc = mfma_wgrad_reduce(red, st);
+    if (rc) return rc;
+    return direct_fwd(dy, w_bwd, nullptr, dx, nullptr, N, C_out, C_in, Lo, K, padb, st);
+}
+
 ECG_API int ecg_conv1d_bn_relu_pool_eval_supported(int C_in, int C_out, int K, int pad) {
     return mfma_fwd_supported(C_in, C_out, K, pad) ? 1 : 0;
 }
diff --git a/ptbxl-multimodal_amd/csrc/conv1d_direct.hip b/ptbxl-multimodal_amd/csrc/conv1d_direct.hip
--- a/ptbxl-multimodal_amd/csrc/conv1d_direct.hip
+++ b/ptbxl-multimodal_amd/csrc/conv1d_direct.hip
@@ -1,4 +1,5 @@
 #include "common.h"
+#include "wgrad_reduce.h"
 #include <cstdlib>
 
 namespace ecg {
@@ -232,20 +233,9 @@
     __shared__ double part[G][64];
     const int lane = threadIdx.x & 63, w = threadIdx.x >> 6;
     const size_t i = (size_t)blockIdx.x * 64 + lane;
-    const size_t total = wslab + Cout;
-    const bool live = i < total && (i < wslab || db);
+    const bool live = wgrad_reduce_live(i, wslab, Cout, db);
     double a = 0.0;
-    if (live) {
-        const float *src = i < wslab ? slab + i : slab + (size_t)S * wslab + (i - wslab);
-        const size_t stride = i < wslab ? wslab : (size_t)Cout;
-        int s = w;
-        for (; s + 3 * G < S; s += 4 * G) {
-            const float v0 = src[(size_t)s * stride], v1 = src[(size_t)(s + G) * stride];
-            const float v2 = src[(size_t)(s + 2 * G) * stride], v3 = src[(size_t)(s + 3 * G) * stride];
-            a += (double)v0; a += (double)v1; a += (double)v2; a += (double)v3;
-        }
-        for (; s < S; s += G) a += (double)src[(size_t)s * stride];
-    }
+    if (live) a = wgrad_reduce_part(slab, wslab, Cout, S, i, w, G);
     if (G > 1) {
         part[w][lane] = a;
         __syncthreads();
@@ -253,9 +243,7 @@
 #pragma unroll
         for (int g = 1; g < G; ++g) a += part[g][lane];
     }
-    if (live) {
-        if (i < wslab) dw[i] = (float)a; else db[i - wslab] = (float)a;
-    }
+    if (live) wgrad_reduce_store(dw, db, wslab, i, a);
 }
 
 template <int G>
@@ -264,37 +252,9 @@
     __shared__ double part[G][64][4];
     const int lane = threadIdx.x & 63, w = threadIdx.x >> 6;
     const size_t i = ((size_t)blockIdx.x * 64 + lane) * 4;
-    const size_t total = wslab + Cout;
-    const bool live = i < total && (i < wslab || db);
+    const bool live = wgrad_reduce_live(i, wslab, Cout, db);
     double a[4] = {0.0, 0.0, 0.0, 0.0};
-    if (live) {
-        const float *src = i < wslab ? slab + i : slab + (size_t)S * wslab + (i - wslab);
-        const size_t stride = i < wslab ? wslab : (size_t)Cout;
-        int s = w;
-        for (; s + 7 * G < S; s += 8 * G) {
-            float4 v[8];
-#pragma unroll
-            for (int u = 0; u < 8; ++u) v[u] = *reinterpret_cast<const float4 *>(src + (size_t)(s + u * G) * stride);
-#pragma unroll
-            for (int u = 0; u < 8; ++u) {
-                a[0] += (double)v[u].x; a[1] += (double)v[u].y; a[2] += (double)v[u].z; a[3] += (double)v[u].w;
-            }
-        }
-        for (; s + 3 * G < S; s += 4 * G) {
-            const float4 v0 = *reinterpret_cast<const float4 *>(src + (size_t)s * stride);
-            const float4 v1 = *reinterpret_cast<const float4 *>(src + (size_t)(s + G) * stride);
-            const float4 v2 = *reinterpret_cast<const float4 *>(src + (size_t)(s + 2 * G) * stride);
-            const float4 v3 = *reinterpret_cast<const float4 *>(src + (size_t)(s + 3 * G) * stride);
-            a[0] += (double)v0.x; a[0] += (double)v1.x; a[0] += (double)v2.x; a[0] += (double)v3.x;
-            a[1] += (double)v0.y; a[1] += (double)v1.y; a[1] += (double)v2.y; a[1] += (double)v3.y;
-            a[2] += (double)v0.z; a[2] += (double)v1.z; a[2] += (double)v2.z; a[2] += (double)v3.z;
-            a[3] += (double)v0.w; a[3] += (double)v1.w; a[3] += (double)v2.w; a[3] += (double)v3.w;
-        }
-        for (; s < S; s += G) {
-            const float4 v = *reinterpret_cast<const float4 *>(src + (size_t)s * stride);
-            a[0] += (double)v.x; a[1] += (double)v.y; a[2] += (double)v.z; a[3] += (double)v.w;
-        }
-    }
+    if (live) wgrad_reduce4_part(slab, wslab, Cout, S, i, w, G, a);
     if (G > 1) {
 #pragma unroll
         for (int e = 0; e < 4; ++e) part[w][lane][e] = a[e];
@@ -305,25 +265,32 @@
 #pragma unroll
             for (int e = 0; e < 4; ++e) a[e] += part[g][lane][e];
     }
-    if (live) {
-        const float4 o = make_float4((float)a[0], (float)a[1], (float)a[2], (float)a[3]);
-        if (i < wslab) *reinterpret_cast<float4 *>(dw + i) = o; else *reinterpret_cast<float4 *>(db + (i - wslab)) = o;
-    }
-}
-
-int wgrad_reduce(const float *ws, float *dw, float *db, size_t wslab, int Cout, int S,
-                 hipStream_t st) {
+    if (live) wgrad_reduce4_store(dw, db, wslab, i, a);
+}
+
+WgradReduce wgrad_reduce_describe(const float *ws, float *dw, float *db, size_t wslab, int Cin, int Cout, int S) {
+    WgradReduce r{ws, dw, db, wslab, Cin, Cout, S, WGR_GROUPED, 1, 0};
     const size_t total = wslab + Cout;
     if (wslab % 4 == 0 && Cout % 4 == 0 && (size_t)cdiv(total, 64) >= 1024 &&
         ((reinterpret_cast<uintptr_t>(ws) | reinterpret_cast<uintptr_t>(dw) | reinterpret_cast<uintptr_t>(db)) & 15) == 0) {
-        hipLaunchKernelGGL((wgrad_reduce4_kernel<1>), dim3(cdiv(total / 4, 64)), dim3(64), 0, st, ws, dw, db, wslab, Cout, S);
+        r.form = WGR_FLOAT4;
+        return r;
+    }
+    const size_t groups = cdiv(total, 64);
+    int G = 1;
+    while (G < 16 && groups * G < 1024 && S / (2 * G) >= 8) G *= 2;
+    r.G = G;
+    return r;
+}
+
+int wgrad_reduce_launch(const WgradReduce &r, hipStream_t st) {
+    const dim3 grid((unsigned)wgrad_reduce_groups(r));
+    if (r.form == WGR_FLOAT4) {
+        hipLaunchKernelGGL((wgrad_reduce4_kernel<1>), grid, dim3(64), 0, st, r.slab, r.dw, r.db, r.stride, r.Cout, r.S);
         return check_launch("wgrad_reduce4_kernel");
     }
-    const dim3 grid(cdiv(total, 64));
-    int G = 1;
-    while (G < 16 && (size_t)grid.x * G < 1024 && S / (2 * G) >= 8) G *= 2;
-#define ECG_RED(GG) hipLaunchKernelGGL((wgrad_reduce_kernel<GG>), grid, dim3(64 * GG), 0, st, ws, dw, db, wslab, Cout, S)
-    switch (G) {
+#define ECG_RED(GG) hipLaunchKernelGGL((wgrad_reduce_kernel<GG>), grid, dim3(64 * GG), 0, st, r.slab, r.dw, r.db, r.stride, r.Cout, r.S)
+    switch (r.G) {
         case 1: ECG_RED(1); break;
         case 2: ECG_RED(2); break;
         case 4: ECG_RED(4); break;
@@ -332,6 +299,11 @@
     }
 #undef ECG_RED
     return check_launch("wgrad_reduce_kernel");
+}
+
+int wgrad_reduce(const float *ws, float *dw, float *db, size_t wslab, int Cout, int S,
+                 hipStream_t st) {
+    return wgrad_reduce_launch(wgrad_reduce_describe(ws, dw, db, wslab, 0, Cout, S), st);
 }
 
 static bool wgrad_fast_ok(int Cout, int K) { return K == 15 && Cout % 8 == 0; }
@@ -350,8 +322,8 @@
     return (size_t)S * ((size_t)Cout * Cin * K + Cout);
 }
 
-int direct_wgrad(const float *dy, const float *x, float *dw, float *db, float *ws, int N, int Cin,
-                 int Cout, int L, int K, int pad, hipStream_t st) {
+int direct_wgrad_slabs(const float *dy, const float *x, float *dw, float *db, float *ws, int N, int Cin,
+                       int Cout, int L, int K, int pad, hipStream_t st, WgradReduce *red) {
     const int Lo = L + 2 * pad - K + 1;
     const int S = direct_wgrad_splits(N, Cin, Cout, K);
     const size_t wslab = (size_t)Cout * Cin * K;
@@ -364,9 +336,16 @@
         hipLaunchKernelGGL(conv1d_wgrad_generic_kernel, grid, block, 0, st, dy, x, ws, N, Cin,
                            Cout, L, Lo, K, pad);
     }
-    int rc = check_launch("conv1d_wgrad kernel");
+    *red = wgrad_reduce_describe(ws, dw, db, wslab, Cin, Cout, S);
+    return check_launch("conv1d_wgrad kernel");
+}
+
+int direct_wgrad(const float *dy, const float *x, float *dw, float *db, float *ws, int N, int Cin,
+                 int Cout, int L, int K, int pad, hipStream_t st) {
+    WgradReduce red;
+    int rc = direct_wgrad_slabs(dy, x, dw, db, ws, N, Cin, Cout, L, K, pad, st, &red);
     if (rc) return rc;
-    return wgrad_reduce(ws, dw, db, wslab, Cout, S, st);
+    return wgrad_reduce_launch(red, st);
 }
 
 int pack_weights(const float *w, float *w_fwd, float *w_bwd, int Co, int Ci, int K, hipStream_t st);
diff --git a/ptbxl-multimodal_amd/csrc/conv1d_mfma.hip b/ptbxl-multimodal_amd/csrc/conv1d_mfma.hip
--- a/ptbxl-multimodal_amd/csrc/conv1d_mfma.hip
+++ b/ptbxl-multimodal_amd/csrc/conv1d_mfma.hip
@@ -1,5 +1,7 @@
 #include "mfma_util.h"
+#include "wgrad_reduce.h"
 #include <cstdlib>
+#include <tuple>
 #include <type_traits>
 
 namespace ecg {
@@ -33,11 +35,14 @@
 #ifndef ECG_FFA_FLP2
 #define ECG_FFA_FLP2 64
 #endif
-template <int CO_T, int M_T, int WCO, int WT, int EPI, int CI_C = 4, int FLP = 1>
+template <int CO_T, int M_T, int WCO, int WT, int EPI, int CI_C = 4, int FLP = 1, class... RD>
 __global__ __launch_bounds__(256, ECG_FFA_MINB) void conv1d_mfma_ffa_kernel(
     const float *__restrict__ x, const float *__restrict__ wp, const float *__restrict__ bias,
     float *__restrict__ y, float *__restrict__ partials, int Cin, int Cout, int L, int ldx, int Lo,
-    int pad, int P, int tiles_t, EvalEpi ev) {
+    int pad, int P, int tiles_t, EvalEpi ev, RD... rdp) {
+    constexpr bool RIDER = sizeof...(RD) != 0;
+    static_assert(!RIDER || (EPI == EPI_PLAIN && sizeof...(RD) == 1 && (std::is_same<RD, WgradReduce>::value && ...)),
+                  "the reduce rides on the input gradient only");
     constexpr bool STATS = (EPI == EPI_STATS), GAP = (EPI == EPI_EVAL_GAP);
     constexpr bool EVALM = (EPI == EPI_EVAL || EPI == EPI_EVAL_GAP);
     static_assert(WCO * WT == 4, "4 waves per workgroup");
@@ -60,11 +65,21 @@
 
     __shared__ __attribute__((aligned(1024))) float lds[2 * IMG];
 
+    int nconv = gridDim.x;
+    if constexpr (RIDER) {
+        static_assert(2 * IMG * sizeof(float) >= 16 * 64 * sizeof(double), "wave combine of the grouped reduce (G <= 16)");
+        const WgradReduce &rd = std::get<0>(std::tie(rdp...));
+        nconv -= rd.riders;
+        if ((int)blockIdx.x >= nconv) {
+            wgrad_reduce_rider(rd, (int)blockIdx.x - nconv, reinterpret_cast<double *>(lds));
+            return;
+        }
+    }
     const int tid = threadIdx.x, lane = tid & 63, wave = tid >> 6;
     const int half = lane >> 5, l31 = lane & 31;
     ECG_STAMP_AT(g_stamps, 0);
     const int CT = Cout / CO_T;
-    const int tile = xcd_chunked(blockIdx.x, gridDim.x);
+    const int tile = xcd_chunked(blockIdx.x, nconv);
     const int tile_co = tile % CT, tile_nt = tile / CT;
     const int tile_t = tile_nt % tiles_t, n = tile_nt / tiles_t;
     const int t0 = tile_t * TS, co0 = tile_co * CO_T;
@@ -307,7 +322,7 @@
 template <int CO_T, int T_T, int WCO, int WT>
 static void launch_fwd(const float *x, const float *wp, const float *bias, float *y,
                        float *partials, const EvalEpi *ev, int N, int Cin, int Cout, int L, int ldx,
-                       int Lo, int pad, hipStream_t st) {
+                       int Lo, int pad, hipStream_t st, const WgradReduce *rider = nullptr) {
     const int tiles_t = cdiv(Lo, T_T - 2);
     dim3 grid((unsigned)((size_t)tiles_t * (Cout / CO_T) * N)), block(256);
     const int P = N * tiles_t;
@@ -319,6 +334,16 @@
     else \
         hipLaunchKernelGGL((conv1d_mfma_ffa_kernel<CO_T, T_T / 2, WCO, WT, MODE>), grid, block, 0, st, x, wp, bias, y, \
                            partials, Cin, Cout, L, ldx, Lo, pad, P, tiles_t, EV); } while (0)
+    if (rider) {
+        const dim3 rgrid(grid.x + (unsigned)rider->riders);
+        if (ECG_FFA_FLP2 && Cin % 8 == 0 && Cin >= ECG_FFA_FLP2)
+            hipLaunchKernelGGL((conv1d_mfma_ffa_kernel<CO_T, T_T / 2, WCO, WT, EPI_PLAIN, 4, 2, WgradReduce>), rgrid, block, 0, st, x,
+                               wp, bias, y, partials, Cin, Cout, L, ldx, Lo, pad, P, tiles_t, none, *rider);
+        else
+            hipLaunchKernelGGL((conv1d_mfma_ffa_kernel<CO_T, T_T / 2, WCO, WT, EPI_PLAIN, 4, 1, WgradReduce>), rgrid, block, 0, st, x,
+                               wp, bias, y, partials, Cin, Cout, L, ldx, Lo, pad, P, tiles_t, none, *rider);
+        return;
+    }
     if (ev && ev->gap) ECG_FFA(EPI_EVAL_GAP, *ev);
     else if (ev) ECG_FFA(EPI_EVAL, *ev);
     else if (partials) ECG_FFA(EPI_STATS, none);
@@ -328,18 +353,25 @@
 
 static int mfma_fwd_any(const float *x, const float *wp, const float *bias, float *y,
                         float *partials, const EvalEpi *ev, int N, int Cin, int Cout, int L, int ldx,
-                        int K, int pad, hipStream_t st) {
+                        int K, int pad, hipStream_t st, const WgradReduce *rider = nullptr) {
     const int Lo = L + 2 * pad - K + 1;
     if (fwd_cfg(Cout).co_t == 64)
-        launch_fwd<64, 128, 2, 2>(x, wp, bias, y, partials, ev, N, Cin, Cout, L, ldx, Lo, pad, st);
+        launch_fwd<64, 128, 2, 2>(x, wp, bias, y, partials, ev, N, Cin, Cout, L, ldx, Lo, pad, st, rider);
     else
-        launch_fwd<32, 256, 1, 4>(x, wp, bias, y, partials, ev, N, Cin, Cout, L, ldx, Lo, pad, st);
+        launch_fwd<32, 256, 1, 4>(x, wp, bias, y, partials, ev, N, Cin, Cout, L, ldx, Lo, pad, st, rider);
     return check_launch("conv1d_mfma_ffa_kernel");
 }
 
 int mfma_fwd(const float *x, int ldx, const float *wp, const float *bias, float *y, float *partials,
              int N, int Cin, int Cout, int L, int K, int pad, hipStream_t st) {
     return mfma_fwd_any(x, wp, bias, y, partials, nullptr, N, Cin, Cout, L, ldx, K, pad, st);
+}
+
+int mfma_fwd_rider(const float *x, int ldx, const float *wp, float *y, int N, int Cin, int Cout, int L, int K, int pad,
+                   WgradReduce red, hipStream_t st) {
+    const size_t groups = wgrad_reduce_groups(red);
+    red.riders = (int)(groups < 1024 ? groups : 1024);
+    return mfma_fwd_any(x, wp, nullptr, y, nullptr, nullptr, N, Cin, Cout, L, ldx, K, pad, st, &red);
 }
 
 int mfma_fwd_eval_pool(const float *x, const float *wp, const float *bias, const float *gamma,
@@ -1129,56 +1161,11 @@
 
 __global__ __launch_bounds__(64) void wgrad_ffa_reduce_kernel(const float *__restrict__ slab, float *__restrict__ dw,
                                                               float *__restrict__ db, int Cin, int Cout, int S) {
-    const int lane = threadIdx.x;
-    const size_t i = (size_t)blockIdx.x * 64 + lane;
-    const size_t npair = (size_t)Cout * Cin * 8, RVT = (size_t)Cin * 23, wslab = (size_t)Cout * RVT;
-    const bool live = i < npair + Cout && (i < npair || db);
-    double a[4] = {0.0, 0.0, 0.0, 0.0};
-    int j = 0;
-    size_t o = 0;
-    if (live) {
-        if (i < npair) {
-            const int co = (int)(i / ((size_t)Cin * 8)), rem = (int)(i - (size_t)co * Cin * 8);
-            const int ci = rem >> 3;
-            j = rem & 7;
-            o = ((size_t)co * Cin + ci) * 15 + 2 * j;
-            const int jv = j < 7 ? j : 6;
-            const float *pu = slab + (size_t)co * RVT + ci * 8 + j;
-            const float *pg = slab + (size_t)co * RVT + Cin * 15 + ci * 8 + j;
-            const float *pv = slab + (size_t)co * RVT + Cin * 8 + ci * 7 + jv;
-            const int g1 = j < 7 ? 1 : 0;
-            int s = 0;
-            for (; s + 3 < S; s += 4) {
-                float v[4][4];
-#pragma unroll
-                for (int u = 0; u < 4; ++u) {
-                    const size_t off = (size_t)(s + u) * wslab;
-                    v[u][0] = pu[off]; v[u][1] = pg[off]; v[u][2] = pv[off]; v[u][3] = pg[off + g1];
-                }
-#pragma unroll
-                for (int u = 0; u < 4; ++u)
-#pragma unroll
-                    for (int e = 0; e < 4; ++e) a[e] += (double)v[u][e];
-            }
-            for (; s < S; ++s) {
-                const size_t off = (size_t)s * wslab;
-                a[0] += (double)pu[off]; a[1] += (double)pg[off]; a[2] += (double)pv[off]; a[3] += (double)pg[off + g1];
-            }
-        } else {
-            const float *src = slab + (size_t)S * wslab + (i - npair);
-            for (int s = 0; s < S; ++s) a[0] += (double)src[(size_t)s * Cout];
-        }
-    }
-    if (live) {
-        if (i < npair) {
-            dw[o] = (float)(a[0] - a[1]);
-            if (j < 7) dw[o + 1] = (float)(a[2] + a[3]);
-        } else db[i - npair] = (float)a[0];
-    }
-}
-
-int wgrad_reduce(const float *ws, float *dw, float *db, size_t wslab, int Cout, int S,
-                 hipStream_t st);
+    wgrad_ffa_reduce_lane(slab, dw, db, Cin, Cout, S, (size_t)blockIdx.x * 64 + threadIdx.x);
+}
+
+WgradReduce wgrad_reduce_describe(const float *ws, float *dw, float *db, size_t wslab, int Cin, int Cout, int S);
+int wgrad_reduce_launch(const WgradReduce &r, hipStream_t st);
 
 struct WgCfg { int m_t, r_t, splits; };
 
@@ -1243,8 +1230,8 @@
     return K == kKM && Cout % 32 == 0;
 }
 
-int mfma_wgrad(const float *dy, int ldy, const float *x, float *dw, float *db, float *ws, int N,
-               int Cin, int Cout, int L, int K, int pad, hipStream_t st) {
+int mfma_wgrad_slabs(const float *dy, int ldy, const float *x, float *dw, float *db, float *ws, int N,
+                     int Cin, int Cout, int L, int K, int pad, hipStream_t st, WgradReduce *red) {
     const int Lo = L + 2 * pad - K + 1;
     const int R = Cin * K;
     const bool dma = mfma_wgrad_dma_supported(Cin, Cout, K) && ldy % 64 == 0 && ldy >= cdiv(Lo, 64) * 64 &&
@@ -1255,12 +1242,8 @@
         dim3 fgrid((unsigned)(wgrad_ffa_tiles(Cin, Cout) * S)), fblock(256);
         hipLaunchKernelGGL((conv1d_mfma_wgrad_ffa_kernel<128, 128, 2, 2, 64>), fgrid, fblock, 0, st, dy, x, ws, N, Cin, Cout, L, Lo,
                            ldy, pad, S);
-        int frc = check_launch("conv1d_mfma_wgrad_ffa_kernel");
-        if (frc) return frc;
-        const size_t nout = (size_t)Cout * Cin * 8 + Cout;
-        const dim3 rgrid((unsigned)cdiv(nout, (size_t)64));
-        hipLaunchKernelGGL(wgrad_ffa_reduce_kernel, rgrid, dim3(64), 0, st, ws, dw, db, Cin, Cout, S);
-        return check_launch("wgrad_ffa_reduce_kernel");
+        *red = WgradReduce{ws, dw, db, (size_t)Cout * Cin * 23, Cin, Cout, S, WGR_FFA, 1, 0};
+        return check_launch("conv1d_mfma_wgrad_ffa_kernel");
     }
     const WgCfg c = wgrad_cfg(N, Cin, Cout, Lo, dma, tt128 ? 128 : 64);
     dim3 grid((unsigned)(cdiv(R, c.r_t) * (Cout / c.m_t) * c.splits)), block(256);
@@ -1275,9 +1258,25 @@
     else if (c.m_t == 64) ECG_WG((conv1d_mfma_wgrad_kernel<64, 128, 2, 2, 1, 64, kKM>));
     else ECG_WG((conv1d_mfma_wgrad_kernel<32, 192, 1, 2, 2, 128, kKM>));
 #undef ECG_WG
-    int rc = check_launch("conv1d_mfma_wgrad_kernel");
+    *red = wgrad_reduce_describe(ws, dw, db, (size_t)Cout * R, Cin, Cout, c.splits);
+    return check_launch("conv1d_mfma_wgrad_kernel");
+}
+
+int mfma_wgrad_reduce(const WgradReduce &red, hipStream_t st) {
+    if (red.form == WGR_FFA) {
+        hipLaunchKernelGGL(wgrad_ffa_reduce_kernel, dim3((unsigned)wgrad_reduce_groups(red)), dim3(64), 0, st, red.slab, red.dw,
+                           red.db, red.Cin, red.Cout, red.S);
+        return check_launch("wgrad_ffa_reduce_kernel");
+    }
+    return wgrad_reduce_launch(red, st);
+}
+
+int mfma_wgrad(const float *dy, int ldy, const float *x, float *dw, float *db, float *ws, int N,
+               int Cin, int Cout, int L, int K, int pad, hipStream_t st) {
+    WgradReduce red;
+    int rc = mfma_wgrad_slabs(dy, ldy, x, dw, db, ws, N, Cin, Cout, L, K, pad, st, &red);
     if (rc) return rc;
-    return wgrad_reduce(ws, dw, db, (size_t)Cout * R, Cout, c.splits, st);
+    return mfma_wgrad_reduce(red, st);
 }
 
 }
diff --git a/ptbxl-multimodal_amd/csrc/wgrad_reduce.h b/ptbxl-multimodal_amd/csrc/wgrad_reduce.h
--- /dev/null
+++ b/ptbxl-multimodal_amd/csrc/wgrad_reduce.h
@@ -0,0 +1,171 @@
+#pragma once
+#include "common.h"
+
+namespace ecg {
+
+enum { WGR_GROUPED = 0, WGR_FLOAT4 = 1, WGR_FFA = 2 };
+
+struct WgradReduce {
+    const float *slab;
+    float *dw, *db;
+    size_t stride;
+    int Cin, Cout, S;
+    int form;
+    int G;
+    int riders;
+};
+
+__host__ __device__ __forceinline__ size_t wgrad_reduce_groups(const WgradReduce &r) {
+    if (r.form == WGR_FFA) return ((size_t)r.Cout * r.Cin * 8 + r.Cout + 63) / 64;
+    const size_t total = r.stride + r.Cout;
+    return ((r.form == WGR_FLOAT4 ? total / 4 : total) + 63) / 64;
+}
+
+__device__ __forceinline__ bool wgrad_reduce_live(size_t i, size_t wslab, int Cout, const float *db) {
+    return i < wslab + Cout && (i < wslab || db);
+}
+
+__device__ __forceinline__ double wgrad_reduce_part(const float *__restrict__ slab, size_t wslab, int Cout, int S, size_t i,
+                                                    int w, int G) {
+    double a = 0.0;
+    const float *src = i < wslab ? slab + i : slab + (size_t)S * wslab + (i - wslab);
+    const size_t stride = i < wslab ? wslab : (size_t)Cout;
+    int s = w;
+    for (; s + 3 * G < S; s += 4 * G) {
+        const float v0 = src[(size_t)s * stride], v1 = src[(size_t)(s + G) * stride];
+        const float v2 = src[(size_t)(s + 2 * G) * stride], v3 = src[(size_t)(s + 3 * G) * stride];
+        a += (double)v0; a += (double)v1; a += (double)v2; a += (double)v3;
+    }
+    for (; s < S; s += G) a += (double)src[(size_t)s * stride];
+    return a;
+}
+
+__device__ __forceinline__ void wgrad_reduce_store(float *__restrict__ dw, float *__restrict__ db, size_t wslab, size_t i,
+                                                   double a) {
+    if (i < wslab) dw[i] = (float)a; else db[i - wslab] = (float)a;
+}
+
+__device__ __forceinline__ void wgrad_reduce4_part(const float *__restrict__ slab, size_t wslab, int Cout, int S, size_t i,
+                                                   int w, int G, double a[4]) {
+    const float *src = i < wslab ? slab + i : slab + (size_t)S * wslab + (i - wslab);
+    const size_t stride = i < wslab ? wslab : (size_t)Cout;
+    int s = w;
+    for (; s + 7 * G < S; s += 8 * G) {
+        float4 v[8];
+#pragma unroll
+        for (int u = 0; u < 8; ++u) v[u] = *reinterpret_cast<const float4 *>(src + (size_t)(s + u * G) * stride);
+#pragma unroll
+        for (int u = 0; u < 8; ++u) {
+            a[0] += (double)v[u].x; a[1] += (double)v[u].y; a[2] += (double)v[u].z; a[3] += (double)v[u].w;
+        }
+    }
+    for (; s + 3 * G < S; s += 4 * G) {
+        const float4 v0 = *reinterpret_cast<const float4 *>(src + (size_t)s * stride);
+        const float4 v1 = *reinterpret_cast<const float4 *>(src + (size_t)(s + G) * stride);
+        const float4 v2 = *reinterpret_cast<const float4 *>(src + (size_t)(s + 2 * G) * stride);
+        const float4 v3 = *reinterpret_cast<const float4 *>(src + (size_t)(s + 3 * G) * stride);
+        a[0] += (double)v0.x; a[0] += (double)v1.x; a[0] += (double)v2.x; a[0] += (double)v3.x;
+        a[1] += (double)v0.y; a[1] += (double)v1.y; a[1] += (double)v2.y; a[1] += (double)v3.y;
+        a[2] += (double)v0.z; a[2] += (double)v1.z; a[2] += (double)v2.z; a[2] += (double)v3.z;
+        a[3] += (double)v0.w; a[3] += (double)v1.w; a[3] += (double)v2.w; a[3] += (double)v3.w;
+    }
+    for (; s < S; s += G) {
+        const float4 v = *reinterpret_cast<const float4 *>(src + (size_t)s * stride);
+        a[0] += (double)v.x; a[1] += (double)v.y; a[2] += (double)v.z; a[3] += (double)v.w;
+    }
+}
+
+__device__ __forceinline__ void wgrad_reduce4_store(float *__restrict__ dw, float *__restrict__ db, size_t wslab, size_t i,
+                                                    const double a[4]) {
+    const float4 o = make_float4((float)a[0], (float)a[1], (float)a[2], (float)a[3]);
+    if (i < wslab) *reinterpret_cast<float4 *>(dw + i) = o; else *reinterpret_cast<float4 *>(db + (i - wslab)) = o;
+}
+
+__device__ __forceinline__ void wgrad_ffa_reduce_lane(const float *__restrict__ slab, float *__restrict__ dw,
+                                                      float *__restrict__ db, int Cin, int Cout, int S, size_t i) {
+    const size_t npair = (size_t)Cout * Cin * 8, RVT = (size_t)Cin * 23, wslab = (size_t)Cout * RVT;
+    const bool live = i < npair + Cout && (i < npair || db);
+    double a[4] = {0.0, 0.0, 0.0, 0.0};
+    int j = 0;
+    size_t o = 0;
+    if (live) {
+        if (i < npair) {
+            const int co = (int)(i / ((size_t)Cin * 8)), rem = (int)(i - (size_t)co * Cin * 8);
+            const int ci = rem >> 3;
+            j = rem & 7;
+            o = ((size_t)co * Cin + ci) * 15 + 2 * j;
+            const int jv = j < 7 ? j : 6;
+            const float *pu = slab + (size_t)co * RVT + ci * 8 + j;
+            const float *pg = slab + (size_t)co * RVT + Cin * 15 + ci * 8 + j;
+            const float *pv = slab + (size_t)co * RVT + Cin * 8 + ci * 7 + jv;
+            const int g1 = j < 7 ? 1 : 0;
+            int s = 0;
+            for (; s + 3 < S; s += 4) {
+                float v[4][4];
+#pragma unroll
+                for (int u = 0; u < 4; ++u) {
+                    const size_t off = (size_t)(s + u) * wslab;
+                    v[u][0] = pu[off]; v[u][1] = pg[off]; v[u][2] = pv[off]; v[u][3] = pg[off + g1];
+                }
+#pragma unroll
+                for (int u = 0; u < 4; ++u)
+#pragma unroll
+                    for (int e = 0; e < 4; ++e) a[e] += (double)v[u][e];
+            }
+            for (; s < S; ++s) {
+                const size_t off = (size_t)s * wslab;
+                a[0] += (double)pu[off]; a[1] += (double)pg[off]; a[2] += (double)pv[off]; a[3] += (double)pg[off + g1];
+            }
+        } else {
+            const float *src = slab + (size_t)S * wslab + (i - npair);
+            for (int s = 0; s < S; ++s) a[0] += (double)src[(size_t)s * Cout];
+        }
+    }
+    if (live) {
+        if (i < npair) {
+            dw[o] = (float)(a[0] - a[1]);
+            if (j < 7) dw[o + 1] = (float)(a[2] + a[3]);
+        } else db[i - npair] = (float)a[0];
+    }
+}
+
+__device__ __forceinline__ void wgrad_reduce_rider(const WgradReduce &r, int rider, double *part) {
+    const int lane = threadIdx.x & 63, wave = threadIdx.x >> 6;
+    const int G = r.form == WGR_GROUPED ? r.G : 1;
+    const int GW = G < 4 ? G : 4, slots = 4 / GW;
+    const int slot = wave / GW, w0 = wave - slot * GW;
+    const size_t groups = wgrad_reduce_groups(r);
+    const size_t per_pass = (size_t)r.riders * slots;
+    for (size_t base = 0; base < groups; base += per_pass) {
+        const size_t g = base + rider + (size_t)r.riders * slot;
+        const bool have = g < groups && slot < slots;
+        if (r.form == WGR_FFA) {
+            if (have) wgrad_ffa_reduce_lane(r.slab, r.dw, r.db, r.Cin, r.Cout, r.S, g * 64 + lane);
+        } else if (r.form == WGR_FLOAT4) {
+            const size_t i = (g * 64 + lane) * 4;
+            if (have && wgrad_reduce_live(i, r.stride, r.Cout, r.db)) {
+                double a[4] = {0.0, 0.0, 0.0, 0.0};
+                wgrad_reduce4_part(r.slab, r.stride, r.Cout, r.S, i, 0, 1, a);
+                wgrad_reduce4_store(r.dw, r.db, r.stride, i, a);
+            }
+        } else {
+            const size_t i = g * 64 + lane;
+            const bool live = have && wgrad_reduce_live(i, r.stride, r.Cout, r.db);
+            if (G == 1) {
+                if (live) wgrad_reduce_store(r.dw, r.db, r.stride, i, wgrad_reduce_part(r.slab, r.stride, r.Cout, r.S, i, 0, 1));
+            } else {
+                double *mine = part + (size_t)slot * G * 64;
+                for (int w = w0; w < G; w += GW)
+                    mine[w * 64 + lane] = live ? wgrad_reduce_part(r.slab, r.stride, r.Cout, r.S, i, w, G) : 0.0;
+                __syncthreads();
+                if (live && w0 == 0) {
+                    double a = mine[lane];
+                    for (int w = 1; w < G; ++w) a += mine[w * 64 + lane];
+                    wgrad_reduce_store(r.dw, r.db, r.stride, i, a);
+                }
+                __syncthreads();
+            }
+        }
+    }
+}
+}
diff --git a/ptbxl-multimodal_amd/ecg_hip/_lib.py b/ptbxl-multimodal_amd/ecg_hip/_lib.py
--- a/ptbxl-multimodal_amd/ecg_hip/_lib.py
+++ b/ptbxl-multimodal_amd/ecg_hip/_lib.py
@@ -29,6 +29,7 @@
     "ecg_conv1d_multiplies_per_output_pair": (_i, [_i] * 5),
     "ecg_conv1d_bwd_data_ld": (_i, [_vp, _i, _vp, _vp, _i, _i, _i, _i, _i, _i, _vp]),
     "ecg_conv1d_bwd_weight_bias_ld": (_i, [_vp, _i, _vp, _vp, _vp, _vp, _i, _i, _i, _i, _i, _i, _vp]),
+    "ecg_conv1d_bwd_weight_data_ld": (_i, [_vp, _i, _vp, _vp, _vp, _vp, _vp, _vp, _i, _i, _i, _i, _i, _i, _vp]),
     "ecg_conv1d_bf16_supported": (_i, [_i, _i, _i, _i]),
     "ecg_conv1d_bf16_packed_elems": (_sz, [_i, _i, _i]),
     "ecg_conv1d_pack_weights_bf16": (_i, [_vp, _vp, _vp, _i, _i, _i, _vp]),
diff --git a/ptbxl-multimodal_amd/ecg_hip/functional.py b/ptbxl-multimodal_amd/ecg_hip/functional.py
--- a/ptbxl-multimodal_amd/ecg_hip/functional.py
+++ b/ptbxl-multimodal_amd/ecg_hip/functional.py
@@ -272,6 +272,10 @@
     return y, partials, P
 
 
+def _fused_weight_data_ok():
+    return L._events is None and _conv_precision != "bf16"
+
+
 def conv1d_backward_raw(x, dy, w_shape, w_bwd, pad, need_dx, need_db=True, ldy=None, sink_keys=(None, None)):
     N, Ci, Lin = x.shape
     Co, _, K = w_shape
@@ -280,6 +284,11 @@
     dw = _grad_out(sink_keys[0], x, Co, Ci, K)
     db = _grad_out(sink_keys[1], x, Co) if need_db else None
     ws = _empty(x, max(1, _query("ecg_conv1d_bwd_weight_ws_floats", N, Ci, Co, Lin, K, pad)))
+    if need_dx and _fused_weight_data_ok():
+        dx = torch.empty_like(x)
+        _call("ecg_conv1d_bwd_weight_data_ld", _f32(dy), ldy, _f32(x), _f32(w_bwd), _f32(dw), _f32(db), _f32(dx), _f32(ws),
+              N, Ci, Co, Lin, K, pad, _st())
+        return dx, dw, db
     _call("ecg_conv1d_bwd_weight_bias_ld", _f32(dy), ldy, _f32(x), _f32(dw), _f32(db), _f32(ws), N, Ci, Co, Lin, K, pad,
           _st())
     dx = None
```

New measurement: 183,800 windows/s (median of 6 runs). +1.2%, better.
